# nhcha6/embodied-object-detection

Measured on AMD Instinct MI355X. Metric: frames/sec (640x640, implicit_memory); frames/sec/GPU = value / n_gpus, higher is better.
Workload: dtype f32

## Files before the change

embodied_object_detection_amd/_lib.py:

```python
from __future__ import annotations

import ctypes as C
import os

HERE = os.path.dirname(os.path.abspath(__file__))
LIB_PATH = os.environ.get("EOD_LIB_PATH") or os.path.join(HERE, "libeod_hip.so")

c_f32p = C.c_void_p
c_i32p = C.c_void_p
c_void_p = C.c_void_p


class EodError(RuntimeError):
    pass


_ERR = {-1: "EOD_ERR_BAD_DIMS", -2: "EOD_ERR_ALIGN", -3: "EOD_ERR_LAUNCH", -4: "EOD_ERR_NULL", -5: "EOD_ERR_CAPACITY"}


MAX_BATCH = 8
MAX_LEVELS = 40
SEMMAP_SCORES = 0x10000
SEMMAP_LOCATE = 0x40000
SEMMAP_PEAKS = 0x80000
SEMMAP_K_SHIFT, SEMMAP_RADIUS_SHIFT, SEMMAP_Q_SHIFT = 12, 20, 24


class EodConvDesc(C.Structure):
    _fields_ = [
        ("x", C.c_void_p), ("w", C.c_void_p), ("bias", C.c_void_p), ("res", C.c_void_p), ("y", C.c_void_p),
        ("workspace", C.c_void_p), ("workspace_bytes", C.c_size_t), ("m_count", C.c_void_p), ("m_unit", C.c_int32),
        ("m_segments", C.c_int32),
        ("N", C.c_int32), ("H", C.c_int32), ("W", C.c_int32), ("Cin", C.c_int32), ("OH", C.c_int32), ("OW", C.c_int32),
        ("Cout", C.c_int32), ("KH", C.c_int32), ("KW", C.c_int32), ("stride", C.c_int32), ("pad", C.c_int32),
        ("Kpad", C.c_int32), ("relu", C.c_int32), ("res_mode", C.c_int32), ("in_relu", C.c_int32),
        ("out_mode", C.c_int32), ("tap4", C.c_int32), ("force_tile", C.c_int32), ("force_splitk", C.c_int32),
        ("out_scale", C.c_float), ("levels", C.c_int32), ("level_off", C.c_int32 * (MAX_LEVELS + 1)), ("level_h", C.c_int32 * MAX_LEVELS),
        ("level_w", C.c_int32 * MAX_LEVELS), ("fuse_w", C.c_void_p), ("out_units", C.c_void_p), ("fuse_b", C.c_float), ("w_split", C.c_void_p),
        ("plan_rows", C.c_int32), ("lds_reserve", C.c_int32), ("gn_partial", C.c_void_p), ("gn_groups", C.c_int32),
        ("y2", C.c_void_p), ("split_n", C.c_int32), ("prefetch2", C.c_int32), ("gate", C.c_void_p),
        ("w_half", C.c_void_p), ("math", C.c_int32),
    ]


class EodConvPlan(C.Structure):
    _fields_ = [(n, C.c_int32) for n in ("tile", "bm", "bn", "bk", "splitk", "cps", "nchunks", "wavek", "glds", "tiles_m", "tiles_n",
                                         "gn_fused")]


class EodBoxRefine(C.Structure):
    _fields_ = [("deltas", C.c_void_p), ("ld", C.c_int32), ("wx", C.c_float), ("wy", C.c_float), ("ww", C.c_float), ("wh", C.c_float),
                ("clip", C.c_int32), ("img_w", C.c_float), ("img_h", C.c_float), ("boxes_out", C.c_void_p)]


class EodCenterNetLossDesc(C.Structure):
    _fields_ = [
        ("head_out", C.c_void_p), ("head_stride", C.c_int32), ("P", C.c_int32), ("levels", C.c_int32), ("level_off", C.c_int32 * 9),
        ("level_scale", C.c_float * 8), ("agn_heatmap", C.c_void_p), ("reg_targets", C.c_void_p), ("pos_inds", C.c_void_p),
        ("n_pos", C.c_int32), ("hm_focal_alpha", C.c_float), ("hm_focal_beta", C.c_float), ("loss_gamma", C.c_float),
        ("sigmoid_clamp", C.c_float), ("ignore_high_fp", C.c_float), ("pos_weight", C.c_float), ("neg_weight", C.c_float),
        ("reg_weight", C.c_float), ("num_pos_avg", C.c_float), ("reg_norm", C.c_float), ("counts_local", C.c_void_p),
        ("counts_total", C.c_void_p), ("world_size", C.c_float), ("d_head_out", C.c_void_p),
        ("losses", C.c_void_p), ("workspace", C.c_void_p), ("workspace_bytes", C.c_size_t),
    ]


class EodCenterNetTargetDesc(C.Structure):
    _fields_ = [
        ("gt_boxes", C.c_void_p), ("n_boxes", C.c_int32), ("levels", C.c_int32), ("level_off", C.c_int32 * 9), ("level_w", C.c_int32 * 8),
        ("level_stride", C.c_int32 * 8), ("soi_lo", C.c_float * 8), ("soi_hi", C.c_float * 8), ("hm_min_overlap", C.c_double),
        ("min_radius", C.c_double), ("agn_heatmap", C.c_void_p), ("reg_targets", C.c_void_p), ("pos_inds", C.c_void_p),
        ("counts", C.c_void_p),
    ]


class EodProposalDesc(C.Structure):
    _fields_ = [
        ("head_out", C.c_void_p), ("head_stride", C.c_int32), ("levels", C.c_int32), ("level_off", C.c_int32 * 6),
        ("level_w", C.c_int32 * 5), ("level_stride", C.c_int32 * 5), ("level_scale", C.c_float * 5),
        ("score_thresh", C.c_float), ("pre_nms_topk", C.c_int32), ("post_nms_topk", C.c_int32), ("nms_thresh", C.c_float),
        ("cap", C.c_int32), ("out_boxes", C.c_void_p), ("out_scores", C.c_void_p), ("out_count", C.c_void_p),
        ("workspace", C.c_void_p), ("workspace_bytes", C.c_size_t), ("batch", C.c_int32),
    ]


class EodDetDesc(C.Structure):
    _fields_ = [
        ("boxes", C.c_void_p), ("scores", C.c_void_p), ("count", C.c_void_p), ("R_cap", C.c_int32), ("C1", C.c_int32),
        ("img_w", C.c_float), ("img_h", C.c_float), ("score_thresh", C.c_float), ("nms_thresh", C.c_float),
        ("topk", C.c_int32), ("out_boxes", C.c_void_p), ("out_scores", C.c_void_p), ("out_classes", C.c_void_p),
        ("out_rows", C.c_void_p), ("out_count", C.c_void_p), ("workspace", C.c_void_p), ("workspace_bytes", C.c_size_t),
        ("out_unique_rows", C.c_void_p), ("out_unique_count", C.c_void_p), ("unique_cap", C.c_int32),
        ("out_rep_of", C.c_void_p), ("out_rep_list", C.c_void_p), ("out_rep_count", C.c_void_p), ("batch", C.c_int32),
    ]


class EodStageTailDesc(C.Structure):
    _fields_ = [("feat", C.c_void_p), ("zs", C.c_void_p), ("prob_acc", C.c_void_p), ("accumulate", C.c_int32), ("feat_norm_out", C.c_void_p),
                ("count", C.c_void_p), ("R_cap", C.c_int32), ("D", C.c_int32), ("C1", C.c_int32), ("temp", C.c_float), ("zs_mem", C.c_void_p),
                ("prop_scores", C.c_void_p), ("mem_scores_out", C.c_void_p), ("final_inv_stages", C.c_float), ("batch", C.c_int32),
                ("hb", C.c_void_p), ("w2", C.c_void_p), ("b2", C.c_void_p), ("hb_dim", C.c_int32), ("w2_ld", C.c_int32),
                ("boxes_in", C.c_void_p), ("boxes_out", C.c_void_p), ("deltas_out", C.c_void_p), ("wx", C.c_float), ("wy", C.c_float),
                ("ww", C.c_float), ("wh", C.c_float), ("clip", C.c_int32), ("img_w", C.c_float), ("img_h", C.c_float)]


class EodAdamWTensor(C.Structure):
    _fields_ = [("param", C.c_void_p), ("grad", C.c_void_p), ("exp_avg", C.c_void_p), ("exp_avg_sq", C.c_void_p), ("n", C.c_size_t),
                ("lr", C.c_double), ("weight_decay", C.c_double), ("step", C.c_int32), ("folded_out", C.c_void_p), ("row_scale", C.c_void_p),
                ("cols", C.c_int32), ("ld_out", C.c_int32), ("grad_of_folded", C.c_int32), ("inv_scale", C.c_float), ("found_inf", C.c_void_p)]


class EodRotateTensor(C.Structure):
    _fields_ = [("w", C.c_void_p), ("out", C.c_void_p), ("Cout", C.c_int32), ("KH", C.c_int32), ("KW", C.c_int32), ("Cin", C.c_int32),
                ("ld_in", C.c_int32), ("ld_out", C.c_int32)]


class EodMemWriteDesc(C.Structure):
    _fields_ = [
        ("featn", C.c_void_p), ("prop_boxes", C.c_void_p), ("prop_masks", C.c_void_p), ("det_rows", C.c_void_p),
        ("det_count", C.c_void_p), ("K_cap", C.c_int32), ("R_cap", C.c_int32), ("proj", C.c_void_p),
        ("H", C.c_int32), ("W", C.c_int32), ("D", C.c_int32), ("n_cells", C.c_int32), ("mask_thresh", C.c_float),
        ("mem", C.c_void_p), ("obs", C.c_void_p), ("k_out", C.c_void_p), ("workspace", C.c_void_p),
        ("workspace_bytes", C.c_size_t), ("dirty", C.c_void_p), ("err_flags", C.c_void_p), ("snapshot_f16", C.c_void_p),
        ("batch", C.c_int32),
    ]


SIGNATURES = {
    "eod_abi_version": (C.c_int, []),
    "eod_conv2d": (C.c_int, [C.POINTER(EodConvDesc), C.c_void_p]),
    "eod_conv2d_workspace_bytes": (C.c_size_t, [C.POINTER(EodConvDesc)]),
    "eod_conv2d_gn_fused": (C.c_int, [C.POINTER(EodConvDesc)]),
    "eod_conv2d_plan": (C.c_int, [C.POINTER(EodConvDesc), C.POINTER(EodConvPlan)]),
    "eod_groupnorm_partial_offset": (C.c_size_t, [C.c_int, C.c_int]),
    "eod_set_conv_math": (C.c_int, [C.c_int]),
    "eod_get_conv_math": (C.c_int, []),
    "eod_conv_split_weights_bytes": (C.c_size_t, [C.c_int, C.c_int]),
    "eod_conv_split_weights_bf16x3": (C.c_int, [C.c_void_p, C.c_int, C.c_int, C.c_void_p, C.c_void_p]),
    "eod_conv_half_weights_bytes": (C.c_size_t, [C.c_int, C.c_int]),
    "eod_conv_half_weights": (C.c_int, [C.c_void_p, C.c_int, C.c_int, C.c_void_p, C.c_void_p]),
    "eod_preprocess_image": (C.c_int, [C.c_void_p, C.c_void_p, C.c_int, C.c_int, C.c_int, C.c_int,
                                       C.POINTER(C.c_float), C.POINTER(C.c_float), C.c_void_p]),
    "eod_maxpool3x3s2": (C.c_int, [C.c_void_p, C.c_void_p] + [C.c_int] * 6 + [C.c_void_p]),
    "eod_groupnorm_workspace_bytes": (C.c_size_t, [C.POINTER(C.c_int32), C.c_int, C.c_int]),
    "eod_groupnorm_relu": (C.c_int, [C.c_void_p, C.c_void_p, C.c_void_p, C.c_void_p, C.POINTER(C.c_int32), C.c_int, C.c_int,
                                     C.c_int, C.c_float, C.c_void_p, C.c_int, C.c_void_p]),
    "eod_groupnorm_backward_workspace_bytes": (C.c_size_t, [C.POINTER(C.c_int32), C.c_int, C.c_int]),
    "eod_groupnorm_relu_backward": (C.c_int, [C.c_void_p, C.c_void_p, C.c_void_p, C.c_void_p, C.POINTER(C.c_int32), C.c_int, C.c_int, C.c_int,
                                              C.c_float, C.c_void_p, C.c_void_p, C.c_void_p, C.c_void_p, C.c_void_p, C.c_void_p]),
    "eod_mask_predictor_sigmoid": (C.c_int, [C.c_void_p, C.c_void_p, C.c_float, C.c_void_p, C.c_int, C.c_int, C.c_void_p,
                                             C.c_int, C.c_void_p, C.c_void_p]),
    "eod_roi_align": (C.c_int, [C.c_void_p, C.c_void_p, C.c_void_p, C.c_int, C.c_int, C.c_int, C.c_void_p, C.c_void_p, C.c_void_p,
                                C.c_int, C.c_int, C.c_void_p, C.c_int, C.c_int, C.c_void_p, C.c_void_p]),
    "eod_roi_align_backward": (C.c_int, [C.c_void_p, C.c_void_p, C.c_void_p, C.c_int, C.c_int, C.c_int, C.c_void_p, C.c_void_p, C.c_int,
                                         C.c_int, C.c_void_p, C.c_void_p]),
    "eod_centernet_loss_workspace_bytes": (C.c_size_t, []),
    "eod_centernet_loss": (C.c_int, [C.POINTER(EodCenterNetLossDesc), C.c_void_p]),
    "eod_fast_rcnn_loss_workspace_bytes": (C.c_size_t, [C.c_int]),
    "eod_fast_rcnn_loss": (C.c_int, [C.c_void_p, C.c_int, C.c_void_p, C.c_void_p, C.c_void_p, C.c_void_p, C.c_void_p, C.c_int, C.c_int,
                                     C.c_float, C.c_float, C.c_float, C.c_float, C.c_float, C.c_void_p, C.c_void_p, C.c_void_p,
                                     C.c_void_p, C.c_size_t, C.c_void_p]),
    "eod_match_label": (C.c_int, [C.c_void_p, C.c_int, C.c_void_p, C.c_void_p, C.c_int, C.c_float, C.c_int, C.c_void_p, C.c_void_p,
                                  C.c_void_p, C.c_void_p, C.c_void_p]),
    "eod_match_label_proposals": (C.c_int, [C.c_void_p, C.c_void_p, C.c_int, C.c_void_p, C.c_void_p, C.c_int, C.c_int, C.c_float, C.c_int,
                                            C.c_void_p, C.c_void_p, C.c_void_p, C.c_void_p, C.c_void_p, C.c_void_p]),
    "eod_sample_proposals": (C.c_int, [C.c_void_p, C.c_void_p, C.c_int, C.c_int, C.c_int, C.c_float, C.c_void_p, C.c_void_p, C.c_void_p]),
    "eod_zs_logits": (C.c_int, [C.c_void_p, C.c_void_p, C.c_int, C.c_int, C.c_int, C.c_float, C.c_void_p, C.c_int, C.c_void_p, C.c_void_p]),
    "eod_zs_logits_backward": (C.c_int, [C.c_void_p, C.c_void_p, C.c_void_p, C.c_int, C.c_int, C.c_int, C.c_int, C.c_float, C.c_void_p,
                                         C.c_void_p]),
    "eod_centernet_targets": (C.c_int, [C.POINTER(EodCenterNetTargetDesc), C.c_void_p]),
    "eod_unique_rows": (C.c_int, [C.c_void_p, C.c_void_p, C.c_int, C.c_int, C.c_void_p, C.c_void_p, C.c_void_p]),
    "eod_proposals_workspace_bytes": (C.c_size_t, [C.c_int, C.c_int, C.c_int, C.c_int]),
    "eod_centernet_proposals": (C.c_int, [C.POINTER(EodProposalDesc), C.c_void_p]),
    "eod_zs_classify": (C.c_int, [C.c_void_p, C.c_void_p, C.c_void_p, C.c_int, C.c_void_p, C.c_void_p, C.c_int, C.c_int,
                                  C.c_int, C.c_float, C.c_void_p, C.c_void_p, C.c_void_p, C.c_float, C.c_int, C.c_void_p]),
    "eod_cascade_stage_tail": (C.c_int, [C.POINTER(EodStageTailDesc), C.c_void_p]),
    "eod_apply_deltas": (C.c_int, [C.c_void_p, C.c_int, C.c_void_p, C.c_void_p, C.c_void_p, C.c_int, C.c_float, C.c_float,
                                   C.c_float, C.c_float, C.c_int, C.c_float, C.c_float, C.c_int, C.c_void_p]),
    "eod_cascade_scores": (C.c_int, [C.c_void_p, C.c_void_p, C.c_void_p, C.c_int, C.c_int, C.c_float, C.c_void_p]),
    "eod_detections_workspace_bytes": (C.c_size_t, [C.c_int, C.c_int]),
    "eod_fast_rcnn_inference": (C.c_int, [C.POINTER(EodDetDesc), C.c_void_p]),
    "eod_detector_postprocess": (C.c_int, [C.c_void_p, C.c_void_p, C.c_void_p, C.c_void_p, C.c_int, C.c_float, C.c_float,
                                           C.c_float, C.c_float, C.c_void_p, C.c_void_p, C.c_void_p, C.c_void_p, C.c_void_p,
                                           C.c_void_p, C.c_int, C.c_void_p]),
    "eod_concat_lists": (C.c_int, [C.c_void_p, C.c_void_p, C.c_int, C.c_int, C.c_int, C.c_void_p, C.c_void_p, C.c_void_p]),
    "eod_paste_masks": (C.c_int, [C.c_void_p, C.c_void_p, C.c_void_p, C.c_void_p, C.c_int, C.c_int, C.c_int, C.c_float,
                                  C.c_void_p, C.c_int, C.c_int, C.c_void_p]),
    "eod_unproject_grid_index": (C.c_int, [C.c_void_p, C.c_int, C.c_int, C.POINTER(C.c_float), C.c_float, C.c_float, C.c_float,
                                           C.c_float, C.POINTER(C.c_float), C.POINTER(C.c_float), C.c_float, C.c_int, C.c_int,
                                           C.c_int, C.c_void_p, C.c_void_p, C.c_void_p]),
    "eod_memory_normalize_f16": (C.c_int, [C.c_void_p, C.c_void_p, C.c_void_p, C.c_int, C.c_int, C.c_void_p]),
    "eod_memory_normalize_dirty_f16": (C.c_int, [C.c_void_p, C.c_void_p, C.c_void_p, C.c_void_p, C.c_int, C.c_int, C.c_void_p]),
    "eod_memory_gather_pool": (C.c_int, [C.c_void_p, C.c_void_p, C.c_int, C.c_int, C.c_int, C.c_int, C.c_void_p, C.c_void_p,
                                         C.c_int, C.c_int, C.c_void_p]),
    "eod_memory_pooled_halves": (C.c_size_t, [C.c_int, C.c_int]),
    "eod_memory_project_weights_bytes": (C.c_size_t, []),
    "eod_memory_project_prepare": (C.c_int, [C.c_void_p] * 8),
    "eod_memory_project_fuse": (C.c_int, [C.c_void_p, C.c_void_p, C.c_void_p, C.c_int, C.c_int, C.c_float, C.c_int, C.c_int, C.c_void_p]),
    "eod_memory_project_backward_weights": (C.c_int, [C.c_void_p] * 4 + [C.c_int, C.c_int, C.c_float] + [C.c_void_p] * 7),
    "eod_memory_project_backward_weights_workspace_bytes": (C.c_size_t, []),
    "eod_memory_project_backward_weights_ws": (C.c_int, [C.c_void_p] * 4 + [C.c_int, C.c_int, C.c_float] + [C.c_void_p] * 7 +
                                               [C.c_size_t, C.c_void_p]),
    "eod_memory_pool_backward": (C.c_int, [C.c_void_p] * 3 + [C.c_int, C.c_int] + [C.c_void_p] * 5),
    "eod_conv2d_backward_weights": (C.c_int, [C.c_void_p, C.c_void_p] + [C.c_int] * 9 + [C.c_void_p, C.c_void_p, C.c_void_p]),
    "eod_conv2d_backward_weights_levels_workspace_bytes": (C.c_size_t, [C.c_int] * 5),
    "eod_conv2d_backward_weights_levels": (C.c_int, [C.c_void_p, C.c_void_p, C.c_int, C.c_void_p, C.c_void_p, C.c_void_p] + [C.c_int] * 5 +
                                           [C.c_void_p, C.c_void_p, C.c_void_p, C.c_size_t, C.c_void_p]),
    "eod_conv2d_backward_weights_workspace_bytes": (C.c_size_t, [C.c_int] * 9),
    "eod_conv2d_backward_weights_ws": (C.c_int, [C.c_void_p, C.c_void_p] + [C.c_int] * 9 + [C.c_void_p, C.c_void_p, C.c_void_p, C.c_size_t,
                                                                                          C.c_void_p]),
    "eod_conv2d_backward_input": (C.c_int, [C.c_void_p, C.c_void_p] + [C.c_int] * 10 + [C.c_void_p, C.c_void_p]),
    "eod_upsample2_sum_backward": (C.c_int, [C.c_void_p, C.c_void_p, C.c_int, C.c_int, C.c_int, C.c_int, C.c_int, C.c_void_p]),
    "eod_maxpool3x3s2_backward": (C.c_int, [C.c_void_p] * 4 + [C.c_int] * 6 + [C.c_void_p]),
    "eod_relu_backward": (C.c_int, [C.c_void_p, C.c_void_p, C.c_void_p, C.c_size_t, C.c_void_p]),
    "eod_adamw_step": (C.c_int, [C.c_void_p, C.c_void_p, C.c_void_p, C.c_void_p, C.c_size_t, C.c_double, C.c_double, C.c_double, C.c_double,
                                 C.c_double, C.c_int, C.c_double, C.c_void_p]),
    "eod_conv_rotate_weights": (C.c_int, [C.c_void_p, C.c_int, C.c_int, C.c_int, C.c_int, C.c_int, C.c_void_p, C.c_int, C.c_void_p]),
    "eod_conv_rotate_weights_multi": (C.c_int, [C.POINTER(EodRotateTensor), C.c_int, C.c_void_p]),
    "eod_adamw_step_multi": (C.c_int, [C.POINTER(EodAdamWTensor), C.c_int, C.c_double, C.c_double, C.c_double, C.c_double, C.c_void_p]),
    "eod_memory_scores": (C.c_int, [C.c_void_p, C.c_void_p, C.c_void_p, C.c_void_p, C.c_void_p, C.c_int, C.c_int, C.c_int,
                                    C.c_void_p]),
    "eod_memory_write_workspace_bytes": (C.c_size_t, [C.c_int] * 6),
    "eod_memory_write_init": (C.c_int, [C.c_void_p, C.c_size_t, C.c_int, C.c_int, C.c_int, C.c_int, C.c_int, C.c_int, C.c_void_p]),
    "eod_memory_write": (C.c_int, [C.POINTER(EodMemWriteDesc), C.c_void_p]),
    "eod_semmap_labels": (C.c_int, [C.c_void_p, C.c_void_p, C.c_void_p, C.c_int, C.c_int, C.c_int, C.c_float, C.c_void_p,
                                    C.c_void_p, C.c_void_p]),
    "eod_fill_f32": (C.c_int, [C.c_void_p, C.c_float, C.c_size_t, C.c_void_p]),
    "eod_fill_i32": (C.c_int, [C.c_void_p, C.c_int32, C.c_size_t, C.c_void_p]),
}

_lib = None


def load():
    global _lib
    if _lib is not None:
        return _lib
    if not os.path.exists(LIB_PATH):
        raise EodError(
            f"{LIB_PATH} is missing: the HIP extension is not built. Run `python -m embodied_object_detection_amd.build` "
            "(hipcc --offload-arch=gfx950). There is no CPU fallback for the product path.")
    lib = C.CDLL(LIB_PATH)
    for name, (res, args) in SIGNATURES.items():
        fn = getattr(lib, name)
        fn.restype = res
        fn.argtypes = args
    _lib = lib
    return lib


def check(status: int, what: str):
    if status != 0:
        raise EodError(f"{what} failed: {_ERR.get(status, status)}")
```

embodied_object_detection_amd/csrc/conv_common.h:

```cpp
#pragma once
#include "eod_common.h"
#include "conv_border_order.h"
#include "../../include/eod_hip.h"

namespace eodconv {


struct ConvArgs {
  const float* x;
  const float* w;
  const float* bias;
  const float* res;
  const float* gate;
  float* y;
  float* partial;
  const int* m_count;
  int m_unit;
  int m_segs, seg_rows;
  const float* fuse_w;
  const int* out_units;
  float fuse_b;
  int N, H, W, Cin, OH, OW, Cout, KH, KW, stride, pad, Kpad;
  int M, nchunks, splitk, cps;
  int relu, res_mode, in_relu, out_mode;
  int tiles_m, tiles_n;
  float out_scale;
  int nlv;
  int lv_off[EOD_MAX_LEVELS + 1], lv_h[EOD_MAX_LEVELS], lv_w[EOD_MAX_LEVELS];
  unsigned x_bytes, w_bytes;
  const void* w3;
  unsigned w3_bytes;
  const void* wh;
  unsigned wh_bytes;
  double* gn_partial;
  int gn_groups;
  float* y2;
  int split_n;
  FastDiv div_ow, div_oh, div_cd, div_row;
  int border;
  FastDiv div_bh, div_bw, div_bi;
};

__device__ __forceinline__ int conv_row_limit(const ConvArgs& p, int M) {
  if (p.m_count && p.m_segs <= 1) {
    const int lim = *p.m_count * p.m_unit;
    M = lim < M ? lim : M;
  }
  return M;
}

__device__ __forceinline__ bool conv_row_active(const ConvArgs& p, int m) {
  if (!p.m_count || p.m_segs <= 1) return true;
  const int s = m / p.seg_rows;
  return m - s * p.seg_rows < p.m_count[s] * p.m_unit;
}

__device__ __forceinline__ bool conv_tile_active(const ConvArgs& p, int m0, int bm) {
  if (!p.m_count || p.m_segs <= 1) return true;
  const int last = (m0 + bm - 1 < p.M ? m0 + bm - 1 : p.M - 1);
  const int s0 = m0 / p.seg_rows, s1 = last / p.seg_rows;
  if (m0 - s0 * p.seg_rows < p.m_count[s0] * p.m_unit) return true;
  for (int s = s0 + 1; s <= s1; ++s)
    if (p.m_count[s] > 0) return true;
  return false;
}

__device__ __forceinline__ int border_rois(const ConvArgs& p) {
  const int c = *p.m_count;
  return c < p.N ? c : p.N;
}
__device__ __forceinline__ int border_storage_row(const ConvArgs& p, int m, int rois) {
  const BorderRow b = border_row(m, rois, p.OH, p.OW, p.div_ow, p.div_bh, p.div_bw, p.div_bi);
  return (b.img * p.OH + b.oy) * p.OW + b.ox;
}

template <bool GATE = false>
__device__ __forceinline__ float epilogue_store(const ConvArgs& p, float v, int m, int n) {
  int co = n;
  size_t oidx;
  if (p.out_mode == 1) {
    const int Cd = p.Cout >> 2;
    const int quad = (int)fdiv((unsigned)n, p.div_cd);
    co = n - quad * Cd;
    const int dy = quad >> 1, dx = quad & 1;
    const int t = (int)fdiv((unsigned)m, p.div_ow);
    const int ox = m - t * p.OW;
    const int img = (int)fdiv((unsigned)t, p.div_oh);
    const int oy = t - img * p.OH;
    oidx = ((size_t)(img * 2 * p.OH + 2 * oy + dy) * (2 * p.OW) + (2 * ox + dx)) * Cd + co;
  } else {
    oidx = (size_t)m * p.Cout + n;
  }
  if (p.bias) v += p.bias[co];
  v *= p.out_scale;
  if (p.res_mode == 1) {
    v += p.res[(size_t)m * p.Cout + n];
  } else if (p.res_mode == 2) {
    const int t = (int)fdiv((unsigned)m, p.div_ow);
    const int ox = m - t * p.OW;
    const int img = (int)fdiv((unsigned)t, p.div_oh);
    const int oy = t - img * p.OH;
    const int rh = p.OH >> 1, rw = p.OW >> 1;
    v += p.res[((size_t)(img * rh + (oy >> 1)) * rw + (ox >> 1)) * p.Cout + n];
  }
  if (p.split_n > 0) {
    if (n >= p.split_n) {
      if (p.relu) v = fmaxf(v, 0.0f);
      p.y2[(size_t)m * (p.Cout - p.split_n) + (n - p.split_n)] = v;
    } else {
      p.y[(size_t)m * p.split_n + n] = v;
    }
    return v;
  }
  if (p.relu) v = fmaxf(v, 0.0f);
  if (GATE && p.gate && !(p.gate[oidx] > 0.0f)) v = 0.0f;
  p.y[oidx] = v;
  return v;
}

__device__ __forceinline__ unsigned long long tap_mask(int iy0, int ix0, int hh, int ww, int KH, int KW) {
  unsigned long long mask = 0;
  int tp = 0;
  for (int ky = 0; ky < KH; ++ky) {
    const bool rok = (unsigned)(iy0 + ky) < (unsigned)hh;
    for (int kx = 0; kx < KW; ++kx, ++tp) {
      const bool ok = rok && ((unsigned)(ix0 + kx) < (unsigned)ww);
      mask |= (unsigned long long)ok << tp;
    }
  }
  return mask;
}

template <int TM, int TN, bool GATE = false, bool BORDER = false>
__device__ __forceinline__ void store_wave_tiles(const ConvArgs& p, const f32x16 (&acc)[TM][TN], int m_base, int n_base, int M, int z,
                                                 int lane) {
  const int half = lane >> 5;
  const int rois = BORDER ? border_rois(p) : 0;
#pragma unroll
  for (int i = 0; i < TM; ++i) {
#pragma unroll
    for (int j = 0; j < TN; ++j) {
      const int n = n_base + j * 32 + (lane & 31);
#pragma unroll
      for (int r = 0; r < 16; ++r) {
        const int row = (r & 3) + 8 * (r >> 2) + 4 * half;
        const int m = m_base + i * 32 + row;
        if (m < M && n < p.Cout && conv_row_active(p, m)) {
          const float v = acc[i][j][r];
          if (BORDER) {
            epilogue_store<GATE>(p, v, border_storage_row(p, m, rois), n);
          } else if (p.splitk > 1) {
            p.partial[((size_t)z * p.M + m) * p.Cout + n] = v;
          } else {
            epilogue_store<GATE>(p, v, m, n);
          }
        }
      }
    }
  }
}

void launch_conv_fp32(const ConvArgs& a, int tile, int bk, bool tap4, dim3 grid, hipStream_t s, int lds_reserve = 0, int prefetch2 = 0);
void launch_conv_bf16x3(const ConvArgs& a, int tile, dim3 grid, hipStream_t s);
void launch_conv_wavek(const ConvArgs& a, int nw, dim3 grid, hipStream_t s);
void launch_conv_pointwise(const ConvArgs& a, int np, dim3 grid, hipStream_t s);
void launch_split_weights(const float* w, void* out, int Cout, int Kpad, hipStream_t s);
void launch_conv_f16(const ConvArgs& a, int tile, int bk, dim3 grid, hipStream_t s);
void launch_half_weights(const float* w, void* out, int Cout, int Kpad, hipStream_t s);

}
```

embodied_object_detection_amd/csrc/conv_fp32.hip:

```cpp
#include "conv_operands.h"

namespace eodconv {
namespace {

template <int BM, int BN, int BK, bool TAP4, bool MULTI, int PIPE = 0>
__global__ __launch_bounds__(256) void conv_igemm_kernel(ConvArgs p) {
  constexpr bool BORDER = PIPE == 3;
  static_assert(!BORDER || (BM == 64 && BN == 64 && BK == 32 && !TAP4 && !MULTI), "border-major order: the plain 64x64 kernel");
  constexpr bool PF2 = PIPE == 1;
  constexpr bool DB = PIPE == 2;
  constexpr int LS = BK + 4;
  constexpr int TM = BM / 64, TN = BN / 64;
  constexpr int QPR = BK / 4;
  constexpr int RPP = 256 / QPR;
  constexpr int AR = BM / RPP, BR = BN / RPP;
  static_assert(!TAP4 || BK == 32, "the stem path stages one 7x7 tap per float4: BK must be 32");
  constexpr int BUF = (BM + BN) * LS;
  __shared__ __attribute__((aligned(16))) float lds[(DB ? 2 : 1) * BUF];
  float* As = lds;
  float* Bs = lds + BM * LS;

  const int tid = threadIdx.x;
  const int lane = tid & 63;
  const int wave = tid >> 6;
  const int wm = wave >> 1, wn = wave & 1;

  int M, tile_m, tile_n;
  if constexpr (BORDER) {
    if (!conv_claim_tile_border<BM>(p, M, tile_m, tile_n)) return;
  } else {
    const int t = conv_first_tile<BM>(p, M);
    if (t < 0) return;
    tile_m = t / p.tiles_n;
    tile_n = t - tile_m * p.tiles_n;
  }
  const int m0 = tile_m * BM, n0 = tile_n * BN;
  if (!conv_tile_active(p, m0, BM)) return;
  const int z = blockIdx.y;
  int c_end;
  const int c_begin = conv_chunk_range(p, p.cps, z, c_end);

  const int lr = tid / QPR, lq = tid % QPR;
  int a_off[AR], a_iy[AR], a_ix[AR];
  unsigned a_voff[AR];
  unsigned long long a_mask[AR];
  unsigned a_pitch[MULTI ? AR : 1];
  const int rois = BORDER ? border_rois(p) : 0;
#pragma unroll
  for (int i = 0; i < AR; ++i) {
    const int m = m0 + lr + RPP * i;
    const bool rowok = m < M;
    RowOrigin o;
    if constexpr (BORDER) o = conv_row_origin_border(p, m, rowok, rois);
    else o = conv_row_origin<MULTI>(p, m, rowok);
    a_iy[i] = rowok ? o.iy0 : -(1 << 28);
    a_ix[i] = o.ix0;
    a_off[i] = o.off;
    if (!TAP4) conv_row_address<MULTI>(p, o, rowok, lq, a_voff[i], a_mask[i], a_pitch[MULTI ? i : 0]);
  }
  unsigned w_voff[BR];
#pragma unroll
  for (int j = 0; j < BR; ++j) w_voff[j] = conv_w_row_offset(p, n0 + lr + RPP * j, lq);
  const __amdgpu_buffer_rsrc_t rsrc_x = conv_buffer(p.x, p.x_bytes);
  const __amdgpu_buffer_rsrc_t rsrc_w = conv_buffer(p.w, p.w_bytes);

  unsigned live = 0;
  if constexpr (BORDER) {
    unsigned mine = 0;
#pragma unroll
    for (int i = 0; i < AR; ++i) mine |= (unsigned)a_mask[i];
    unsigned wv = 0;
#pragma unroll
    for (int tp = 0; tp < 9; ++tp) wv |= (__ballot((mine >> tp) & 1u) != 0ull ? 1u : 0u) << tp;
    if (lane == 0) lds[wave] = __uint_as_float(wv);
    __syncthreads();
    live = __float_as_uint(lds[0]) | __float_as_uint(lds[1]) | __float_as_uint(lds[2]) | __float_as_uint(lds[3]);
    live = __builtin_amdgcn_readfirstlane(live);
    __syncthreads();
    c_end = c_begin + __popc(live) * (p.Cin / BK);
  }

  f32x4 ar0[AR], br0[BR];
  f32x4 ar1[PF2 ? AR : 1], br1[PF2 ? BR : 1];
  ChunkWalker<BK, MULTI> walk(p, c_begin);
  auto load_chunk = [&](int chunk, auto& ar, auto& br) {
    int k0 = chunk * BK;
    if (!TAP4) {
      if constexpr (BORDER) {
        const unsigned rest = live >> walk.tap;
        if (walk.c0 == 0 && !(rest & 1u)) walk.seek(p, walk.tap + __builtin_ctz(rest));
      }
      const TapInfo ti = walk.next(p);
      if constexpr (BORDER) k0 = (int)(ti.k0b >> 2);
#pragma unroll
      for (int i = 0; i < AR; ++i) ar[i] = conv_load_a<MULTI>(rsrc_x, ti, a_voff[i], a_mask[i], a_pitch[MULTI ? i : 0]);
    } else {
      const int tap = chunk * 8 + lq;
      const int ky = tap / p.KW;
      const int kx = tap - ky * p.KW;
      const bool tv = tap < p.KH * p.KW;
#pragma unroll
      for (int i = 0; i < AR; ++i) {
        const int iy = a_iy[i] + ky, ix = a_ix[i] + kx;
        const bool ok = tv && ((unsigned)iy < (unsigned)p.H) && ((unsigned)ix < (unsigned)p.W);
        f32x4 v = {0.f, 0.f, 0.f, 0.f};
        if (ok) v = *reinterpret_cast<const f32x4*>(p.x + (size_t)(a_off[i] + iy * p.W + ix) * 4);
        ar[i] = v;
      }
    }
    if (p.in_relu) {
#pragma unroll
      for (int i = 0; i < AR; ++i) ar[i] = conv_relu4(ar[i]);
    }
#pragma unroll
    for (int j = 0; j < BR; ++j)
      br[j] = __builtin_bit_cast(f32x4, __builtin_amdgcn_raw_buffer_load_b128(rsrc_w, w_voff[j], k0 * 4, 0));
  };

  f32x16 acc[TM][TN];
#pragma unroll
  for (int i = 0; i < TM; ++i)
#pragma unroll
    for (int j = 0; j < TN; ++j)
#pragma unroll
      for (int r = 0; r < 16; ++r) acc[i][j][r] = 0.f;
  f32x16 acc_b;
#pragma unroll
  for (int r = 0; r < 16; ++r) acc_b[r] = 0.f;

  const int frag_row = lane & 31;
  const int frag_k = 4 * (lane >> 5);
  const float* a_base = As + (wm * TM * 32 + frag_row) * LS + frag_k;
  const float* b_base = Bs + (wn * TN * 32 + frag_row) * LS + frag_k;

  auto multiply = [&](const float* ab, const float* bb) {
#pragma unroll
    for (int kk = 0; kk < BK / 8; ++kk) {
      f32x4 af[TM], bf[TN];
#pragma unroll
      for (int i = 0; i < TM; ++i) af[i] = *reinterpret_cast<const f32x4*>(ab + i * 32 * LS + kk * 8);
#pragma unroll
      for (int j = 0; j < TN; ++j) bf[j] = *reinterpret_cast<const f32x4*>(bb + j * 32 * LS + kk * 8);
      __builtin_amdgcn_s_setprio(1);
#pragma unroll
      for (int tt = 0; tt < 4; ++tt)
#pragma unroll
        for (int i = 0; i < TM; ++i)
#pragma unroll
          for (int j = 0; j < TN; ++j)
            if (TM * TN == 1 && (tt & 1))
              acc_b = __builtin_amdgcn_mfma_f32_32x32x2f32(af[i][tt], bf[j][tt], acc_b, 0, 0, 0);
            else
              acc[i][j] = __builtin_amdgcn_mfma_f32_32x32x2f32(af[i][tt], bf[j][tt], acc[i][j], 0, 0, 0);
      __builtin_amdgcn_s_setprio(0);
    }
  };
  auto stage_and_multiply = [&](auto& ar, auto& br, int next_chunk) {
#pragma unroll
    for (int i = 0; i < AR; ++i) *reinterpret_cast<f32x4*>(As + (lr + RPP * i) * LS + 4 * lq) = ar[i];
#pragma unroll
    for (int j = 0; j < BR; ++j) *reinterpret_cast<f32x4*>(Bs + (lr + RPP * j) * LS + 4 * lq) = br[j];
    __syncthreads();
    if (next_chunk < c_end) load_chunk(next_chunk, ar, br);
    if constexpr (TM * TN == 1) {
      f32x4 af[2], bf[2];
      af[0] = *reinterpret_cast<const f32x4*>(a_base);
      bf[0] = *reinterpret_cast<const f32x4*>(b_base);
#pragma unroll
      for (int kk = 0; kk < BK / 8; ++kk) {
        const int cur = kk & 1, nxt = cur ^ 1;
        if (kk + 1 < BK / 8) {
          af[nxt] = *reinterpret_cast<const f32x4*>(a_base + (kk + 1) * 8);
          bf[nxt] = *reinterpret_cast<const f32x4*>(b_base + (kk + 1) * 8);
        }
        __builtin_amdgcn_s_setprio(1);
#pragma unroll
        for (int tt = 0; tt < 4; ++tt)
          if (tt & 1)
            acc_b = __builtin_amdgcn_mfma_f32_32x32x2f32(af[cur][tt], bf[cur][tt], acc_b, 0, 0, 0);
          else
            acc[0][0] = __builtin_amdgcn_mfma_f32_32x32x2f32(af[cur][tt], bf[cur][tt], acc[0][0], 0, 0, 0);
        __builtin_amdgcn_s_setprio(0);
      }
    } else {
      multiply(a_base, b_base);
    }
    __syncthreads();
  };
  load_chunk(c_begin, ar0, br0);
  if constexpr (DB) {
    auto store_tiles = [&](int buf) {
#pragma unroll
      for (int i = 0; i < AR; ++i) *reinterpret_cast<f32x4*>(As + buf * BUF + (lr + RPP * i) * LS + 4 * lq) = ar0[i];
#pragma unroll
      for (int j = 0; j < BR; ++j) *reinterpret_cast<f32x4*>(Bs + buf * BUF + (lr + RPP * j) * LS + 4 * lq) = br0[j];
    };
    store_tiles(0);
    __syncthreads();
    int cur = 0;
    for (int chunk = c_begin; chunk < c_end; ++chunk) {
      const bool more = chunk + 1 < c_end;
      if (more) load_chunk(chunk + 1, ar0, br0);
      multiply(a_base + cur * BUF, b_base + cur * BUF);
      if (more) store_tiles(cur ^ 1);
      __syncthreads();
      cur ^= 1;
    }
  } else if constexpr (PF2) {
    if (c_begin + 1 < c_end) load_chunk(c_begin + 1, ar1, br1);
    for (int chunk = c_begin; chunk < c_end; chunk += 2) {
      stage_and_multiply(ar0, br0, chunk + 2);
      if (chunk + 1 < c_end) stage_and_multiply(ar1, br1, chunk + 3);
    }
  } else {
    for (int chunk = c_begin; chunk < c_end; ++chunk) stage_and_multiply(ar0, br0, chunk + 1);
  }

  if (TM * TN == 1) {
#pragma unroll
    for (int r = 0; r < 16; ++r) acc[0][0][r] += acc_b[r];
  }
  if constexpr (BM == 64 && BN == 256) {
    if (p.out_mode == 2) {
      float sred[16];
#pragma unroll
      for (int r = 0; r < 16; ++r) sred[r] = 0.f;
#pragma unroll
      for (int j = 0; j < TN; ++j) {
        const int co = (wn * TN + j) * 32 + (lane & 31);
        const float bw = p.bias ? p.bias[co] : 0.f;
        const float pw = p.fuse_w[co];
#pragma unroll
        for (int r = 0; r < 16; ++r) {
          float v = (acc[0][j][r] + bw) * p.out_scale;
          if (p.relu) v = fmaxf(v, 0.f);
          sred[r] += v * pw;
        }
      }
#pragma unroll
      for (int off = 16; off > 0; off >>= 1)
#pragma unroll
        for (int r = 0; r < 16; ++r) sred[r] += __shfl_xor(sred[r], off, 64);
      float* red = lds;
      if ((lane & 31) == 0) {
        const int half = lane >> 5;
#pragma unroll
        for (int r = 0; r < 16; ++r) red[(wm * 2 + wn) * 32 + (r & 3) + 8 * (r >> 2) + 4 * half] = sred[r];
      }
      __syncthreads();
      if (tid < BM) {
        const int wr = tid >> 5, rr = tid & 31;
        const float v = red[(wr * 2 + 0) * 32 + rr] + red[(wr * 2 + 1) * 32 + rr] + p.fuse_b;
        const int m = m0 + tid;
        if (m < M) {
          const int tq = (int)fdiv((unsigned)m, p.div_ow);
          const int ox = m - tq * p.OW;
          const int img = (int)fdiv((unsigned)tq, p.div_oh);
          const int oy = tq - img * p.OH;
          const int unit = p.out_units ? p.out_units[img] : img;
          const int dy = tile_n >> 1, dx = tile_n & 1;
          p.y[((size_t)unit * 2 * p.OH + 2 * oy + dy) * (2 * p.OW) + 2 * ox + dx] = eod_sigmoid_precise(v);
        }
      }
      return;
    }
  }
  store_wave_tiles<TM, TN, BM == 64 && BN == 64, BORDER>(p, acc, m0 + wm * TM * 32, n0 + wn * TN * 32, M, z, lane);
}


template <int NW, bool MULTI>
__global__ __launch_bounds__(NW * 64) void conv_wavek_kernel(ConvArgs p) {
  constexpr int BK = 32;
  constexpr int LS = BK + 4;
  constexpr int AR = 4;
  __shared__ __attribute__((aligned(16))) float lds[NW * 2 * 32 * LS];
  const int tid = threadIdx.x;
  const int lane = tid & 63;
  const int wave = tid >> 6;
  float* As = lds + wave * (2 * 32 * LS);
  float* Bs = As + 32 * LS;

  int M;
  const int t = conv_first_tile<32>(p, M);
  if (t < 0) return;
  const int tile_m = t / p.tiles_n;
  const int tile_n = t - tile_m * p.tiles_n;
  const int m0 = tile_m * 32, n0 = tile_n * 32;
  if (!conv_tile_active(p, m0, 32)) return;

  int c_end;
  const int c_begin = conv_chunk_range(p, (p.nchunks + NW - 1) / NW, wave, c_end);

  const int lr = lane >> 3, lq = lane & 7;
  unsigned a_voff[AR];
  unsigned long long a_mask[AR];
  unsigned a_pitch[MULTI ? AR : 1];
  unsigned w_voff[AR];
#pragma unroll
  for (int i = 0; i < AR; ++i) {
    conv_row_address<MULTI>(p, m0 + lr + 8 * i, M, lq, a_voff[i], a_mask[i], a_pitch[MULTI ? i : 0]);
    w_voff[i] = conv_w_row_offset(p, n0 + lr + 8 * i, lq);
  }
  const __amdgpu_buffer_rsrc_t rsrc_x = conv_buffer(p.x, p.x_bytes);
  const __amdgpu_buffer_rsrc_t rsrc_w = conv_buffer(p.w, p.w_bytes);

  f32x4 ar0[AR], br0[AR], ar1[AR], br1[AR];
  ChunkWalker<BK, MULTI> walk(p, c_begin);
  auto load_chunk = [&](int chunk, f32x4 (&ar)[AR], f32x4 (&br)[AR]) {
    const int k0 = chunk * BK;
    const TapInfo ti = walk.next(p);
#pragma unroll
    for (int i = 0; i < AR; ++i) ar[i] = conv_load_a<MULTI>(rsrc_x, ti, a_voff[i], a_mask[i], a_pitch[MULTI ? i : 0]);
    if (p.in_relu) {
#pragma unroll
      for (int i = 0; i < AR; ++i) ar[i] = conv_relu4(ar[i]);
    }
#pragma unroll
    for (int j = 0; j < AR; ++j)
      br[j] = __builtin_bit_cast(f32x4, __builtin_amdgcn_raw_buffer_load_b128(rsrc_w, w_voff[j], k0 * 4, 0));
  };

  f32x16 acc, acc_b;
#pragma unroll
  for (int r = 0; r < 16; ++r) {
    acc[r] = 0.f;
    acc_b[r] = 0.f;
  }
  const int frag_row = lane & 31;
  const int frag_k = 4 * (lane >> 5);
  const float* a_base = As + frag_row * LS + frag_k;
  const float* b_base = Bs + frag_row * LS + frag_k;

  auto stage_and_multiply = [&](f32x4 (&ar)[AR], f32x4 (&br)[AR], int next_chunk) {
#pragma unroll
    for (int i = 0; i < AR; ++i) *reinterpret_cast<f32x4*>(As + (lr + 8 * i) * LS + 4 * lq) = ar[i];
#pragma unroll
    for (int j = 0; j < AR; ++j) *reinterpret_cast<f32x4*>(Bs + (lr + 8 * j) * LS + 4 * lq) = br[j];
    __builtin_amdgcn_fence(__ATOMIC_RELEASE, "wavefront");
    __builtin_amdgcn_wave_barrier();
    __builtin_amdgcn_fence(__ATOMIC_ACQUIRE, "wavefront");
    if (next_chunk < c_end) load_chunk(next_chunk, ar, br);
#pragma unroll
    for (int kk = 0; kk < BK / 8; ++kk) {
      const f32x4 af = *reinterpret_cast<const f32x4*>(a_base + kk * 8);
      const f32x4 bf = *reinterpret_cast<const f32x4*>(b_base + kk * 8);
      acc = __builtin_amdgcn_mfma_f32_32x32x2f32(af[0], bf[0], acc, 0, 0, 0);
      acc_b = __builtin_amdgcn_mfma_f32_32x32x2f32(af[1], bf[1], acc_b, 0, 0, 0);
      acc = __builtin_amdgcn_mfma_f32_32x32x2f32(af[2], bf[2], acc, 0, 0, 0);
      acc_b = __builtin_amdgcn_mfma_f32_32x32x2f32(af[3], bf[3], acc_b, 0, 0, 0);
    }
    __builtin_amdgcn_fence(__ATOMIC_RELEASE, "wavefront");
    __builtin_amdgcn_wave_barrier();
    __builtin_amdgcn_fence(__ATOMIC_ACQUIRE, "wavefront");
  };
  if (c_begin < c_end) load_chunk(c_begin, ar0, br0);
  if (c_begin + 1 < c_end) load_chunk(c_begin + 1, ar1, br1);
  for (int chunk = c_begin; chunk < c_end; chunk += 2) {
    stage_and_multiply(ar0, br0, chunk + 2);
    if (chunk + 1 < c_end) stage_and_multiply(ar1, br1, chunk + 3);
  }
#pragma unroll
  for (int r = 0; r < 16; ++r) acc[r] += acc_b[r];

  __syncthreads();
  float* red = lds;
  if (wave > 0) {
#pragma unroll
    for (int r = 0; r < 16; ++r) red[((wave - 1) * 16 + r) * 64 + lane] = acc[r];
  }
  __syncthreads();
  if (wave != 0) return;
#pragma unroll
  for (int w = 1; w < NW; ++w)
#pragma unroll
    for (int r = 0; r < 16; ++r) acc[r] += red[((w - 1) * 16 + r) * 64 + lane];
  f32x16 out[1][1];
  out[0][0] = acc;
  store_wave_tiles<1, 1, true>(p, out, m0, n0, M, 0, lane);
}

}

template <int BM, int BN>
static void launch_fp32_tile(const ConvArgs& a, bool tap4, int bk, dim3 grid, hipStream_t s, int dyn) {
  if (tap4)
    hipLaunchKernelGGL((conv_igemm_kernel<BM, BN, 32, true, false>), grid, dim3(256), dyn, s, a);
  else if (a.nlv > 0 && bk == 64)
    hipLaunchKernelGGL((conv_igemm_kernel<BM, BN, 64, false, true>), grid, dim3(256), dyn, s, a);
  else if (a.nlv > 0)
    hipLaunchKernelGGL((conv_igemm_kernel<BM, BN, 32, false, true>), grid, dim3(256), dyn, s, a);
  else if (bk == 64)
    hipLaunchKernelGGL((conv_igemm_kernel<BM, BN, 64, false, false>), grid, dim3(256), dyn, s, a);
  else
    hipLaunchKernelGGL((conv_igemm_kernel<BM, BN, 32, false, false>), grid, dim3(256), dyn, s, a);
}

void launch_conv_fp32(const ConvArgs& a, int tile, int bk, bool tap4, dim3 grid, hipStream_t s, int lds_reserve, int prefetch2) {
  const int dyn = lds_reserve > 0 ? lds_reserve : 0;
  if (a.border) {
    hipLaunchKernelGGL((conv_igemm_kernel<64, 64, 32, false, false, 3>), grid, dim3(256), dyn, s, a);
    return;
  }
  if (prefetch2 == 1 && !tap4 && a.nlv == 0 && bk == 32 && tile == 3) {
    hipLaunchKernelGGL((conv_igemm_kernel<64, 64, 32, false, false, 1>), grid, dim3(256), dyn, s, a);
    return;
  }
  if (prefetch2 == 2 && !tap4 && bk == 32 && tile == 3) {
    if (a.nlv > 0) hipLaunchKernelGGL((conv_igemm_kernel<64, 64, 32, false, true, 2>), grid, dim3(256), dyn, s, a);
    else hipLaunchKernelGGL((conv_igemm_kernel<64, 64, 32, false, false, 2>), grid, dim3(256), dyn, s, a);
    return;
  }
  switch (tile) {
    case 5: hipLaunchKernelGGL((conv_igemm_kernel<64, 256, 32, false, false>), grid, dim3(256), dyn, s, a); break;
    case 1: launch_fp32_tile<128, 128>(a, tap4, bk, grid, s, dyn); break;
    case 2: launch_fp32_tile<128, 64>(a, tap4, bk, grid, s, dyn); break;
    default: launch_fp32_tile<64, 64>(a, tap4, bk, grid, s, dyn); break;
  }
}

void launch_conv_wavek(const ConvArgs& a, int nw, dim3 grid, hipStream_t s) {
  if (a.nlv > 0) {
    if (nw == 8) hipLaunchKernelGGL((conv_wavek_kernel<8, true>), grid, dim3(512), 0, s, a);
    else hipLaunchKernelGGL((conv_wavek_kernel<4, true>), grid, dim3(256), 0, s, a);
  } else {
    if (nw == 8) hipLaunchKernelGGL((conv_wavek_kernel<8, false>), grid, dim3(512), 0, s, a);
    else hipLaunchKernelGGL((conv_wavek_kernel<4, false>), grid, dim3(256), 0, s, a);
  }
}

}
```

embodied_object_detection_amd/csrc/conv_igemm.hip:

```cpp
#include "conv_common.h"
#include "../../include/eod_hip.h"
#include <atomic>
#include <cstdlib>
#include <cstring>

namespace {

using namespace eodconv;

template <int VEC>
__global__ __launch_bounds__(256) void conv_splitk_reduce_kernel(ConvArgs p) {
  EOD_CHAIN_PRIO();
  const int M = conv_row_limit(p, p.M);
  const unsigned per_row = (unsigned)p.Cout / VEC;
  const unsigned total = (unsigned)M * per_row;
  const size_t slab = (size_t)p.M * p.Cout;
  for (unsigned idx = blockIdx.x * blockDim.x + threadIdx.x; idx < total; idx += gridDim.x * blockDim.x) {
    const unsigned m = fdiv(idx, p.div_row);
    if (!conv_row_active(p, (int)m)) continue;
    const unsigned n = (idx - m * per_row) * VEC;
    const float* src = p.partial + (size_t)m * p.Cout + n;
    if (VEC == 4) {
      f32x4 v = {0.f, 0.f, 0.f, 0.f};
      for (int zb = 0; zb < p.splitk; zb += 4) {
        f32x4 t[4];
#pragma unroll
        for (int j = 0; j < 4; ++j)
          if (zb + j < p.splitk) t[j] = *reinterpret_cast<const f32x4*>(src + (size_t)(zb + j) * slab);
#pragma unroll
        for (int j = 0; j < 4; ++j)
          if (zb + j < p.splitk) v += t[j];
      }
      epilogue_store<true>(p, v.x, (int)m, (int)n);
      epilogue_store<true>(p, v.y, (int)m, (int)n + 1);
      epilogue_store<true>(p, v.z, (int)m, (int)n + 2);
      epilogue_store<true>(p, v.w, (int)m, (int)n + 3);
    } else {
      float v = 0.f;
      for (int z = 0; z < p.splitk; ++z) v += src[z * slab];
      epilogue_store<true>(p, v, (int)m, (int)n);
    }
  }
}

#define EOD_GN_ROWS 32
__global__ __launch_bounds__(256) void conv_splitk_reduce_gn_kernel(ConvArgs p) {
  EOD_CHAIN_PRIO();
  __shared__ double red[4][64][2];
  int level = 0, first_chunk = 0;
  for (;;) {
    const int rows = p.lv_off[level + 1] - p.lv_off[level];
    const int nch = (rows + EOD_GN_ROWS - 1) / EOD_GN_ROWS;
    if ((int)blockIdx.x < first_chunk + nch || level + 1 >= p.nlv) break;
    first_chunk += nch;
    ++level;
  }
  const int r0 = p.lv_off[level] + ((int)blockIdx.x - first_chunk) * EOD_GN_ROWS;
  const int r1 = min(r0 + EOD_GN_ROWS, p.lv_off[level + 1]);
  const int C = p.Cout;
  const int c4 = C >> 2;
  const int nsub = 256 / c4;
  const int col = threadIdx.x % c4, sub = threadIdx.x / c4;
  const int cpg4 = (C / p.gn_groups) >> 2;
  const size_t slab = (size_t)p.M * C;
  double s = 0.0, q = 0.0;
  for (int r = r0 + sub; r < r1; r += nsub) {
    const float* src = p.partial + (size_t)r * C + col * 4;
    f32x4 v = {0.f, 0.f, 0.f, 0.f};
    for (int zb = 0; zb < p.splitk; zb += 4) {
      f32x4 t[4];
#pragma unroll
      for (int j = 0; j < 4; ++j)
        if (zb + j < p.splitk) t[j] = *reinterpret_cast<const f32x4*>(src + (size_t)(zb + j) * slab);
#pragma unroll
      for (int j = 0; j < 4; ++j)
        if (zb + j < p.splitk) v += t[j];
    }
    const double o0 = (double)epilogue_store<true>(p, v.x, r, col * 4 + 0);
    const double o1 = (double)epilogue_store<true>(p, v.y, r, col * 4 + 1);
    const double o2 = (double)epilogue_store<true>(p, v.z, r, col * 4 + 2);
    const double o3 = (double)epilogue_store<true>(p, v.w, r, col * 4 + 3);
    s += o0; q += o0 * o0;
    s += o1; q += o1 * o1;
    s += o2; q += o2 * o2;
    s += o3; q += o3 * o3;
  }
  for (int off = 1; off < cpg4; off <<= 1) {
    s += __shfl_xor(s, off, 64);
    q += __shfl_xor(q, off, 64);
  }
  if ((col % cpg4) == 0) {
    red[sub][col / cpg4][0] = s;
    red[sub][col / cpg4][1] = q;
  }
  __syncthreads();
  if ((int)threadIdx.x < p.gn_groups) {
    double ts = 0.0, tq = 0.0;
    for (int u = 0; u < nsub; ++u) {
      ts += red[u][threadIdx.x][0];
      tq += red[u][threadIdx.x][1];
    }
    p.gn_partial[((size_t)blockIdx.x * p.gn_groups + threadIdx.x) * 2 + 0] = ts;
    p.gn_partial[((size_t)blockIdx.x * p.gn_groups + threadIdx.x) * 2 + 1] = tq;
  }
}

std::atomic<int>& math_mode() {
  static std::atomic<int> v([] {
    const char* e = getenv("EOD_CONV_MATH");
    if (e && strcmp(e, "bf16x3") == 0) return EOD_MATH_BF16X3;
    if (e && strcmp(e, "f16") == 0) return EOD_MATH_F16;
    return EOD_MATH_FP32;
  }());
  return v;
}

struct Plan {
  int tile;
  int bk;
  int glds;
  int bm, bn, tiles_m, tiles_n, splitk, cps, nchunks;
  int wavek;
  int pw_np;
  int border;
};

constexpr int kForcePointwise = 30;

int effective_math(const EodConvDesc* d) { return d->math > 0 ? d->math - 1 : math_mode().load(std::memory_order_relaxed); }

bool pointwise_eligible(const EodConvDesc* d) {
  return effective_math(d) == EOD_MATH_FP32 && d->KH == 1 && d->KW == 1 && d->stride == 1 && d->pad == 0 && d->levels <= 0 && !d->tap4 &&
         d->Cin == d->Kpad && (d->Cin == 64 || d->Cin == 128 || d->Cin == 256) && d->Cout % 64 == 0 && d->out_mode == 0 &&
         (d->res_mode == 0 || d->res_mode == 1) && !d->in_relu && !d->gate && !d->m_count && d->split_n == 0 && !d->gn_partial &&
         d->lds_reserve == 0;
}

constexpr int kForceBorder = 43;
constexpr bool kBorderAuto = true;

bool border_eligible(const EodConvDesc* d) {
  return effective_math(d) == EOD_MATH_FP32 && d->KH == 3 && d->KW == 3 && d->stride == 1 && d->pad == 1 && d->levels <= 0 && !d->tap4 &&
         d->m_count && d->m_segments <= 1 && d->m_unit == d->OH * d->OW && d->OH >= 3 && d->OW >= 3 && d->Cin % 32 == 0 &&
         d->out_mode == 0 && d->res_mode == 0 && !d->in_relu && !d->gate && d->split_n == 0 && !d->gn_partial && d->prefetch2 == 0;
}

Plan make_plan(const EodConvDesc* d, int M) {
  static const int cfg[5][2] = {{128, 128}, {128, 64}, {64, 64}, {256, 128}, {64, 256}};
  Plan pl{};
  int pick = 2;
  const int ft = d->force_tile % 10, fbk = d->force_tile / 10;
  const bool half_ok = !d->tap4 && !d->in_relu;
  const bool f16_forced = (fbk == 8 || fbk == 9) && half_ok;
  if (f16_forced) pick = ft == 4 ? 3 : 2;
  else if (ft >= 1 && ft <= 3) pick = ft - 1;
  else if (ft == 4 && fbk == 5 && half_ok) pick = 3;
  const bool bk64_ok = !d->tap4 && d->Cin % 64 == 0 && d->Kpad % 64 == 0;
  pl.glds = f16_forced ? 3 : ((fbk == 5 && half_ok) ? 2 : 0);
  const int Mp = (d->plan_rows > 0 && d->plan_rows < M) ? d->plan_rows : M;
  const int math = effective_math(d);
  if (d->force_tile == 0 && math == EOD_MATH_F16 && half_ok) {
    pl.glds = 3;
    pick = (long)((Mp + 255) / 256) * ((d->Cout + 127) / 128) >= 256 ? 3 : 2;
  }
  if (d->force_tile == 0 && math == EOD_MATH_BF16X3 && half_ok) {
    pl.glds = 2;
    const long t128 = (long)((Mp + 127) / 128) * ((d->Cout + 127) / 128);
    const long t256 = (long)((Mp + 255) / 256) * ((d->Cout + 127) / 128);
    pick = t256 >= 256 ? 3 : (t128 >= 512 ? 0 : 2);
  }
  if (d->out_mode == 2) {
    pick = 4;
    pl.glds = 0;
  }
  if (d->gate) {
    const bool f16_gated = d->math == EOD_MATH_F16 + 1 && half_ok && d->levels <= 0 && (d->force_tile == 0 || f16_forced);
    pick = 2;
    pl.glds = f16_gated ? 3 : 0;
  }
  if (pl.glds == 3) pl.bk = (fbk == 8 && d->Cin % 64 == 0) ? 64 : 32;
  else pl.bk = (pl.glds == 0 && d->out_mode != 2 && fbk == 2 && bk64_ok) ? 64 : 32;
  const int nchunks = d->Kpad / pl.bk;
  pl.nchunks = nchunks;
  pl.tile = pick + 1;
  pl.bm = cfg[pick][0];
  pl.bn = cfg[pick][1];
  pl.tiles_m = (M + pl.bm - 1) / pl.bm;
  pl.tiles_n = (d->Cout + pl.bn - 1) / pl.bn;
  const long tiles = (long)((Mp + pl.bm - 1) / pl.bm) * pl.tiles_n;
  int splitk = 1;
  if (d->out_mode == 2) {
    splitk = 1;
  } else if (d->force_splitk > 0) {
    splitk = d->force_splitk;
  } else if (pl.glds == 0 && !d->tap4 && nchunks >= 8 &&
             ((d->force_tile == 6 || d->force_tile == 7) ||
              (tiles < 256 && nchunks <= 192 && pl.bk == 32 && d->force_tile == 0 &&
               ((Mp <= 512 && nchunks / (nchunks >= 64 ? 8 : 4) >= 8) || nchunks >= 128)))) {
    pl.wavek = d->force_tile == 6 ? 4 : (d->force_tile == 7 ? 8 : (nchunks >= 64 ? 8 : 4));
    pl.bk = 32;
    pl.nchunks = d->Kpad / 32;
    pl.bm = pl.bn = 32;
    pl.tiles_m = (M + 31) / 32;
    pl.tiles_n = (d->Cout + 31) / 32;
  } else if (tiles < 256 && nchunks >= 8) {
    const int target = (nchunks >= 128 && Mp <= 512) ? 1792 : 512;
    int want = (int)((target + tiles - 1) / tiles);
    int maxs = nchunks / 4;
    splitk = want < maxs ? want : maxs;
    if (splitk < 1) splitk = 1;
  } else if (tiles >= 256 && tiles <= 1024 && d->m_count == nullptr && nchunks >= 18) {
    double best = 1e30;
    for (int sct = 1; sct <= 4; ++sct) {
      if (nchunks / sct < 9) break;
      const double est = (double)((tiles * sct + 255) / 256) / sct + (sct > 1 ? 0.12 : 0.0);
      if (est < best - 1e-9) {
        best = est;
        splitk = sct;
      }
    }
  }
  if (splitk > nchunks) splitk = nchunks;
  pl.cps = (nchunks + splitk - 1) / splitk;
  pl.splitk = (nchunks + pl.cps - 1) / pl.cps;
  const bool pw_forced = d->force_tile == kForcePointwise && d->force_splitk <= 1;
  const bool pw_auto = d->force_tile == 0 && d->force_splitk == 0 && pointwise_eligible(d) && pl.splitk == 1 && !pl.wavek && tiles >= 256 &&
                       !(d->Kpad == 256 && d->Cout < 1024);
  if (pw_forced || pw_auto) {
    const int panels = d->Cout / 64;
    const long row_tiles = (Mp + 63) / 64;
    const long want = tiles >= 256 ? 512 : 1;
    int np = 1;
    for (int cand = 4; cand > 1; cand >>= 1)
      if (panels >= cand && row_tiles * ((panels + cand - 1) / cand) >= want) {
        np = cand;
        break;
      }
    pl.pw_np = np;
    pl.tile = 6;
    pl.glds = 0;
    pl.bk = 32;
    pl.nchunks = d->Kpad / 32;
    pl.bm = 64;
    pl.bn = 64 * np;
    pl.tiles_m = (M + 63) / 64;
    pl.tiles_n = (panels + np - 1) / np;
    pl.splitk = 1;
    pl.cps = pl.nchunks;
    pl.wavek = 0;
  }
  const bool border_forced = d->force_tile == kForceBorder && d->force_splitk <= 1;
  const bool border_auto = kBorderAuto && d->force_tile == 0 && border_eligible(d) && pl.glds == 0 && pl.tile == 3 && pl.bk == 32 &&
                           pl.splitk == 1 && !pl.wavek;
  if (border_forced) {
    pl.splitk = 1;
    pl.cps = pl.nchunks;
  }
  pl.border = (border_forced || border_auto) ? 1 : 0;
  return pl;
}

int total_rows(const EodConvDesc* d) { return d->levels > 0 ? d->level_off[d->levels] : d->N * d->OH * d->OW; }

int check_desc(const EodConvDesc* d) {
  if (!d || !d->x || !d->w || !d->y) return EOD_ERR_NULL;
  if (d->N <= 0 || d->Cin <= 0 || d->Cout <= 0) return EOD_ERR_BAD_DIMS;
  if (d->levels <= 0 && (d->H <= 0 || d->W <= 0 || d->OH <= 0 || d->OW <= 0)) return EOD_ERR_BAD_DIMS;
  if (d->KH <= 0 || d->KW <= 0 || d->stride <= 0 || d->pad < 0) return EOD_ERR_BAD_DIMS;
  if (d->Kpad % 32 != 0 || d->Kpad < d->KH * d->KW * d->Cin) return EOD_ERR_BAD_DIMS;
  if (d->tap4) {
    if (d->Cin != 4) return EOD_ERR_BAD_DIMS;
  } else {
    if (d->Cin % 32 != 0 || d->Kpad != d->KH * d->KW * d->Cin) return EOD_ERR_BAD_DIMS;
  }
  if (d->levels > 0) {
    if (d->levels > EOD_MAX_LEVELS || d->N != 1 || d->stride != 1 || d->KH != d->KW || d->pad != d->KH / 2 || d->tap4 || d->out_mode != 0 ||
        d->res_mode == 2 || d->level_off[0] != 0)
      return EOD_ERR_BAD_DIMS;
    for (int l = 0; l < d->levels; ++l)
      if (d->level_h[l] <= 0 || d->level_w[l] <= 0 || d->level_off[l + 1] - d->level_off[l] != d->level_h[l] * d->level_w[l])
        return EOD_ERR_BAD_DIMS;
  } else {
    if (d->OH != (d->H + 2 * d->pad - d->KH) / d->stride + 1) return EOD_ERR_BAD_DIMS;
    if (d->OW != (d->W + 2 * d->pad - d->KW) / d->stride + 1) return EOD_ERR_BAD_DIMS;
  }
  if (d->levels <= 0 && (long)d->N * d->H * d->W * d->Cin >= (1L << 29)) return EOD_ERR_BAD_DIMS;
  if ((long)d->Cout * d->Kpad >= (1L << 29)) return EOD_ERR_BAD_DIMS;
  if (d->KH * d->KW > 64) return EOD_ERR_BAD_DIMS;
  if ((long)total_rows(d) * (d->Cout > d->Cin ? d->Cout : d->Cin) >= (1L << 31)) return EOD_ERR_BAD_DIMS;
  if (d->out_mode == 1 && (d->Cout % 4 != 0)) return EOD_ERR_BAD_DIMS;
  if (d->out_mode == 2) {
    if (d->Cout != 1024 || d->KH != 1 || d->KW != 1 || d->stride != 1 || d->tap4 || d->levels > 0 || d->res_mode != 0 || d->in_relu ||
        d->force_splitk > 1)
      return EOD_ERR_BAD_DIMS;
    if (!d->fuse_w) return EOD_ERR_NULL;
  }
  if (d->out_mode < 0 || d->out_mode > 2) return EOD_ERR_BAD_DIMS;
  if (d->res_mode != 0 && !d->res) return EOD_ERR_NULL;
  if (d->res_mode == 2 && ((d->OH & 1) || (d->OW & 1))) return EOD_ERR_BAD_DIMS;
  if (d->m_count && d->m_unit <= 0) return EOD_ERR_BAD_DIMS;
  if (d->m_segments > 1) {
    if (!d->m_count || d->levels > 0 || d->out_mode == 2 || d->m_segments > EOD_MAX_BATCH || d->N % d->m_segments != 0)
      return EOD_ERR_BAD_DIMS;
    if (((long)(d->N / d->m_segments) * d->OH * d->OW) % d->m_unit != 0) return EOD_ERR_BAD_DIMS;
  }
  if (d->gate && (d->out_mode != 0 || d->split_n != 0 || d->gn_partial)) return EOD_ERR_BAD_DIMS;
  if (d->gate && d->force_tile != 0 && d->force_tile % 10 != 3 && d->force_tile != 6 && d->force_tile != 7) return EOD_ERR_BAD_DIMS;
  if (d->gate && d->force_tile / 10 == 5) return EOD_ERR_BAD_DIMS;
  if (d->gate && (d->force_tile / 10 == 8 || d->force_tile / 10 == 9) &&
      (d->math != EOD_MATH_F16 + 1 || d->force_tile % 10 != 3 || d->levels > 0 || d->tap4 || d->in_relu))
    return EOD_ERR_BAD_DIMS;
  if (d->math < 0 || d->math > EOD_MATH_F16 + 1) return EOD_ERR_BAD_DIMS;
  if ((d->force_tile / 10 == 8 || d->force_tile / 10 == 9) && d->force_tile % 10 != 3 && d->force_tile % 10 != 4) return EOD_ERR_BAD_DIMS;
  if (d->lds_reserve < 0 || d->lds_reserve > 48 * 1024) return EOD_ERR_BAD_DIMS;
  if (d->force_tile == kForcePointwise && (!pointwise_eligible(d) || d->force_splitk > 1)) return EOD_ERR_BAD_DIMS;
  if (d->force_tile == kForceBorder && (!border_eligible(d) || d->force_splitk > 1)) return EOD_ERR_BAD_DIMS;
  if (d->split_n != 0) {
    if (!d->y2) return EOD_ERR_NULL;
    if (d->split_n < 0 || d->split_n >= d->Cout || d->out_mode != 0 || d->res_mode != 0 || d->levels > 0 || d->gn_partial)
      return EOD_ERR_BAD_DIMS;
  }
  if (d->gn_partial) {
    const int cpg = d->gn_groups > 0 ? d->Cout / d->gn_groups : 0;
    if (d->levels <= 0 || d->m_count || d->out_mode != 0 || d->gn_groups <= 0 || d->gn_groups > 64 || d->Cout % d->gn_groups != 0 ||
        cpg > 64 || (cpg & (cpg - 1)) != 0 || cpg < 4 || d->Cout % 4 != 0 || d->Cout > 1024 || 256 % (d->Cout / 4) != 0 ||
        64 % (cpg / 4) != 0)
      return EOD_ERR_BAD_DIMS;
  }
  if (!eod_aligned16(d->x) || !eod_aligned16(d->w) || !eod_aligned16(d->w_split) || !eod_aligned16(d->w_half)) return EOD_ERR_ALIGN;
  return EOD_OK;
}

}

extern "C" int eod_set_conv_math(int mode) {
  if (mode != EOD_MATH_FP32 && mode != EOD_MATH_BF16X3 && mode != EOD_MATH_F16) return EOD_ERR_BAD_DIMS;
  return math_mode().exchange(mode);
}

extern "C" int eod_get_conv_math(void) { return math_mode().load(); }

extern "C" size_t eod_conv_split_weights_bytes(int Cout, int Kpad) {
  return (Cout > 0 && Kpad > 0 && Kpad % 32 == 0) ? (size_t)Cout * Kpad * 6 : 0;
}

extern "C" int eod_conv_split_weights_bf16x3(const float* w, int Cout, int Kpad, void* out, eod_stream_t stream) {
  if (!w || !out) return EOD_ERR_NULL;
  if (Cout <= 0 || Kpad <= 0 || Kpad % 32 != 0 || (long)Cout * Kpad * 6 >= (1L << 32)) return EOD_ERR_BAD_DIMS;
  if (!eod_aligned16(w) || !eod_aligned16(out)) return EOD_ERR_ALIGN;
  launch_split_weights(w, out, Cout, Kpad, static_cast<hipStream_t>(stream));
  return eod_launch_status();
}

extern "C" size_t eod_conv_half_weights_bytes(int Cout, int Kpad) {
  return (Cout > 0 && Kpad > 0 && Kpad % 32 == 0) ? (size_t)Cout * Kpad * 2 : 0;
}

extern "C" int eod_conv_half_weights(const float* w, int Cout, int Kpad, void* out, eod_stream_t stream) {
  if (!w || !out) return EOD_ERR_NULL;
  if (Cout <= 0 || Kpad <= 0 || Kpad % 32 != 0 || (long)Cout * Kpad >= (1L << 29)) return EOD_ERR_BAD_DIMS;
  if (!eod_aligned16(w) || !eod_aligned16(out)) return EOD_ERR_ALIGN;
  launch_half_weights(w, out, Cout, Kpad, static_cast<hipStream_t>(stream));
  return eod_launch_status();
}

extern "C" int eod_conv2d_gn_fused(const EodConvDesc* d) {
  EodConvDesc t = *d;
  t.gn_partial = nullptr;
  if (check_desc(&t) != EOD_OK) return 0;
  return make_plan(&t, total_rows(&t)).splitk > 1 ? 1 : 0;
}

extern "C" int eod_conv2d_plan(const EodConvDesc* d, EodConvPlan* out) {
  if (!out) return EOD_ERR_NULL;
  const int st = check_desc(d);
  if (st != EOD_OK) return st;
  const Plan pl = make_plan(d, total_rows(d));
  out->tile = pl.tile; out->bm = pl.bm; out->bn = pl.bn; out->bk = pl.bk;
  out->splitk = pl.splitk; out->cps = pl.cps; out->nchunks = pl.nchunks;
  out->wavek = pl.wavek; out->glds = pl.glds;
  out->tiles_m = pl.tiles_m; out->tiles_n = pl.tiles_n;
  out->gn_fused = (d->gn_partial && pl.splitk > 1) ? 1 : 0;
  return EOD_OK;
}

extern "C" size_t eod_conv2d_workspace_bytes(const EodConvDesc* d) {
  if (check_desc(d) != EOD_OK) return 0;
  const int M = total_rows(d);
  const Plan pl = make_plan(d, M);
  if (pl.splitk <= 1) return 0;
  return (size_t)pl.splitk * M * d->Cout * sizeof(float);
}

extern "C" int eod_conv2d(const EodConvDesc* d, eod_stream_t stream) {
  const int st = check_desc(d);
  if (st != EOD_OK) return st;
  hipStream_t s = static_cast<hipStream_t>(stream);
  ConvArgs a{};
  a.x = d->x; a.w = d->w; a.bias = d->bias; a.res = d->res; a.y = d->y;
  a.partial = d->workspace;
  a.m_count = d->m_count; a.m_unit = d->m_unit;
  a.m_segs = d->m_segments > 1 ? d->m_segments : 1;
  a.seg_rows = a.m_segs > 1 ? (d->N / d->m_segments) * d->OH * d->OW : 0;
  a.fuse_w = d->fuse_w; a.out_units = d->out_units; a.fuse_b = d->fuse_b;
  a.N = d->N; a.H = d->H; a.W = d->W; a.Cin = d->Cin; a.OH = d->OH; a.OW = d->OW; a.Cout = d->Cout;
  a.KH = d->KH; a.KW = d->KW; a.stride = d->stride; a.pad = d->pad; a.Kpad = d->Kpad;
  a.M = total_rows(d);
  a.div_ow = eod_make_fastdiv((unsigned)(d->OW > 0 ? d->OW : 1));
  a.div_oh = eod_make_fastdiv((unsigned)(d->OH > 0 ? d->OH : 1));
  a.div_row = eod_make_fastdiv((unsigned)(d->Cout % 4 == 0 ? d->Cout / 4 : d->Cout));
  a.div_cd = eod_make_fastdiv((unsigned)((d->Cout >> 2) > 0 ? (d->Cout >> 2) : 1));
  a.div_bh = eod_make_fastdiv((unsigned)(d->OH > 2 ? d->OH - 2 : 1));
  a.div_bw = eod_make_fastdiv((unsigned)(d->OW > 2 ? d->OW - 2 : 1));
  a.div_bi = eod_make_fastdiv((unsigned)(d->OH > 2 && d->OW > 2 ? (d->OH - 2) * (d->OW - 2) : 1));
  {
    const size_t xe = d->levels > 0 ? (size_t)d->level_off[d->levels] * d->Cin : (size_t)d->N * d->H * d->W * d->Cin;
    a.x_bytes = (unsigned)(xe * sizeof(float));
    a.w_bytes = (unsigned)((size_t)d->Cout * d->Kpad * sizeof(float));
    a.w3 = d->w_split;
    a.w3_bytes = (unsigned)((size_t)d->Cout * d->Kpad * 6);
    a.wh = d->w_half;
    a.wh_bytes = (unsigned)((size_t)d->Cout * d->Kpad * 2);
  }
  a.nlv = d->levels > 0 ? d->levels : 0;
  for (int l = 0; l < a.nlv; ++l) {
    a.lv_off[l] = d->level_off[l];
    a.lv_h[l] = d->level_h[l];
    a.lv_w[l] = d->level_w[l];
  }
  if (a.nlv) a.lv_off[a.nlv] = d->level_off[a.nlv];
  a.relu = d->relu; a.res_mode = d->res_mode; a.in_relu = d->in_relu; a.out_mode = d->out_mode;
  a.gate = d->gate;
  a.out_scale = d->out_scale;
  a.gn_partial = d->gn_partial;
  a.gn_groups = d->gn_groups;
  a.y2 = d->y2;
  a.split_n = d->split_n;
  const Plan pl = make_plan(d, a.M);
  if (d->gn_partial && pl.splitk <= 1) return EOD_ERR_BAD_DIMS;
  a.nchunks = pl.nchunks;
  a.splitk = pl.splitk; a.cps = pl.cps; a.tiles_m = pl.tiles_m; a.tiles_n = pl.tiles_n;
  a.border = pl.border;
  if (pl.splitk > 1) {
    const size_t need = (size_t)pl.splitk * a.M * a.Cout * sizeof(float);
    if (!d->workspace || d->workspace_bytes < need) return EOD_ERR_CAPACITY;
  }
  dim3 grid(pl.tiles_m * pl.tiles_n, pl.splitk);
  if (pl.border) grid.x = (pl.tiles_m + 7) / 8 * 8 * pl.tiles_n;
  if (pl.pw_np) launch_conv_pointwise(a, pl.pw_np, grid, s);
  else if (pl.wavek) launch_conv_wavek(a, pl.wavek, grid, s);
  else if (pl.glds == 3) launch_conv_f16(a, pl.tile, pl.bk, grid, s);
  else if (pl.glds == 2) launch_conv_bf16x3(a, pl.tile, grid, s);
  else launch_conv_fp32(a, pl.tile, pl.bk, d->tap4 != 0, grid, s, d->lds_reserve, d->prefetch2);
  if (pl.splitk > 1) {
    const size_t total = (size_t)a.M * a.Cout;
    const bool vec = a.Cout % 4 == 0;
    int blocks = (int)((total / (vec ? 4 : 1) + 255) / 256);
    if (blocks > 2048) blocks = 2048;
    if (blocks < 1) blocks = 1;
    if (a.gn_partial) {
      int chunks = 0;
      for (int l = 0; l < a.nlv; ++l) chunks += (a.lv_off[l + 1] - a.lv_off[l] + EOD_GN_ROWS - 1) / EOD_GN_ROWS;
      hipLaunchKernelGGL(conv_splitk_reduce_gn_kernel, dim3(chunks), dim3(256), 0, s, a);
    } else if (vec) hipLaunchKernelGGL(conv_splitk_reduce_kernel<4>, dim3(blocks), dim3(256), 0, s, a);
    else hipLaunchKernelGGL(conv_splitk_reduce_kernel<1>, dim3(blocks), dim3(256), 0, s, a);
  }
  return eod_launch_status();
}
```

embodied_object_detection_amd/csrc/conv_operands.h:

```cpp
#pragma once
#include "conv_common.h"

namespace eodconv {

template <int BM>
__device__ __forceinline__ int conv_first_tile(const ConvArgs& p, int& M) {
  M = conv_row_limit(p, p.M);
  const int ntiles = ((M + BM - 1) / BM) * p.tiles_n;
  if ((int)blockIdx.x >= ntiles) return -1;
  return xcd_remap(blockIdx.x, ntiles);
}

template <int BM>
__device__ __forceinline__ bool conv_claim_tile_border(const ConvArgs& p, int& M, int& tile_m, int& tile_n) {
  M = conv_row_limit(p, p.M);
  const int live = (M + BM - 1) / BM;
  const int xcd = blockIdx.x & 7, k = blockIdx.x >> 3;
  const int g = k / p.tiles_n;
  const int r = g * 8 + xcd;
  tile_n = k - g * p.tiles_n;
  tile_m = live - 1 - r;
  return r < live;
}

__device__ __forceinline__ int conv_chunk_range(const ConvArgs& p, int per, int idx, int& c_end) {
  const int c_begin = idx * per;
  c_end = c_begin + per;
  if (c_end > p.nchunks) c_end = p.nchunks;
  return c_begin;
}

struct RowOrigin {
  int iy0, ix0, off, hh, ww;
};
template <bool MULTI>
__device__ __forceinline__ RowOrigin conv_row_origin(const ConvArgs& p, int m, bool rowok) {
  RowOrigin o = {0, 0, 0, 1, 1};
  if (rowok) {
    if (MULTI) {
      int l = 0;
      while (l + 1 < p.nlv && m >= p.lv_off[l + 1]) ++l;
      const int local = m - p.lv_off[l];
      o.ww = p.lv_w[l];
      o.hh = p.lv_h[l];
      const int oy = local / o.ww;
      o.iy0 = oy - p.pad;
      o.ix0 = (local - oy * o.ww) - p.pad;
      o.off = p.lv_off[l];
    } else {
      const int t = (int)fdiv((unsigned)m, p.div_ow);
      const int ox = m - t * p.OW;
      const int img = (int)fdiv((unsigned)t, p.div_oh);
      const int oy = t - img * p.OH;
      o.iy0 = oy * p.stride - p.pad;
      o.ix0 = ox * p.stride - p.pad;
      o.off = img * p.H * p.W;
      o.hh = p.H;
      o.ww = p.W;
    }
  }
  return o;
}

__device__ __forceinline__ RowOrigin conv_row_origin_border(const ConvArgs& p, int m, bool rowok, int rois) {
  RowOrigin o = {0, 0, 0, 1, 1};
  if (rowok) {
    const BorderRow b = border_row(m, rois, p.OH, p.OW, p.div_ow, p.div_bh, p.div_bw, p.div_bi);
    o.iy0 = b.oy * p.stride - p.pad;
    o.ix0 = b.ox * p.stride - p.pad;
    o.off = b.img * p.H * p.W;
    o.hh = p.H;
    o.ww = p.W;
  }
  return o;
}

template <bool MULTI>
__device__ __forceinline__ void conv_row_address(const ConvArgs& p, const RowOrigin& o, bool rowok, int lq, unsigned& voff,
                                                 unsigned long long& mask, unsigned& pitch) {
  mask = rowok ? tap_mask(o.iy0, o.ix0, o.hh, o.ww, p.KH, p.KW) : 0ull;
  voff = (unsigned)(((o.off + o.iy0 * o.ww + o.ix0) * p.Cin + 4 * lq) * 4);
  if (MULTI) pitch = (unsigned)(o.ww * p.Cin * 4);
}
template <bool MULTI>
__device__ __forceinline__ void conv_row_address(const ConvArgs& p, int m, int M, int lq, unsigned& voff, unsigned long long& mask,
                                                 unsigned& pitch) {
  const bool rowok = m < M;
  conv_row_address<MULTI>(p, conv_row_origin<MULTI>(p, m, rowok), rowok, lq, voff, mask, pitch);
}

__device__ __forceinline__ unsigned conv_w_row_offset(const ConvArgs& p, int n, int lq) {
  return n < p.Cout ? (unsigned)((n * p.Kpad + 4 * lq) * 4) : 0xFFFFFFFFu;
}

__device__ __forceinline__ __amdgpu_buffer_rsrc_t conv_buffer(const void* ptr, unsigned bytes) {
  return __builtin_amdgcn_make_buffer_rsrc(const_cast<void*>(ptr), 0, bytes, 0x00020000);
}

struct TapInfo {
  int tap, ky;
  unsigned tap_off, k0b;
};

template <int BK, bool MULTI>
struct ChunkWalker {
  int tap, c0, ky, kx, k0;
  __device__ __forceinline__ ChunkWalker(const ConvArgs& p, int c_begin) {
    k0 = c_begin * BK;
    tap = k0 / p.Cin;
    c0 = k0 - tap * p.Cin;
    ky = tap / p.KW;
    kx = tap - ky * p.KW;
  }
  __device__ __forceinline__ void seek(const ConvArgs& p, int t) {
    tap = t;
    c0 = 0;
    k0 = t * p.Cin;
    ky = t / p.KW;
    kx = t - ky * p.KW;
  }
  __device__ __forceinline__ TapInfo next(const ConvArgs& p) {
    TapInfo ti;
    ti.tap = tap < 63 ? tap : 63;
    ti.ky = ky;
    ti.tap_off = MULTI ? (unsigned)((kx * p.Cin + c0) * 4) : (unsigned)(((ky * p.W + kx) * p.Cin + c0) * 4);
    ti.k0b = (unsigned)(k0 * 4);
    k0 += BK;
    c0 += BK;
    if (c0 >= p.Cin) {
      c0 = 0;
      ++tap;
      if (++kx == p.KW) {
        kx = 0;
        ++ky;
      }
    }
    return ti;
  }
};

template <bool MULTI>
__device__ __forceinline__ f32x4 conv_load_a(__amdgpu_buffer_rsrc_t rsrc_x, const TapInfo& ti, unsigned voff, unsigned long long mask,
                                             unsigned pitch) {
  const bool ok = (mask >> ti.tap) & 1ull;
  unsigned vo = voff + ti.tap_off;
  if (MULTI) vo += (unsigned)ti.ky * pitch;
  vo = ok ? vo : 0xFFFFFFFFu;
  return __builtin_bit_cast(f32x4, __builtin_amdgcn_raw_buffer_load_b128(rsrc_x, vo, 0, 0));
}

__device__ __forceinline__ f32x4 conv_relu4(f32x4 v) {
  v.x = fmaxf(v.x, 0.f);
  v.y = fmaxf(v.y, 0.f);
  v.z = fmaxf(v.z, 0.f);
  v.w = fmaxf(v.w, 0.f);
  return v;
}

}
```

embodied_object_detection_amd/modeling/backbone.py:

```python
from __future__ import annotations

from typing import Dict, List, Optional, Tuple

import torch

from .. import ops
from ..registry import BACKBONE_REGISTRY

RESNET50_LAYERS = (3, 4, 6, 3)


class ResNet50Trunk:
    def __init__(self, sd: Dict[str, torch.Tensor], device):
        base = "backbone.bottom_up.base"

        def bn(p):
            return sd[f"{p}.weight"], sd[f"{p}.bias"], sd[f"{p}.running_mean"], sd[f"{p}.running_var"]

        w, b = ops.fold_bn(sd[f"{base}.conv1.weight"], *bn(f"{base}.bn1"))
        self.stem = ops.Conv(w, b, stride=2, pad=3, device=device, cin_pad=4, name="stem")
        self.blocks: List[Tuple] = []
        for li, nblk in enumerate(RESNET50_LAYERS, start=1):
            for bi in range(nblk):
                p = f"{base}.layer{li}.{bi}"
                stride = 2 if (bi == 0 and li > 1) else 1
                w1, b1 = ops.fold_bn(sd[f"{p}.conv1.weight"], *bn(f"{p}.bn1"))
                w2, b2 = ops.fold_bn(sd[f"{p}.conv2.weight"], *bn(f"{p}.bn2"))
                w3, b3 = ops.fold_bn(sd[f"{p}.conv3.weight"], *bn(f"{p}.bn3"))
                c1 = ops.Conv(w1, b1, device=device, name=f"{p}.conv1")
                c2 = ops.Conv(w2, b2, stride=stride, pad=1, device=device, name=f"{p}.conv2")
                c3 = ops.Conv(w3, b3, device=device, name=f"{p}.conv3")
                ds = None
                if f"{p}.downsample.0.weight" in sd:
                    wd, bd = ops.fold_bn(sd[f"{p}.downsample.0.weight"], *bn(f"{p}.downsample.1"))
                    ds = ops.Conv(wd, bd, stride=stride, device=device, name=f"{p}.downsample")
                self.blocks.append((li, c1, c2, c3, ds))

    def forward(self, x4: torch.Tensor, H: int, W: int, N: int = 1, plan_like_single: bool = True, keep: Optional[dict] = None,
                math: Optional[str] = None):
        mk = {} if math is None else {"math": math}

        def pr(conv, hh, ww):
            oh, ow = conv.out_hw(hh, ww)
            return oh * ow if (N > 1 and plan_like_single) else 0

        x = self.stem(x4, N, H, W, relu=True, plan_rows=pr(self.stem, H, W), **mk)
        h, w = self.stem.out_hw(H, W)
        stem_out, hs, ws = x, h, w
        x, h, w = ops.maxpool3x3s2(x, N, h, w, 64)
        if keep is not None:
            keep["stem"] = (stem_out, hs, ws, x, h, w)
            keep["blocks"] = []
        feats = {}
        cur_layer = 1
        for (li, c1, c2, c3, ds) in self.blocks:
            if li != cur_layer:
                feats[f"layer{cur_layer + 1}"] = (x, h, w)
                cur_layer = li
            sc = x
            if ds is not None:
                sc = ds(x, N, h, w, plan_rows=pr(ds, h, w), **mk)
            o = c1(x, N, h, w, relu=True, plan_rows=pr(c1, h, w), **mk)
            o1 = o
            o = c2(o, N, h, w, relu=True, plan_rows=pr(c2, h, w), **mk)
            h2, w2 = c2.out_hw(h, w)
            x_in = x
            x = c3(o, N, h2, w2, res=sc, res_mode=1, relu=True, plan_rows=pr(c3, h2, w2), **mk)
            if keep is not None:
                keep["blocks"].append((x_in, o1, o, x, h, w, h2, w2))
            h, w = h2, w2
        feats[f"layer{cur_layer + 1}"] = (x, h, w)
        return feats


class CustomRecurrentFPN:
    size_divisibility = 32

    def __init__(self, cfg, sd: Dict[str, torch.Tensor], device):
        self.device = device
        self.memory_type = cfg.MODEL.MEMORY_TYPE
        self.feat_fusion = cfg.MODEL.MAP_FEAT_FUSION
        self.map_feature_weight = float(cfg.MODEL.MAP_FEATURE_WEIGHT)
        if self.memory_type == "implicit_memory" and self.feat_fusion not in ("sum", "mem_only", "image_only"):
            raise ValueError(f"MODEL.MAP_FEAT_FUSION={self.feat_fusion!r} not supported (timm.py:181-186)")
        self.bottom_up = ResNet50Trunk(sd, device)
        self.lateral, self.output = {}, {}
        for l in (3, 4, 5):
            self.lateral[l] = ops.Conv(sd[f"backbone.fpn_lateral{l}.weight"], sd[f"backbone.fpn_lateral{l}.bias"], device=device,
                                       name=f"fpn_lateral{l}")
            self.output[l] = ops.Conv(sd[f"backbone.fpn_output{l}.weight"], sd[f"backbone.fpn_output{l}.bias"], pad=1, device=device,
                                      name=f"fpn_output{l}")
        self.p6 = ops.Conv(sd["backbone.top_block.p6.weight"], sd["backbone.top_block.p6.bias"], stride=2, pad=1, device=device, name="p6")
        self.p7 = ops.Conv(sd["backbone.top_block.p7.weight"], sd["backbone.top_block.p7.bias"], stride=2, pad=1, device=device, name="p7")
        self.merge = ops.MemoryProjector([sd[f"backbone.map_merge_projection{i}.weight"] for i in (1, 2, 3)],
                                         [sd[f"backbone.map_merge_projection{i}.bias"] for i in (1, 2, 3)], device)
        self._plans = {}
        self.pool_in_torch_order = True

    def level_shapes(self, H: int, W: int) -> List[Tuple[int, int]]:
        hw = [(H // 8, W // 8), (H // 16, W // 16), (H // 32, W // 32)]
        h6, w6 = self.p6.out_hw(*hw[2])
        h7, w7 = self.p7.out_hw(h6, w6)
        return hw + [(h6, w6), (h7, w7)]

    def _plan(self, H: int, W: int, which: int = 0):
        key = (H, W, which)
        if key not in self._plans:
            shapes = self.level_shapes(H, W)
            off = [0]
            for (h, w) in shapes:
                off.append(off[-1] + h * w)
            feats = torch.empty((off[-1], 256), dtype=torch.float32, device=self.device)
            views = [feats[off[i]:off[i + 1]].view(1, shapes[i][0], shapes[i][1], 256) for i in range(5)]
            pooled = torch.empty((ops.pooled_rows(H, W), 512), dtype=torch.float16, device=self.device)
            self._plans[key] = (shapes, off, feats, views, pooled)
        return self._plans[key]

    def top_down(self, c: dict, H: int, W: int, which: int = 0):
        shapes, off, feats, views, pooled = self._plan(H, W, which)
        (c5, h5, w5), (c4, h4, w4), (c3, h3, w3) = c["layer5"], c["layer4"], c["layer3"]
        assert (h3, w3) == shapes[0] and (h5, w5) == shapes[2]
        lat5 = self.lateral[5](c5, 1, h5, w5)
        self.output[5](lat5, 1, h5, w5, out=views[2])
        lat4 = self.lateral[4](c4, 1, h4, w4, res=lat5, res_mode=2)
        self.output[4](lat4, 1, h4, w4, out=views[1])
        lat3 = self.lateral[3](c3, 1, h3, w3, res=lat4, res_mode=2)
        self.output[3](lat3, 1, h3, w3, out=views[0])

    def top_down_batched(self, c: dict, H: int, W: int, N: int):
        (c5, h5, w5), (c4, h4, w4), (c3, h3, w3) = c["layer5"], c["layer4"], c["layer3"]
        lat5 = self.lateral[5](c5, N, h5, w5, plan_rows=h5 * w5)
        p5 = self.output[5](lat5, N, h5, w5, plan_rows=h5 * w5)
        lat4 = self.lateral[4](c4, N, h4, w4, res=lat5, res_mode=2, plan_rows=h4 * w4)
        p4 = self.output[4](lat4, N, h4, w4, plan_rows=h4 * w4)
        lat3 = self.lateral[3](c3, N, h3, w3, res=lat4, res_mode=2, plan_rows=h3 * w3)
        p3 = self.output[3](lat3, N, h3, w3, plan_rows=h3 * w3)
        return [p3, p4, p5]

    def fuse_memory_and_top(self, H: int, W: int, memory_f16: Optional[torch.Tensor], proj: Optional[torch.Tensor], which: int = 0,
                            err: Optional[torch.Tensor] = None):
        shapes, off, feats, views, pooled = self._plan(H, W, which)
        h5, w5 = shapes[2]
        if self.memory_type == "implicit_memory" and self.feat_fusion != "image_only":
            if memory_f16 is None or proj is None:
                raise ValueError("implicit_memory needs the fp16 memory table and proj_indices")
            ops.memory_gather_pool(memory_f16, proj, H, W, out=pooled, err=err, torch_order=self.pool_in_torch_order)
            self.merge(pooled, feats, H, W, self.map_feature_weight, self.feat_fusion)
        self.p6(views[2], 1, h5, w5, out=views[3])
        self.p7(views[3], 1, shapes[3][0], shapes[3][1], in_relu=True, out=views[4])
        return feats, views, shapes, off

    def forward(self, x4: torch.Tensor, H: int, W: int, memory_f16: Optional[torch.Tensor], proj: Optional[torch.Tensor],
                which: int = 0, err: Optional[torch.Tensor] = None):
        self.top_down(self.bottom_up.forward(x4, H, W), H, W, which)
        return self.fuse_memory_and_top(H, W, memory_f16, proj, which, err)


@BACKBONE_REGISTRY.register()
def build_p67_timm_fpn_backbone_recurrent(cfg, sd, device):
    if cfg.MODEL.TIMM.BASE_NAME != "resnet50_in21k_map":
        raise ValueError("MODEL.TIMM.BASE_NAME must be 'resnet50_in21k_map' for the recurrent path")
    return CustomRecurrentFPN(cfg, sd, device)
```

embodied_object_detection_amd/modeling/batched.py:

```python
from __future__ import annotations

from typing import Dict, List, Optional

import torch

from .. import ops
from .meta_arch import PYRAMID_SETS, CustomRCNNRecurrent


def _share_weights(dst: CustomRCNNRecurrent, src: CustomRCNNRecurrent):
    def convs(m: CustomRCNNRecurrent):
        out = [m.backbone.bottom_up.stem]
        for (_li, c1, c2, c3, ds) in m.backbone.bottom_up.blocks:
            out += [c1, c2, c3] + ([ds] if ds is not None else [])
        for l in (3, 4, 5):
            out += [m.backbone.lateral[l], m.backbone.output[l]]
        out += [m.backbone.p6, m.backbone.p7]
        out += [t[0] for t in m.proposal_generator.tower] + [m.proposal_generator.out_conv]
        for st in m.roi_heads.stages:
            out += [st["fc1"], st["fc2"], st["cls"], st["bb0"], st["bb2"]]
        out += list(m.roi_heads.mask_convs) + [m.roi_heads.deconv]
        return out

    for a, b in zip(convs(dst), convs(src)):
        a.w, a.bias, a.w_split, a.w_half = b.w, b.bias, b.w_split, b.w_half
    dst.backbone.merge.prepared = src.backbone.merge.prepared
    for a, b in zip(dst.proposal_generator.tower, src.proposal_generator.tower):
        pass
    for sa, sb in zip(dst.roi_heads.stages, src.roi_heads.stages):
        sa["zs"] = sb["zs"]
    dst.roi_heads.pred_w = src.roi_heads.pred_w
    dst.zs_weight = src.zs_weight


class BatchedSequences:

    def __init__(self, cfg, batch: int, state_dict: Optional[Dict[str, torch.Tensor]] = None, concurrent_scenes: int = 0):
        if batch < 1:
            raise ValueError("batch must be >= 1")
        self.concurrent_scenes = int(concurrent_scenes)
        self.scenes: List[CustomRCNNRecurrent] = [CustomRCNNRecurrent(cfg, state_dict) for _ in range(batch)]
        for m in self.scenes[1:]:
            _share_weights(m, self.scenes[0])
        torch.cuda.empty_cache()
        self.device = self.scenes[0].device
        self._stream_pool = [torch.cuda.Stream(device=self.device, priority=-1) for _ in range(batch)]
        self.streams = list(self._stream_pool)
        self.trunk_stream = torch.cuda.Stream(device=self.device, priority=-1)
        self._ev_in = torch.cuda.Event()
        self._ev_trunk = torch.cuda.Event()
        self._ev_done = [[torch.cuda.Event(), torch.cuda.Event()] for _ in range(batch)]
        for m in self.scenes:
            m.prefetch_trunk = False
        self.intra_scene_overlap = False
        self.trunk_lookahead = True
        self.stagger = True
        for m in self.scenes:
            m.front_event = torch.cuda.Event()

    def __call__(self, episodes: List[List[dict]]):
        return self.forward(episodes)

    def _batched_trunk(self, scenes: List[CustomRCNNRecurrent], frames: List[dict]):
        m0 = self.scenes[0]
        B = len(frames)
        H, W = int(frames[0]["image"].shape[-2]), int(frames[0]["image"].shape[-1])
        if any((int(f["image"].shape[-2]), int(f["image"].shape[-1])) != (H, W) for f in frames):
            raise ValueError("the frames of one lock-step must have one size")
        xs = []
        for m, f in zip(scenes, frames):
            x4, Hp, Wp = ops.preprocess_image(m._device_image(f), m.pixel_mean, m.pixel_std)
            xs.append(x4)
        x = torch.cat(xs, dim=0)
        c = m0.backbone.bottom_up.forward(x, Hp, Wp, N=B)
        p345 = m0.backbone.top_down_batched(c, Hp, Wp, B)
        for b, (m, f) in enumerate(zip(scenes, frames)):
            nxt = (m._pyramid + 1) % PYRAMID_SETS
            shapes, off, feats, views, pooled = m.backbone._plan(Hp, Wp, nxt)
            for l in range(3):
                views[l].copy_(p345[l][b:b + 1])
            m._prefetched = (f["image"], Hp, Wp)
        return Hp, Wp

    def forward(self, episodes: List[Optional[List[dict]]]):
        B = len(self.scenes)
        if len(episodes) != B:
            raise ValueError(f"need {B} episodes (None for a sequence that sits this call out)")
        episodes = [e if e else [] for e in episodes]
        T = max(len(e) for e in episodes)
        first = next((e[0] for e in episodes if e), None)
        if first is not None:
            n_conc = self.concurrent_scenes if self.concurrent_scenes > 0 else 2
            self.streams = [self._stream_pool[b % max(1, min(n_conc, B))] for b in range(B)]
        outs: List[List[dict]] = [[] for _ in range(B)]
        pending: List[List] = [[] for _ in range(B)]
        cur = torch.cuda.current_stream(self.device)
        ts = self.trunk_stream if self.trunk_lookahead else cur
        active = lambda t: [b for b in range(B) if t < len(episodes[b])]

        def enqueue_trunk(t: int):
            act = active(t)
            for b in act:
                m = self.scenes[b]
                if t >= (2 if self.trunk_lookahead else 1):
                    ts.wait_event(self._ev_done[b][t % 2 if self.trunk_lookahead else (t - 1) % 2])
                rd = m._pyr_reader.get((m._pyramid + 1) % PYRAMID_SETS)
                if rd is not None:
                    ts.wait_event(rd)
            with torch.cuda.stream(ts):
                self._batched_trunk([self.scenes[b] for b in act], [episodes[b][t] for b in act])
                self._ev_trunk.record(ts)

        self._ev_in.record(cur)
        if self.trunk_lookahead:
            ts.wait_event(self._ev_in)
        if T:
            enqueue_trunk(0)
        for t in range(T):
            for b in active(t):
                m, f, s = self.scenes[b], episodes[b][t], self.streams[b]
                s.wait_event(self._ev_trunk)
                if t == 0:
                    s.wait_event(self._ev_in)
                    prev = [a for a in active(0) if a < b]
                    if self.stagger and prev:
                        s.wait_event(self.scenes[prev[-1]].front_event)
                with torch.cuda.stream(s):
                    if f["memory_reset"]:
                        m.reset_memory(int(episodes[b][0]["memory"].shape[0]))
                    if m.implicit_memory is None:
                        raise RuntimeError("first frame of a scene must carry memory_reset=True")
                    refresh = m.test_type in ("default", "episodic") or (m.test_type == "longterm" and t == 0)
                    m._ev_trunk = self._ev_trunk
                    m.overlap_branches = self.intra_scene_overlap
                    m.inference_frame(f, refresh_memory_snapshot=refresh, materialize=False)
                    pending[b].append(m._post_ticket())
                    self._ev_done[b][t % 2].record(s)
            if t + 1 < T:
                enqueue_trunk(t + 1)
            for b, m in enumerate(self.scenes):
                if len(pending[b]) == 3:
                    with torch.cuda.stream(self.streams[b]):
                        outs[b].append({"instances": m._materialize(pending[b].pop(0))})
        for b, m in enumerate(self.scenes):
            with torch.cuda.stream(self.streams[b]):
                for ticket in pending[b]:
                    outs[b].append({"instances": m._materialize(ticket)})
            if episodes[b]:
                cur.wait_event(self._ev_done[b][(len(episodes[b]) - 1) % 2])
        torch.cuda.current_stream(self.device).synchronize()
        return outs
```

embodied_object_detection_amd/modeling/meta_arch.py:

```python
from __future__ import annotations

from typing import Dict, List, Optional, Tuple

import time as _time

import numpy as np
import torch

from .. import _lib, ops
from ..checkpoint import fill_missing, load_checkpoint, load_zs_weight, reset_cls_test, synthetic_state_dict
from ..registry import BACKBONE_REGISTRY, META_ARCH_REGISTRY, PROPOSAL_GENERATOR_REGISTRY, ROI_HEADS_REGISTRY
from ..structures import Boxes, Instances
from .utils import query_classifier


_SCHED_STREAMS: Dict[int, Tuple[torch.cuda.Stream, ...]] = {}
RESULT_SETS = 3
PYRAMID_SETS = 6


def _sched_streams(device: torch.device) -> Tuple[torch.cuda.Stream, ...]:
    idx = device.index if device.index is not None else torch.cuda.current_device()
    if idx not in _SCHED_STREAMS:
        _SCHED_STREAMS[idx] = tuple(torch.cuda.Stream(device=device, priority=-1) for _ in range(4))
    return _SCHED_STREAMS[idx]


_DET_STREAMS: Dict[int, torch.cuda.Stream] = {}


def _det_stream(device: torch.device) -> torch.cuda.Stream:
    idx = device.index if device.index is not None else torch.cuda.current_device()
    if idx not in _DET_STREAMS:
        _DET_STREAMS[idx] = torch.cuda.Stream(device=device, priority=0)
    return _DET_STREAMS[idx]


def _query_matrix(model, mem, classifier, num_classes):
    if mem is None:
        raise _lib.EodError("semantic_map: no memory yet (no frame has run)")
    if classifier is None:
        return model.zs_weight
    return query_classifier(classifier, num_classes, bool(getattr(model.roi_heads, "norm_weight", True)), model.device)


def _semmap_query(model, mem, obs, classifier, num_classes, thresh):
    zs = _query_matrix(model, mem, classifier, num_classes)
    return ops.semmap_query(mem, obs, zs, model.obs_score_thresh if thresh is None else float(thresh))


def _semmap_locate(model, mem, obs, classes, classifier, num_classes, thresh, map_shape, radius, topk):
    zs = _query_matrix(model, mem, classifier, num_classes)
    cols = None
    if map_shape is not None:
        rows, cols = int(map_shape[0]), int(map_shape[1])
        if rows * cols != mem.shape[0]:
            raise _lib.EodError(f"locate: map_shape {tuple(map_shape)} does not hold the memory's {mem.shape[0]} cells")
    return ops.semmap_locate(mem, obs, zs, classes, model.obs_score_thresh if thresh is None else float(thresh), cols=cols,
                             radius=radius, topk=topk)


@META_ARCH_REGISTRY.register()
class CustomRCNNRecurrent:
    def __init__(self, cfg, state_dict: Optional[Dict[str, torch.Tensor]] = None):
        dev = str(cfg.MODEL.DEVICE)
        if not dev.startswith("cuda"):
            raise _lib.EodError(
                f"MODEL.DEVICE={dev!r}: the product path is HIP-only (no CPU fallback). The CPU restatement lives in "
                "oracle/ and is test infrastructure.")
        if not torch.cuda.is_available():
            raise _lib.EodError("no GPU visible: the HIP product path cannot run")
        _lib.load()
        self.cfg = cfg
        self.device = torch.device(dev if ":" in dev else "cuda:0")
        torch.cuda.set_device(self.device)
        self.map_conditioned = cfg.MODEL.TIMM.BASE_NAME == "resnet50_in21k_map"
        self.memory_type = cfg.MODEL.MEMORY_TYPE
        self.save_semmap = bool(cfg.MODEL.TEST_SAVE_SEMMAP)
        self.output_dir = cfg.OUTPUT_DIR
        self.cls_score_thresh = float(cfg.MODEL.MEMORY_CLS_SCORE_THRESH)
        self.obs_score_thresh = float(cfg.MODEL.MEMORY_OBS_SCORE_THRESH)
        self.test_type = cfg.MODEL.TEST_TYPE
        if self.test_type not in ("default", "episodic", "longterm"):
            raise ValueError(f"MODEL.TEST_TYPE={self.test_type!r}")
        self.pixel_mean = [float(v) for v in cfg.MODEL.PIXEL_MEAN]
        self.pixel_std = [float(v) for v in cfg.MODEL.PIXEL_STD]
        self.mask_threshold = 0.5
        self.training = False
        self.lazy_proposal_masks = True
        self.dedup_detection_masks = True
        self.overlap_branches = True
        self._side_stream = None
        self._ev_props = self._ev_pm = self._ev_box = self._ev_mem = self._ev_sel = None
        self.prefetch_trunk = True
        self._ev_start = None
        self._trunk_stream = None
        self._ev_trunk = None
        self._prefetched = None
        self._pyramid = 0
        self.lookahead_frames = 2
        self.lookahead_depth: Optional[int] = 3
        self._ahead: List[dict] = []
        self.front_event: Optional[torch.cuda.Event] = None
        self.detection_pass_after = "cascade"
        self._det_stream = None
        self._ev_call = None
        self._ev_det = [None] * RESULT_SETS
        self._pyr_reader = {}
        self._frame_no = 0

        num_classes = int(cfg.MODEL.ROI_HEADS.NUM_CLASSES)
        if state_dict is None:
            if cfg.MODEL.WEIGHTS and str(cfg.MODEL.WEIGHTS).endswith((".pth", ".pkl")) and __import__("os").path.exists(cfg.MODEL.WEIGHTS):
                sd, _ = load_checkpoint(cfg.MODEL.WEIGHTS, num_classes)
                state_dict = fill_missing(sd, 0, num_classes, cfg.MODEL.ROI_BOX_HEAD.ZEROSHOT_WEIGHT_PATH)
            else:
                state_dict = synthetic_state_dict(0, num_classes, cfg.MODEL.ROI_BOX_HEAD.ZEROSHOT_WEIGHT_PATH)
        if cfg.MODEL.RESET_CLS_TESTS and cfg.MODEL.TEST_CLASSIFIERS:
            import os
            p = cfg.MODEL.TEST_CLASSIFIERS[0]
            if not os.path.exists(p):
                p = cfg.MODEL.ROI_BOX_HEAD.ZEROSHOT_WEIGHT_PATH
            state_dict = dict(state_dict)
            reset_cls_test(state_dict, p, int(cfg.MODEL.TEST_NUM_CLASSES[0]))
        self.state_dict_ref = state_dict
        self.zs_weight = load_zs_weight(cfg.MODEL.ROI_BOX_HEAD.ZEROSHOT_WEIGHT_PATH).contiguous().to(self.device)
        self.C1 = self.zs_weight.shape[1]

        self.backbone = BACKBONE_REGISTRY.get(cfg.MODEL.BACKBONE.NAME)(cfg, state_dict, self.device)
        self.proposal_generator = PROPOSAL_GENERATOR_REGISTRY.get(cfg.MODEL.PROPOSAL_GENERATOR.NAME)(cfg, state_dict, self.device)
        self.roi_heads = ROI_HEADS_REGISTRY.get(cfg.MODEL.ROI_HEADS.NAME)(cfg, state_dict, self.device, self.proposal_generator.cap)
        R = self.proposal_generator.cap
        self.mem_scores = torch.zeros((R, self.C1), dtype=torch.float32, device=self.device)
        self.mem_selector = ops.DetectionSelector(R, self.C1, 100, self.device, unique=True)
        self._uniq_rows, self._uniq_count = self.mem_selector.uniq_rows, self.mem_selector.uniq_count
        self._mem_scores_frame = -1
        self.implicit_memory: Optional[torch.Tensor] = None
        self.observations: Optional[torch.Tensor] = None
        self.semmap = None
        self._mem_f16: Optional[torch.Tensor] = None
        self._dirty: Optional[torch.Tensor] = None
        self._f16_valid = False
        self._dirty_pending = False
        self.snapshot_follows_write: Optional[bool] = None
        self._err = torch.zeros((1,), dtype=torch.int32, device=self.device)
        self._writer = None
        self._writer_key = None
        self._post = None
        self._posts = None
        self._post_slot = 0
        self.last_stats: Dict[str, torch.Tensor] = {}
        self.stats_log = None
        self.trace = None
        self.host_profile = {"frames": 0, "enqueue_s": 0.0, "materialize_s": 0.0, "wait_s": 0.0}

    def eval(self):
        self.training = False
        return self

    def train(self, mode: bool = True):
        self.training = bool(mode)
        return self

    def to(self, *_a, **_k):
        return self

    def __call__(self, batched_inputs):
        return self.forward(batched_inputs)

    def reset_memory(self, n_cells: int):
        if self.implicit_memory is None or self.implicit_memory.shape[0] != n_cells:
            self.implicit_memory = torch.empty((n_cells, 512), dtype=torch.float32, device=self.device)
            self.observations = torch.empty((n_cells,), dtype=torch.float32, device=self.device)
            self._mem_f16 = torch.empty((n_cells, 512), dtype=torch.float16, device=self.device)
            self._dirty = torch.empty((n_cells,), dtype=torch.int32, device=self.device)
        lib = _lib.load()
        s = torch.cuda.current_stream().cuda_stream
        _lib.check(lib.eod_fill_f32(self.implicit_memory.data_ptr(), 0.0, self.implicit_memory.numel(), s), "fill")
        _lib.check(lib.eod_fill_f32(self.observations.data_ptr(), 0.0, self.observations.numel(), s), "fill")
        _lib.check(lib.eod_fill_i32(self._mem_f16.data_ptr(), 0, self._mem_f16.numel() // 2, s), "fill")
        _lib.check(lib.eod_fill_i32(self._dirty.data_ptr(), 0, n_cells, s), "fill")
        self._f16_valid = True
        self._dirty_pending = False
        self.semmap = None

    def invalidate_memory_snapshot(self):
        self._f16_valid = False

    def _refresh_memory_snapshot(self):
        if self._f16_valid:
            if self._dirty_pending:
                ops.memory_normalize_dirty_f16(self.implicit_memory, self.observations, self._dirty, self._mem_f16)
        else:
            ops.memory_normalize_f16(self.implicit_memory, self.observations, out=self._mem_f16)
            _lib.check(_lib.load().eod_fill_i32(self._dirty.data_ptr(), 0, self._dirty.numel(), torch.cuda.current_stream().cuda_stream), "fill")
            self._f16_valid = True
        self._dirty_pending = False

    def _ensure_frame_buffers(self, H: int, W: int, n_cells: int):
        key = (H, W, n_cells)
        if self._writer_key != key:
            self._writer = ops.MemoryWriter(H, W, n_cells, 100, self.proposal_generator.cap, self.device, mask_thresh=0.5)
            self._writer_key = key
        if self._posts is None or self._posts[0]["hw"] != (H, W):
            D = self.roi_heads.topk
            dev = self.device
            self._posts = [dict(
                hw=(H, W), boxes=None, scores=None, classes=None, masks=None,
                src=torch.zeros((D,), dtype=torch.int32, device=dev), count=torch.zeros((1,), dtype=torch.int32, device=dev),
                count_host=torch.zeros((1,), dtype=torch.int32).pin_memory(), err_host=torch.zeros((1,), dtype=torch.int32).pin_memory(),
                ready=torch.cuda.Event(), err_ready=torch.cuda.Event()) for _ in range(RESULT_SETS)]
            self._post_slot = 0
        self._post = self._posts[self._post_slot]

    def forward(self, batched_inputs: List[List[dict]]):
        if self.training:
            if getattr(self, "trainer", None) is None:
                raise RuntimeError("training mode needs a trainer: `modeling.training.Trainer(model, state_dict)` attaches itself to the "
                                   "model; then `model.train(); losses = model(data); trainer.optimizer_step()`")
            return self.trainer.forward_backward_frames(batched_inputs)
        if self.overlap_branches:
            caller = torch.cuda.current_stream(self.device)
            ms = _sched_streams(self.device)[2]
            if self._ev_call is None:
                self._ev_call = (torch.cuda.Event(), torch.cuda.Event())
            self._ev_call[0].record(caller)
            ms.wait_event(self._ev_call[0])
            with torch.cuda.stream(ms):
                out = self._forward_frames(batched_inputs)
                self._ev_call[1].record(ms)
            caller.wait_event(self._ev_call[1])
            return out
        return self._forward_frames(batched_inputs)

    def _forward_frames(self, batched_inputs: List[List[dict]]):
        batch_output = []
        pending = []
        for input_seq in batched_inputs:
            for i, frame in enumerate(input_seq):
                n_cells = int(input_seq[0]["memory"].shape[0])
                if frame["memory_reset"]:
                    self.reset_memory(n_cells)
                if self.implicit_memory is None:
                    raise RuntimeError("first frame of a scene must carry memory_reset=True (custom_rcnn.py:485 reads unset state)")
                refresh = self.test_type in ("default", "episodic") or (self.test_type == "longterm" and i == 0)
                nxt = input_seq[i + 1:i + 1 + PYRAMID_SETS] or None
                last = nxt is None and input_seq is batched_inputs[-1]
                t0 = _time.perf_counter()
                self.inference_frame(frame, refresh_memory_snapshot=refresh, materialize=False, next_frame=nxt,
                                     trailing_detection_pass=not last)
                pending.append(self._post_ticket())
                t1 = _time.perf_counter()
                if len(pending) == RESULT_SETS:
                    batch_output.append({"instances": self._materialize(pending.pop(0))})
                hp = self.host_profile
                hp["frames"] += 1
                hp["enqueue_s"] += t1 - t0
                hp["materialize_s"] += _time.perf_counter() - t1
                if self.save_semmap and i == 0:
                    self.save_memory_snapshot(frame["sequence_name"])
        for ticket in pending:
            batch_output.append({"instances": self._materialize(ticket)})
        return batch_output

    def _post_ticket(self):
        P = self._post
        cur = torch.cuda.current_stream(self.device)
        P["err_host"].copy_(self._err, non_blocking=True)
        k = self._post_slot
        if self.overlap_branches:
            ds = self._det_stream
            ds.wait_event(self._ev_det[k])
            P["err_ready"].record(cur)
            ds.wait_event(P["err_ready"])
            with torch.cuda.stream(ds):
                P["count_host"].copy_(P["count"], non_blocking=True)
                P["ready"].record(ds)
        else:
            P["count_host"].copy_(P["count"], non_blocking=True)
            P["ready"].record(cur)
        self._post_slot = (self._post_slot + 1) % RESULT_SETS
        return P

    def _device_image(self, frame) -> torch.Tensor:
        img = frame["image"]
        if not torch.is_tensor(img):
            img = torch.as_tensor(np.asarray(img))
        if img.dtype != torch.uint8:
            img = img.to(torch.uint8)
        return img.to(self.device, non_blocking=True).contiguous()

    def _device_proj(self, frame) -> torch.Tensor:
        p = frame["proj_indices"]
        if not torch.is_tensor(p):
            p = torch.from_numpy(np.ascontiguousarray(p))
        if p.dim() == 3:
            p = p.squeeze(2)
        if p.dtype != torch.int32:
            p = p.to(torch.int32)
        return p.to(self.device, non_blocking=True).contiguous()

    def _enqueue_trunk(self, frames: List[dict], after: torch.cuda.Event, first: int = 0):
        if self._trunk_stream is None:
            self._trunk_stream = _sched_streams(self.device)[1]
            self._ev_trunk = torch.cuda.Event()
        ts = self._trunk_stream
        ts.wait_event(after)
        done = torch.cuda.Event()
        sets = [(self._pyramid + 1 + first + b) % PYRAMID_SETS for b in range(len(frames))]
        for st in sets:
            if st in self._pyr_reader:
                ts.wait_event(self._pyr_reader[st])
        with torch.cuda.stream(ts):
            self._mark("trunk_lookahead_begin", ts)
            xs = []
            for f in frames:
                x4, Hp, Wp = ops.preprocess_image(self._device_image(f), self.pixel_mean, self.pixel_std)
                xs.append(x4)
            if len(frames) == 1:
                self.backbone.top_down(self.backbone.bottom_up.forward(xs[0], Hp, Wp), Hp, Wp, sets[0])
            else:
                n = len(frames)
                c = self.backbone.bottom_up.forward(torch.cat(xs, dim=0), Hp, Wp, N=n)
                p345 = self.backbone.top_down_batched(c, Hp, Wp, n)
                for b, st in enumerate(sets):
                    views = self.backbone._plan(Hp, Wp, st)[3]
                    for l in range(3):
                        views[l].copy_(p345[l][b:b + 1])
            done.record(ts)
            self._mark("trunk_lookahead", ts)
        self._ahead = self._ahead + [dict(image=f["image"], Hp=Hp, Wp=Wp, event=done) for f in frames]

    def inference_frame(self, frame: dict, refresh_memory_snapshot: bool = True, materialize: bool = True,
                        next_frame=None, trailing_detection_pass: bool = False):
        H, W = int(frame["image"].shape[-2]), int(frame["image"].shape[-1])
        if H % 32 or W % 32:
            raise ValueError("H and W must be multiples of 32 (proj_indices is not padded: SURVEY §8 notation)")
        proj = self._device_proj(frame)
        if tuple(proj.shape) != (H, W):
            raise ValueError(f"proj_indices shape {tuple(proj.shape)} != image {(H, W)}")
        n_cells = self.implicit_memory.shape[0]
        self._ensure_frame_buffers(H, W, n_cells)
        self._frame_no += 1
        self._mark("start")

        mem_f16 = None
        if self.memory_type == "implicit_memory":
            if refresh_memory_snapshot:
                self._refresh_memory_snapshot()
            mem_f16 = self._mem_f16

        coming = [] if next_frame is None else (list(next_frame) if isinstance(next_frame, (list, tuple)) else [next_frame])
        pre, start_batch, first_ahead = self._claim_lookahead(frame, coming)
        if start_batch:
            if self._ev_start is None:
                self._ev_start = torch.cuda.Event()
            self._ev_start.record(torch.cuda.current_stream(self.device))
        views, shapes, props = self._front(frame, pre, proj, mem_f16)
        if start_batch:
            self._enqueue_trunk(start_batch, self._ev_start, first_ahead)
        if self.roi_heads.fuses_mem_rescore(self.zs_weight):
            self._mem_scores_frame = self._frame_no
        if self.overlap_branches:
            self._frame_pipelined(frame, (H, W), views, shapes, props, proj, trailing_detection_pass)
        else:
            self._frame_in_order(frame, (H, W), views, shapes, props, proj)

        P = self._post
        self.last_stats = {"prop_count": props[2], "det_count": P["count"], "mem_k": self._writer.k_out,
                           "det_mask_rois": self.roi_heads.last_selector.rep_count if self.dedup_detection_masks else P["count"]}
        if self.stats_log is not None:
            if self.overlap_branches and trailing_detection_pass:
                with torch.cuda.stream(self._det_stream):
                    cnt = P["count"].clone()
            else:
                cnt = P["count"].clone()
            self.stats_log.append((props[2].clone(), cnt, self._writer.k_out.clone(), self._uniq_count.clone(),
                                   self.last_stats["det_mask_rois"].clone()))
        if not materialize:
            return None
        return {"instances": self._materialize(self._post_ticket())}

    def _claim_lookahead(self, frame: dict, coming: List[dict]):
        cur = torch.cuda.current_stream(self.device)
        ext, self._prefetched = self._prefetched, None
        if isinstance(ext, tuple):
            self._ahead = [dict(image=ext[0], Hp=ext[1], Wp=ext[2], event=self._ev_trunk)]
        ahead = self._ahead
        hit = bool(ahead) and ahead[0]["image"] is frame["image"]
        if ahead and not hit:
            for e in ahead:
                cur.wait_event(e["event"])
            ahead = []
        pre = None
        if hit:
            pre = ahead.pop(0)
            cur.wait_event(pre["event"])
        self._pyramid = (self._pyramid + 1) % PYRAMID_SETS
        if not hit and self._pyramid in self._pyr_reader:
            cur.wait_event(self._pyr_reader[self._pyramid])
        keep = 0
        while keep < len(ahead) and keep < len(coming) and ahead[keep]["image"] is coming[keep]["image"]:
            keep += 1
        for e in ahead[keep:]:
            cur.wait_event(e["event"])
        self._ahead = ahead = ahead[:keep]
        depth = max(1, int(self.lookahead_frames)) if self.lookahead_depth is None else max(1, int(self.lookahead_depth))
        batch = []
        if self.prefetch_trunk and self.overlap_branches and len(ahead) < min(depth, PYRAMID_SETS - 2):
            room = PYRAMID_SETS - 2 - len(ahead)
            batch = coming[len(ahead):len(ahead) + min(max(1, int(self.lookahead_frames)), room)]
            n_same = 0
            for f in batch:
                if tuple(f["image"].shape) != tuple(batch[0]["image"].shape):
                    break
                n_same += 1
            batch = batch[:n_same]
        return pre, batch, len(ahead)

    def _front(self, frame: dict, pre: Optional[dict], proj, mem_f16):
        if pre is not None:
            feats, views, shapes, off = self.backbone.fuse_memory_and_top(pre["Hp"], pre["Wp"], mem_f16, proj, self._pyramid, self._err)
        else:
            x4, Hp, Wp = ops.preprocess_image(self._device_image(frame), self.pixel_mean, self.pixel_std)
            feats, views, shapes, off = self.backbone.forward(x4, Hp, Wp, mem_f16, proj, self._pyramid, self._err)
        return views, shapes, self.proposal_generator.forward(feats, shapes, off)

    def _frame_in_order(self, frame: dict, image_hw, views, shapes, props, proj):
        H, W = image_hw
        prop_boxes, prop_scores, prop_count = props
        det = self.roi_heads.forward_box(views, shapes, prop_boxes, prop_scores, prop_count, (H, W),
                                         mem_rescore=(self.zs_weight, self.mem_scores))
        det_boxes, det_scores, det_classes, det_rows, det_count = det
        if self.front_event is not None:
            self.front_event.record(torch.cuda.current_stream(self.device))
        self._detection_masks(views, shapes, det_boxes, det_count)
        mem_sel = None
        if self.lazy_proposal_masks:
            mem_sel = self.select_memory_instances(prop_boxes, prop_scores, prop_count, (H, W))
            prop_masks = self.roi_heads.forward_mask_memory(views, shapes, prop_boxes, prop_count, rows=self._uniq_rows,
                                                            rows_count=self._uniq_count, tag=("prop", self._frame_no))
        else:
            prop_masks = self.roi_heads.forward_mask_memory(views, shapes, prop_boxes, prop_count, tag=("prop_all", self._frame_no))
        self._postprocess_and_paste(det_boxes, det_scores, det_classes, det_count, (H, W), frame, self._post)
        self.update_implicit_memory(prop_boxes, prop_scores, prop_count, prop_masks, proj, (H, W), mem_sel)

    def _frame_pipelined(self, frame: dict, image_hw, views, shapes, props, proj, trailing_detection_pass: bool):
        H, W = image_hw
        prop_boxes, prop_scores, prop_count = props
        main = torch.cuda.current_stream(self.device)
        if self._side_stream is None:
            self._side_stream = _sched_streams(self.device)[0]
            self._ev_props, self._ev_pm, self._ev_box, self._ev_mem, self._ev_sel = (torch.cuda.Event() for _ in range(5))
        side = self._side_stream
        self._ev_props.record(main)
        self._mark("proposals", main)
        lazy = self.lazy_proposal_masks
        if not lazy:
            prop_masks = self.roi_heads.forward_mask_memory(views, shapes, prop_boxes, prop_count,
                                                            bufs=self.roi_heads.proposal_pass_buffers(), tag=("prop_all", self._frame_no))
            self._ev_pm.record(main)
        mem_sel = None

        def select_memory():
            nonlocal mem_sel
            mem_sel = self.select_memory_instances(prop_boxes, prop_scores, prop_count, (H, W))
            self._ev_sel.record(side)
            self._mark("mem_select", side)

        side.wait_event(self._ev_props)
        with torch.cuda.stream(side):
            k = self._post_slot
            if self._ev_det[k] is not None:
                side.wait_event(self._ev_det[k])
            det = self.roi_heads.forward_box(views, shapes, prop_boxes, prop_scores, prop_count, (H, W), sel=k,
                                             mem_rescore=(self.zs_weight, self.mem_scores),
                                             after_cascade=select_memory if lazy else None)
            self._ev_box.record(side)
            self._mark("cascade+det_select", side)
        det_after = self.detection_pass_after if lazy else "cascade"
        if det_after == "cascade":
            self._enqueue_detection_pass(views, shapes, det, (H, W), frame)
        if lazy:
            main.wait_event(self._ev_sel)
            prop_masks = self.roi_heads.forward_mask_memory(views, shapes, prop_boxes, prop_count, rows=self._uniq_rows,
                                                            rows_count=self._uniq_count,
                                                            bufs=self.roi_heads.proposal_pass_buffers(), tag=("prop", self._frame_no))
            self._ev_pm.record(main)
            self._mark("prop_masks", main)
        if det_after == "proposal_masks":
            self._enqueue_detection_pass(views, shapes, det, (H, W), frame, after=self._ev_pm)
        with torch.cuda.stream(side):
            if not lazy:
                mem_sel = self.select_memory_instances(prop_boxes, prop_scores, prop_count, (H, W))
            side.wait_event(self._ev_pm)
            self.update_implicit_memory(prop_boxes, prop_scores, prop_count, prop_masks, proj, (H, W), mem_sel)
            self._ev_mem.record(side)
            self._mark("mem_write", side)
        if det_after == "memory_write":
            self._enqueue_detection_pass(views, shapes, det, (H, W), frame, after=self._ev_mem)
        main.wait_event(self._ev_mem)
        if not trailing_detection_pass:
            main.wait_event(self._ev_det[self._post_slot])

    def _mark(self, name: str, stream=None):
        if self.trace is None:
            return
        ev = torch.cuda.Event(enable_timing=True)
        ev.record(stream if stream is not None else torch.cuda.current_stream(self.device))
        self.trace.append((self._frame_no, name, ev))

    def _detection_masks(self, views, shapes, det_boxes, det_count):
        rh = self.roi_heads
        sel = rh.last_selector
        if self.dedup_detection_masks:
            return rh.forward_mask(views, shapes, det_boxes, sel.rep_count, rh.topk, rh.det_masks, rows=sel.rep_list,
                                   lds_reserve=rh.det_pass_lds_reserve, tag=("det", self._frame_no))
        return rh.forward_mask(views, shapes, det_boxes, det_count, rh.topk, rh.det_masks, lds_reserve=rh.det_pass_lds_reserve,
                               tag=("det", self._frame_no))

    def _postprocess_and_paste(self, det_boxes, det_scores, det_classes, det_count, image_hw, frame, P):
        H, W = image_hw
        out_h, out_w = int(frame.get("height", H)), int(frame.get("width", W))
        if (out_h, out_w) != (H, W):
            raise NotImplementedError("output size != input size is not used on this path (train_mp3d.py:487-490)")
        D, dev = self.roi_heads.topk, self.device
        P["boxes"] = torch.empty((D, 4), dtype=torch.float32, device=dev)
        P["scores"] = torch.empty((D,), dtype=torch.float32, device=dev)
        P["classes"] = torch.empty((D,), dtype=torch.int32, device=dev)
        P["masks"] = torch.empty((D, H, W), dtype=torch.uint8, device=dev)
        ops.detector_postprocess(det_boxes, det_scores, det_classes, det_count, self.roi_heads.topk, out_w / W, out_h / H,
                                 float(out_w), float(out_h), P["boxes"], P["scores"], P["classes"], P["src"], P["count"],
                                 remap=self.roi_heads.last_selector.rep_of if self.dedup_detection_masks else None)
        ops.paste_masks(self.roi_heads.det_masks, P["boxes"], P["src"], P["count"], self.roi_heads.topk, out_h, out_w,
                        self.mask_threshold, P["masks"])

    def _enqueue_detection_pass(self, views, shapes, det, image_hw, frame, after=None):
        if self._det_stream is None:
            self._det_stream = _det_stream(self.device)
            self._ev_det = [torch.cuda.Event() for _ in range(RESULT_SETS)]
        ds = self._det_stream
        det_boxes, det_scores, det_classes, det_rows, det_count = det
        k = self._post_slot
        ds.wait_event(self._ev_box)
        if after is not None:
            ds.wait_event(after)
        with torch.cuda.stream(ds):
            self._mark("det_pass_begin", ds)
            self._detection_masks(views, shapes, det_boxes, det_count)
            self._postprocess_and_paste(det_boxes, det_scores, det_classes, det_count, image_hw, frame, self._post)
            self._ev_det[k].record(ds)
            self._mark("det_pass", ds)
        self._pyr_reader[self._pyramid] = self._ev_det[k]

    def select_memory_instances(self, prop_boxes, prop_scores, prop_count, image_hw):
        H, W = image_hw
        R = self.proposal_generator.cap
        if self._mem_scores_frame != self._frame_no:
            ops.memory_scores(self.roi_heads.featn0, self.zs_weight, prop_scores, self.mem_scores, prop_count, R, self.C1)
        _, _, _, rows, cnt = self.mem_selector(prop_boxes, self.mem_scores, prop_count, float(W), float(H), self.cls_score_thresh, 0.5)
        return rows, cnt

    def update_implicit_memory(self, prop_boxes, prop_scores, prop_count, prop_masks, proj, image_hw, mem_sel=None):
        rows, cnt = mem_sel if mem_sel is not None else self.select_memory_instances(prop_boxes, prop_scores, prop_count, image_hw)
        self._last_write = (prop_boxes, prop_masks, rows, cnt, proj)
        follow = self.snapshot_follows_write if self.snapshot_follows_write is not None else self.test_type in ("default", "episodic")
        if follow and self._f16_valid and not self._dirty_pending:
            self._writer(self.roi_heads.featn0, prop_boxes, prop_masks, rows, cnt, proj, self.implicit_memory, self.observations,
                         err=self._err, snapshot=self._mem_f16)
        else:
            self._writer(self.roi_heads.featn0, prop_boxes, prop_masks, rows, cnt, proj, self.implicit_memory, self.observations,
                         dirty=self._dirty, err=self._err)
            self._dirty_pending = True

    def save_memory_snapshot(self, sequence_name: str) -> str:
        from ..data.snapshot import write_snapshot
        semmap = self.semantic_map()
        return write_snapshot(self.output_dir, sequence_name, semmap.cpu().numpy(), self.implicit_memory.cpu().numpy(),
                              self.observations.cpu().numpy())

    def _materialize(self, P) -> Instances:
        t0 = _time.perf_counter()
        P["ready"].synchronize()
        self.host_profile["wait_s"] += _time.perf_counter() - t0
        flags = int(P["err_host"][0])
        if flags:
            self._err.zero_()
            raise _lib.EodError(
                f"device error flags {flags:#x}: proj_indices holds cell indices outside [0, {self.implicit_memory.shape[0]}) "
                "(an index image written for another map size?); they were clamped, the frame's results are not trustworthy")
        n = int(P["count_host"][0])
        inst = Instances(P["hw"])
        cur = torch.cuda.current_stream(self.device)
        for k in ("boxes", "scores", "classes", "masks"):
            P[k].record_stream(cur)
        inst.pred_boxes = Boxes(P["boxes"][:n])
        inst.scores = P["scores"][:n]
        inst.pred_classes = P["classes"][:n].to(torch.int64)
        inst.pred_masks = P["masks"][:n].view(torch.bool)
        P["boxes"] = P["scores"] = P["classes"] = P["masks"] = None
        return inst

    def semantic_map(self, classifier=None, num_classes: Optional[int] = None, thresh: Optional[float] = None, scores: bool = False):
        if classifier is None and not scores:
            self.semmap = ops.semmap_labels(self.implicit_memory, self.observations, self.zs_weight,
                                            self.obs_score_thresh if thresh is None else float(thresh))
            return self.semmap
        return _semmap_query(self, self.implicit_memory, self.observations, classifier, num_classes, thresh)

    def locate(self, classes, classifier=None, num_classes: Optional[int] = None, thresh: Optional[float] = None, map_shape=None,
               radius: int = 1, topk: int = 8):
        return _semmap_locate(self, self.implicit_memory, self.observations, classes, classifier, num_classes, thresh, map_shape,
                              radius, topk)

    def proposals_snapshot(self):
        dec = self.proposal_generator._plans[next(iter(self.proposal_generator._plans))][3]
        n = int(dec.count.item())
        return dict(proposal_boxes=dec.boxes[:n].cpu(), scores=dec.scores[:n].cpu(),
                    feat=self.roi_heads.feat0.view(-1, 512)[:n].cpu(), featn=self.roi_heads.featn0[:n].cpu(),
                    pred_masks=self.roi_heads.prop_masks[:n].cpu())
```

embodied_object_detection_amd/ops.py:

```python
from __future__ import annotations

import ctypes as C
from typing import Dict, Optional, Sequence, Tuple

import numpy as np
import torch

from . import _lib
from ._lib import EodConvDesc, EodDetDesc, EodMemWriteDesc, EodProposalDesc, check


_raw_stream = getattr(torch._C, "_cuda_getCurrentRawStream", None)


def _stream() -> int:
    if _raw_stream is not None:
        return _raw_stream(torch.cuda.current_device())
    return torch.cuda.current_stream().cuda_stream


def _ptr(t: Optional[torch.Tensor]) -> Optional[int]:
    return None if t is None else t.data_ptr()


def _need_cuda(*ts):
    for t in ts:
        if t is not None and not t.is_cuda:
            raise _lib.EodError("HIP product path needs device tensors (no CPU fallback)")


class Workspace:

    def __init__(self):
        self.bufs = {}

    def get(self, nbytes: int, device) -> torch.Tensor:
        key = (device.index if isinstance(device, torch.device) else str(device), _stream())
        buf = self.bufs.get(key)
        if buf is None or buf.numel() < nbytes:
            buf = torch.empty(max(int(nbytes), 1 << 20), dtype=torch.uint8, device=device)
            self.bufs[key] = buf
        return buf


_conv_ws = Workspace()


_CONV_MATH = {"fp32": 0, "bf16x3": 1, "f16": 2}
WGRAD_F16 = 512


def set_conv_math(mode: str) -> str:
    if mode not in _CONV_MATH:
        hint = ""
        if str(mode).lower() == "fp16":
            hint = (' ("fp16" / FP16 is the config key of autocast training: modeling.training.build_trainer / AmpTrainer, which choose '
                    'the arithmetic per launch; the process-wide inference arithmetic is "f16")')
        raise ValueError(f"conv math must be one of {sorted(_CONV_MATH)}, got {mode!r}{hint}")
    prev = _lib.load().eod_set_conv_math(_CONV_MATH[mode])
    check(min(prev, 0), "eod_set_conv_math")
    return {v: k for k, v in _CONV_MATH.items()}[prev]


def get_conv_math() -> str:
    return {v: k for k, v in _CONV_MATH.items()}[_lib.load().eod_get_conv_math()]


def fold_bn(w: torch.Tensor, bn_w, bn_b, bn_mean, bn_var, eps: float = 1e-5):
    scale = bn_w / torch.sqrt(bn_var + eps)
    return w * scale.view(-1, 1, 1, 1), bn_b - bn_mean * scale


def pack_conv_weight(w_oihw: torch.Tensor, cin_pad: Optional[int] = None) -> Tuple[torch.Tensor, int]:
    O, I, KH, KW = w_oihw.shape
    w = w_oihw.permute(0, 2, 3, 1).contiguous()
    if cin_pad is not None and cin_pad != I:
        wp = torch.zeros((O, KH, KW, cin_pad), dtype=w.dtype)
        wp[..., :I] = w
        w = wp
    K = w.shape[1] * w.shape[2] * w.shape[3]
    Kpad = (K + 31) // 32 * 32
    out = torch.zeros((O, Kpad), dtype=torch.float32)
    out[:, :K] = w.reshape(O, K)
    return out.contiguous(), Kpad


class Conv:

    def __init__(self, w_oihw: torch.Tensor, bias: Optional[torch.Tensor], stride: int = 1, pad: int = 0,
                 device="cuda", cin_pad: Optional[int] = None, deconv: bool = False, name: str = ""):
        self.name = name
        if deconv:
            Cin, Cout, kh, kw = w_oihw.shape
            assert kh == 2 and kw == 2
            w = w_oihw.permute(2, 3, 1, 0).reshape(4 * Cout, Cin, 1, 1).contiguous()
            self.out_mode = 1
            self.KH = self.KW = 1
            self.stride, self.pad = 1, 0
            self.Cin, self.Cout = Cin, 4 * Cout
        else:
            w = w_oihw
            self.out_mode = 0
            self.Cout, cin, self.KH, self.KW = w.shape
            self.Cin = cin_pad or cin
            self.stride, self.pad = stride, pad
        packed, self.Kpad = pack_conv_weight(w, cin_pad)
        self.tap4 = 1 if self.Cin == 4 else 0
        if not self.tap4 and self.Cin % 32 != 0:
            raise ValueError(f"{name}: Cin={self.Cin} must be a multiple of 32 (or 4 for the stem)")
        self.w = packed.to(device)
        self.bias = None if bias is None else bias.detach().to(torch.float32).contiguous().to(device)
        self.desc = EodConvDesc()
        self._lib = _lib.load()
        self.w_split = None
        self.w_half = None
        self.event_log = None
        self.event_tag = None
        self.lds_reserve = 0
        self.prefetch2 = 0

    def out_hw(self, H: int, W: int) -> Tuple[int, int]:
        return ((H + 2 * self.pad - self.KH) // self.stride + 1, (W + 2 * self.pad - self.KW) // self.stride + 1)

    def __call__(self, x: torch.Tensor, N: int, H: int, W: int, *, res: Optional[torch.Tensor] = None, res_mode: int = 0,
                 relu: bool = False, in_relu: bool = False, out_scale: float = 1.0, m_count: Optional[torch.Tensor] = None,
                 m_unit: int = 0, out: Optional[torch.Tensor] = None, force_tile: int = 0, force_splitk: int = 0,
                 levels: Optional[Tuple[Sequence[int], Sequence[Tuple[int, int]]]] = None,
                 fuse: Optional[Tuple[torch.Tensor, float, Optional[torch.Tensor]]] = None, presplit: bool = True,
                 plan_rows: int = 0, gn_stats: Optional[torch.Tensor] = None, gn_groups: int = 32,
                 split: Optional[Tuple[int, torch.Tensor]] = None, m_segments: int = 0,
                 gate: Optional[torch.Tensor] = None, math: Optional[str] = None) -> torch.Tensor:
        _need_cuda(x, res, out, gate)
        if fuse is not None:
            if self.out_mode != 1 or out is None:
                raise ValueError("fuse= needs a deconv layer and an explicit probability buffer `out`")
            _need_cuda(fuse[0], fuse[2])
        OH, OW = self.out_hw(H, W) if levels is None else (0, 0)
        if levels is not None and out is None:
            out = torch.empty((levels[0][-1], self.Cout), dtype=torch.float32, device=x.device)
        if out is None:
            if self.out_mode == 1:
                out = torch.empty((N, 2 * OH, 2 * OW, self.Cout // 4), dtype=torch.float32, device=x.device)
            else:
                out = torch.empty((N, OH, OW, self.Cout), dtype=torch.float32, device=x.device)
        d = self.desc
        d.x, d.w, d.bias, d.res, d.y = x.data_ptr(), self.w.data_ptr(), _ptr(self.bias), _ptr(res), out.data_ptr()
        d.m_count, d.m_unit, d.m_segments = _ptr(m_count), m_unit, int(m_segments)
        d.gate = _ptr(gate)
        if math is not None and math not in _CONV_MATH:
            raise ValueError(f"math={math!r}: one of {sorted(_CONV_MATH)} or None")
        d.math = 0 if math is None else _CONV_MATH[math] + 1
        d.N, d.H, d.W, d.Cin, d.OH, d.OW, d.Cout = N, H, W, self.Cin, OH, OW, self.Cout
        d.KH, d.KW, d.stride, d.pad, d.Kpad = self.KH, self.KW, self.stride, self.pad, self.Kpad
        d.relu, d.res_mode, d.in_relu, d.out_mode, d.tap4 = int(relu), res_mode, int(in_relu), self.out_mode, self.tap4
        if fuse is not None:
            d.out_mode, d.fuse_w, d.fuse_b, d.out_units = 2, fuse[0].data_ptr(), float(fuse[1]), _ptr(fuse[2])
        else:
            d.fuse_w, d.fuse_b, d.out_units = None, 0.0, None
        d.force_tile, d.force_splitk, d.out_scale = force_tile, force_splitk, out_scale
        d.plan_rows = plan_rows
        d.lds_reserve = self.lds_reserve
        d.prefetch2 = self.prefetch2
        d.gn_partial, d.gn_groups = None, 0
        self.gn_fused = False
        if split is not None:
            _need_cuda(split[1])
            d.split_n, d.y2 = int(split[0]), split[1].data_ptr()
        else:
            d.split_n, d.y2 = 0, None
        if levels is not None:
            off, shapes = levels
            d.levels = len(shapes)
            for i, o in enumerate(off):
                d.level_off[i] = o
            for i, (h, w) in enumerate(shapes):
                d.level_h[i], d.level_w[i] = h, w
        else:
            d.levels = 0
        mode = math if math is not None else get_conv_math()
        use_split = force_tile // 10 == 5 if force_tile else (mode == "bf16x3")
        if use_split and self.w_split is None and not self.tap4:
            nb = self._lib.eod_conv_split_weights_bytes(self.Cout, self.Kpad)
            self.w_split = torch.empty((nb,), dtype=torch.uint8, device=self.w.device)
            check(self._lib.eod_conv_split_weights_bf16x3(self.w.data_ptr(), self.Cout, self.Kpad, self.w_split.data_ptr(), _stream()),
                  f"eod_conv_split_weights_bf16x3[{self.name}]")
        d.w_split = self.w_split.data_ptr() if (use_split and self.w_split is not None and presplit) else None
        use_half = force_tile // 10 in (8, 9) if force_tile else (mode == "f16")
        if use_half and self.w_half is None and not self.tap4:
            nb = self._lib.eod_conv_half_weights_bytes(self.Cout, self.Kpad)
            self.w_half = torch.empty((nb,), dtype=torch.uint8, device=self.w.device)
            check(self._lib.eod_conv_half_weights(self.w.data_ptr(), self.Cout, self.Kpad, self.w_half.data_ptr(), _stream()),
                  f"eod_conv_half_weights[{self.name}]")
            if not torch.cuda.is_current_stream_capturing():
                torch.cuda.current_stream(self.w.device).synchronize()
        d.w_half = self.w_half.data_ptr() if (use_half and self.w_half is not None and presplit) else None
        if gn_stats is not None and levels is not None and self._lib.eod_conv2d_gn_fused(C.byref(d)):
            d.gn_partial = gn_stats.data_ptr() + self._lib.eod_groupnorm_partial_offset(len(levels[1]), gn_groups)
            d.gn_groups = gn_groups
            self.gn_fused = True
        d.workspace, d.workspace_bytes = None, 0
        need = self._lib.eod_conv2d_workspace_bytes(C.byref(d))
        if need:
            ws = _conv_ws.get(need, x.device)
            d.workspace, d.workspace_bytes = ws.data_ptr(), ws.numel()
        if self.event_log is not None:
            e0, e1 = torch.cuda.Event(enable_timing=True), torch.cuda.Event(enable_timing=True)
            e0.record()
            check(self._lib.eod_conv2d(C.byref(d), _stream()), f"eod_conv2d[{self.name}]")
            e1.record()
            self.event_log.append((e0, e1, self.event_tag))
            return out
        check(self._lib.eod_conv2d(C.byref(d), _stream()), f"eod_conv2d[{self.name}]")
        return out

    def plan(self) -> Dict[str, int]:
        p = _lib.EodConvPlan()
        check(self._lib.eod_conv2d_plan(C.byref(self.desc), C.byref(p)), f"eod_conv2d_plan[{self.name}]")
        return {n: int(getattr(p, n)) for n, _t in p._fields_}


def preprocess_image(img_u8_chw: torch.Tensor, mean: Sequence[float], std: Sequence[float], div: int = 32,
                     out: Optional[torch.Tensor] = None) -> Tuple[torch.Tensor, int, int]:
    _need_cuda(img_u8_chw)
    assert img_u8_chw.dtype == torch.uint8 and img_u8_chw.dim() == 3 and img_u8_chw.is_contiguous()
    _, H, W = img_u8_chw.shape
    Hp, Wp = (H + div - 1) // div * div, (W + div - 1) // div * div
    if out is None:
        out = torch.empty((1, Hp, Wp, 4), dtype=torch.float32, device=img_u8_chw.device)
    assert out.numel() == Hp * Wp * 4 and out.is_contiguous()
    m = (C.c_float * 3)(*mean)
    s = (C.c_float * 3)(*std)
    check(_lib.load().eod_preprocess_image(img_u8_chw.data_ptr(), out.data_ptr(), H, W, Hp, Wp, m, s, _stream()),
          "eod_preprocess_image")
    return out, Hp, Wp


def maxpool3x3s2(x: torch.Tensor, N: int, H: int, W: int, Cc: int) -> Tuple[torch.Tensor, int, int]:
    OH, OW = (H + 2 - 3) // 2 + 1, (W + 2 - 3) // 2 + 1
    y = torch.empty((N, OH, OW, Cc), dtype=torch.float32, device=x.device)
    check(_lib.load().eod_maxpool3x3s2(x.data_ptr(), y.data_ptr(), N, H, W, Cc, OH, OW, _stream()), "eod_maxpool3x3s2")
    return y, OH, OW


def groupnorm_workspace(level_off: Sequence[int], device, groups: int = 32) -> torch.Tensor:
    lo = (C.c_int32 * len(level_off))(*level_off)
    n = _lib.load().eod_groupnorm_workspace_bytes(lo, len(level_off) - 1, groups)
    return torch.empty(((n + 7) // 8,), dtype=torch.float64, device=device)


def groupnorm_relu(x: torch.Tensor, gamma: torch.Tensor, beta: torch.Tensor, level_off: Sequence[int], Cc: int,
                   stats: torch.Tensor, groups: int = 32, eps: float = 1e-5, out: Optional[torch.Tensor] = None,
                   partial_ready: bool = False) -> torch.Tensor:
    if out is None:
        out = torch.empty_like(x)
    lo = (C.c_int32 * len(level_off))(*level_off)
    check(_lib.load().eod_groupnorm_relu(x.data_ptr(), out.data_ptr(), gamma.data_ptr(), beta.data_ptr(), lo, len(level_off) - 1,
                                         Cc, groups, eps, stats.data_ptr(), int(partial_ready), _stream()), "eod_groupnorm_relu")
    return out


def groupnorm_relu_backward(x: torch.Tensor, y: torch.Tensor, dy: torch.Tensor, gamma: torch.Tensor, level_off: Sequence[int], Cc: int,
                            fwd_stats: torch.Tensor, groups: int = 32, eps: float = 1e-5):
    _need_cuda(x, y, dy, gamma, fwd_stats)
    lo = (C.c_int32 * len(level_off))(*level_off)
    lib = _lib.load()
    ws = torch.empty((lib.eod_groupnorm_backward_workspace_bytes(lo, len(level_off) - 1, Cc) // 8,), dtype=torch.float64, device=x.device)
    dx = torch.empty_like(x)
    dgamma = torch.empty((Cc,), dtype=torch.float32, device=x.device)
    dbeta = torch.empty((Cc,), dtype=torch.float32, device=x.device)
    check(lib.eod_groupnorm_relu_backward(x.data_ptr(), y.data_ptr(), dy.data_ptr(), gamma.data_ptr(), lo, len(level_off) - 1, Cc, groups, eps,
                                          fwd_stats.data_ptr(), ws.data_ptr(), dx.data_ptr(), dgamma.data_ptr(), dbeta.data_ptr(), _stream()),
          "eod_groupnorm_relu_backward")
    return dx, dgamma, dbeta


def mask_predictor_sigmoid(x: torch.Tensor, w: torch.Tensor, bias: float, rows: int, Cc: int, count: Optional[torch.Tensor],
                           unit_rows: int, out: Optional[torch.Tensor] = None, out_units: Optional[torch.Tensor] = None) -> torch.Tensor:
    if out is None:
        out = torch.empty((rows,), dtype=torch.float32, device=x.device)
    check(_lib.load().eod_mask_predictor_sigmoid(x.data_ptr(), w.data_ptr(), bias, out.data_ptr(), rows, Cc, _ptr(count),
                                                 unit_rows, _ptr(out_units), _stream()), "eod_mask_predictor_sigmoid")
    return out


def roi_align(p3, p4, p5, h3: int, w3: int, Cc: int, boxes: torch.Tensor, count: Optional[torch.Tensor], R_cap: int, S: int,
              out: Optional[torch.Tensor] = None, box_rows: Optional[torch.Tensor] = None, batch: int = 1,
              boxes_per_image: int = 0, refine=None) -> torch.Tensor:
    if out is None:
        out = torch.empty((R_cap, S, S, Cc), dtype=torch.float32, device=p3.device)
    ref = None
    if refine is not None:
        deltas, ld, (wx, wy, ww, wh), clip, img_w, img_h, boxes_out = refine
        _need_cuda(deltas, boxes_out)
        ref = _lib.EodBoxRefine(deltas.data_ptr(), ld, wx, wy, ww, wh, int(clip), img_w, img_h, boxes_out.data_ptr())
    check(_lib.load().eod_roi_align(p3.data_ptr(), p4.data_ptr(), p5.data_ptr(), h3, w3, Cc, boxes.data_ptr(), _ptr(box_rows),
                                    _ptr(count), R_cap, S, out.data_ptr(), batch, boxes_per_image, None if ref is None else C.byref(ref),
                                    _stream()), "eod_roi_align")
    return out


def roi_align_backward(dp3, dp4, dp5, h3: int, w3: int, Cc: int, boxes: torch.Tensor, count: Optional[torch.Tensor], R_cap: int, S: int,
                       g: torch.Tensor):
    _need_cuda(dp3, dp4, dp5, boxes, g)
    assert g.is_contiguous() and tuple(g.shape) == (R_cap, S, S, Cc)
    check(_lib.load().eod_roi_align_backward(dp3.data_ptr(), dp4.data_ptr(), dp5.data_ptr(), h3, w3, Cc, boxes.data_ptr(), _ptr(count),
                                             R_cap, S, g.data_ptr(), _stream()), "eod_roi_align_backward")


def concat_lists(lists: torch.Tensor, counts: torch.Tensor, cap_in: int, id_stride: int, batch: int, out: torch.Tensor,
                 out_count: torch.Tensor):
    check(_lib.load().eod_concat_lists(lists.data_ptr(), counts.data_ptr(), cap_in, id_stride, batch, out.data_ptr(), out_count.data_ptr(),
                                       _stream()), "eod_concat_lists")
    return out, out_count


def unique_rows(rows: torch.Tensor, count: torch.Tensor, K_cap: int, R_cap: int, out_rows: torch.Tensor, out_count: torch.Tensor):
    check(_lib.load().eod_unique_rows(rows.data_ptr(), count.data_ptr(), K_cap, R_cap, out_rows.data_ptr(), out_count.data_ptr(),
                                      _stream()), "eod_unique_rows")


class ProposalDecoder:

    def __init__(self, level_hw: Sequence[Tuple[int, int]], strides: Sequence[int], scales: Sequence[float], score_thresh: float,
                 pre_nms_topk: int, post_nms_topk: int, nms_thresh: float, cap: int, device, head_stride: int = 5, batch: int = 1):
        self.lib = _lib.load()
        d = EodProposalDesc()
        off = [0]
        for (h, w) in level_hw:
            off.append(off[-1] + h * w)
        d.levels = len(level_hw)
        for i, o in enumerate(off):
            d.level_off[i] = o
        for i, (h, w) in enumerate(level_hw):
            d.level_w[i] = w
            d.level_stride[i] = strides[i]
            d.level_scale[i] = scales[i]
        d.head_stride = head_stride
        d.score_thresh, d.pre_nms_topk, d.post_nms_topk, d.nms_thresh, d.cap = score_thresh, pre_nms_topk, post_nms_topk, nms_thresh, cap
        nbytes = self.lib.eod_proposals_workspace_bytes(off[-1], d.levels, pre_nms_topk, batch)
        d.batch = batch
        self.ws = torch.empty((nbytes,), dtype=torch.uint8, device=device)
        self.boxes = torch.zeros((batch * cap, 4), dtype=torch.float32, device=device)
        self.scores = torch.zeros((batch * cap,), dtype=torch.float32, device=device)
        self.count = torch.zeros((batch,), dtype=torch.int32, device=device)
        d.out_boxes, d.out_scores, d.out_count = self.boxes.data_ptr(), self.scores.data_ptr(), self.count.data_ptr()
        d.workspace, d.workspace_bytes = self.ws.data_ptr(), nbytes
        self.desc = d
        self.total = off[-1]
        self.level_off = off

    def __call__(self, head_out: torch.Tensor):
        self.desc.head_out = head_out.data_ptr()
        check(self.lib.eod_centernet_proposals(C.byref(self.desc), _stream()), "eod_centernet_proposals")
        return self.boxes, self.scores, self.count


class DetectionSelector:

    def __init__(self, R_cap: int, C1: int, topk: int, device, unique: bool = False, groups: bool = False, batch: int = 1):
        self.lib = _lib.load()
        self.R_cap, self.C1, self.topk, self.batch = R_cap, C1, topk, batch
        nbytes = self.lib.eod_detections_workspace_bytes(R_cap, C1)
        if nbytes == 0:
            raise _lib.EodError(f"eod_fast_rcnn_inference: {R_cap} rows x {C1 - 1} classes are not supported (at most 512 rows, 2047 classes)")
        self.ws = torch.zeros((nbytes,), dtype=torch.uint8, device=device)
        B = batch
        self.boxes = torch.zeros((B * topk, 4), dtype=torch.float32, device=device)
        self.scores = torch.zeros((B * topk,), dtype=torch.float32, device=device)
        self.classes = torch.zeros((B * topk,), dtype=torch.int32, device=device)
        self.rows = torch.zeros((B * topk,), dtype=torch.int32, device=device)
        self.count = torch.zeros((B,), dtype=torch.int32, device=device)
        d = EodDetDesc()
        d.R_cap, d.C1, d.topk, d.batch = R_cap, C1, topk, batch
        d.out_boxes, d.out_scores, d.out_classes = self.boxes.data_ptr(), self.scores.data_ptr(), self.classes.data_ptr()
        d.out_rows, d.out_count = self.rows.data_ptr(), self.count.data_ptr()
        d.workspace, d.workspace_bytes = self.ws.data_ptr(), nbytes
        self.uniq_rows = self.uniq_count = None
        if unique:
            self.uniq_rows = torch.zeros((B * R_cap,), dtype=torch.int32, device=device)
            self.uniq_count = torch.zeros((B,), dtype=torch.int32, device=device)
            d.out_unique_rows, d.out_unique_count, d.unique_cap = self.uniq_rows.data_ptr(), self.uniq_count.data_ptr(), R_cap
        self.rep_of = self.rep_list = self.rep_count = None
        if groups:
            self.rep_of = torch.zeros((B * topk,), dtype=torch.int32, device=device)
            self.rep_list = torch.zeros((B * topk,), dtype=torch.int32, device=device)
            self.rep_count = torch.zeros((B,), dtype=torch.int32, device=device)
            d.out_rep_of, d.out_rep_list, d.out_rep_count = self.rep_of.data_ptr(), self.rep_list.data_ptr(), self.rep_count.data_ptr()
        self.desc = d

    def __call__(self, boxes: torch.Tensor, scores: torch.Tensor, count: Optional[torch.Tensor], img_w: float, img_h: float,
                 score_thresh: float, nms_thresh: float):
        d = self.desc
        d.boxes, d.scores, d.count = boxes.data_ptr(), scores.data_ptr(), _ptr(count)
        d.img_w, d.img_h, d.score_thresh, d.nms_thresh = img_w, img_h, score_thresh, nms_thresh
        check(self.lib.eod_fast_rcnn_inference(C.byref(d), _stream()), "eod_fast_rcnn_inference")
        return self.boxes, self.scores, self.classes, self.rows, self.count


ZS_WIDE = 2
ZS_MAX_C1 = 24
ZS_WIDE_MAX_C1 = 2048


def _zs_refusal(name: str, C1: int, wide: bool) -> str:
    if wide:
        return (f"{name}: {C1 - 1} classes + background exceed the wide classifier kernel's {ZS_WIDE_MAX_C1} columns "
                f"(at most {ZS_WIDE_MAX_C1 - 1} classes on the HIP path)")
    return (f"{name}: {C1 - 1} classes + background do not fit the narrow kernel's LDS-staged class matrix (at most {ZS_MAX_C1 - 1} "
            f"classes); pass wide=True for a RESET_CLS_TESTS / TEST_NUM_CLASSES vocabulary of up to {ZS_WIDE_MAX_C1 - 1} classes")


def zs_classify(feat, zs, prob_acc, accumulate: bool, featn_out, count, R_cap: int, C1: int, temp: float = 50.0, zs_mem=None,
                prop_scores=None, mem_scores_out=None, final_inv_stages: float = 0.0, batch: int = 1, wide: bool = False):
    st = _lib.load().eod_zs_classify(feat.data_ptr(), zs.data_ptr(), prob_acc.data_ptr(), int(bool(accumulate)) | (ZS_WIDE if wide else 0),
                                     _ptr(featn_out), _ptr(count), R_cap, 512, C1, temp, _ptr(zs_mem), _ptr(prop_scores),
                                     _ptr(mem_scores_out), float(final_inv_stages), batch, _stream())
    if st == -5:
        raise _lib.EodError(_zs_refusal("eod_zs_classify", C1, wide))
    check(st, "eod_zs_classify")


def cascade_stage_tail(feat, zs, prob_acc, accumulate: bool, featn_out, count, R_cap: int, C1: int, temp: float, hb, bb2: "Conv", boxes_in,
                       boxes_out, weights, clip: bool, img_w: float, img_h: float, zs_mem=None, prop_scores=None, mem_scores_out=None,
                       final_inv_stages: float = 0.0, deltas_out=None, batch: int = 1, wide: bool = False):
    d = _lib.EodStageTailDesc()
    d.feat, d.zs, d.prob_acc, d.feat_norm_out, d.count = feat.data_ptr(), zs.data_ptr(), prob_acc.data_ptr(), _ptr(featn_out), _ptr(count)
    d.accumulate = int(bool(accumulate)) | (ZS_WIDE if wide else 0)
    d.R_cap, d.D, d.C1, d.temp = R_cap, 512, C1, temp
    d.zs_mem, d.prop_scores, d.mem_scores_out, d.final_inv_stages, d.batch = _ptr(zs_mem), _ptr(prop_scores), _ptr(mem_scores_out), float(final_inv_stages), batch
    d.hb, d.w2, d.b2, d.hb_dim, d.w2_ld = hb.data_ptr(), bb2.w.data_ptr(), bb2.bias.data_ptr(), bb2.Cin, bb2.Kpad
    d.boxes_in, d.boxes_out, d.deltas_out = boxes_in.data_ptr(), boxes_out.data_ptr(), _ptr(deltas_out)
    d.wx, d.wy, d.ww, d.wh = weights
    d.clip, d.img_w, d.img_h = int(clip), img_w, img_h
    st = _lib.load().eod_cascade_stage_tail(C.byref(d), _stream())
    if st == -5:
        raise _lib.EodError(_zs_refusal("eod_cascade_stage_tail", C1, wide))
    check(st, "eod_cascade_stage_tail")


def apply_deltas(deltas, ld: int, boxes, out, count, R_cap: int, weights, clip: bool, img_w: float, img_h: float, batch: int = 1):
    wx, wy, ww, wh = weights
    check(_lib.load().eod_apply_deltas(deltas.data_ptr(), ld, boxes.data_ptr(), out.data_ptr(), _ptr(count), R_cap, wx, wy, ww, wh,
                                       int(clip), img_w, img_h, batch, _stream()), "eod_apply_deltas")


def cascade_scores(prob_acc, prop_scores, count, R_cap: int, C1: int, inv_stages: float):
    check(_lib.load().eod_cascade_scores(prob_acc.data_ptr(), prop_scores.data_ptr(), _ptr(count), R_cap, C1, inv_stages, _stream()),
          "eod_cascade_scores")


def memory_scores(featn, zs, prop_scores, scores_out, count, R_cap: int, C1: int):
    check(_lib.load().eod_memory_scores(featn.data_ptr(), zs.data_ptr(), prop_scores.data_ptr(), scores_out.data_ptr(), _ptr(count),
                                        R_cap, 512, C1, _stream()), "eod_memory_scores")


def detector_postprocess(boxes, scores, classes, count, cap: int, sx: float, sy: float, out_w: float, out_h: float, ob, os_, oc, osrc,
                         ocount, remap=None, batch: int = 1):
    check(_lib.load().eod_detector_postprocess(boxes.data_ptr(), scores.data_ptr(), classes.data_ptr(), _ptr(count), cap, sx, sy,
                                               out_w, out_h, ob.data_ptr(), os_.data_ptr(), oc.data_ptr(), osrc.data_ptr(),
                                               ocount.data_ptr(), _ptr(remap), batch, _stream()), "eod_detector_postprocess")


def paste_masks(prob, boxes, rows, count, K_cap: int, H: int, W: int, thr: float, out: torch.Tensor, batch: int = 1,
                prob_units: int = 0):
    check(_lib.load().eod_paste_masks(prob.data_ptr(), boxes.data_ptr(), _ptr(rows), _ptr(count), K_cap, H, W, thr, out.data_ptr(),
                                      batch, prob_units, _stream()), "eod_paste_masks")
    return out


def unproject_grid_index(depth: torch.Tensor, T: np.ndarray, intr, proj_shift, map_shift, cell: float, map_w: int, map_h: int,
                         order: int = 0, want_xyz: bool = False):
    _need_cuda(depth)
    H, W = depth.shape
    idx = torch.empty((H, W), dtype=torch.int32, device=depth.device)
    xyz = torch.empty((H, W, 3), dtype=torch.float32, device=depth.device) if want_xyz else None
    T16 = (C.c_float * 16)(*np.asarray(T, dtype=np.float32).reshape(-1).tolist())
    ps = (C.c_float * 3)(*np.asarray(proj_shift, dtype=np.float32).tolist())
    ms = (C.c_float * 3)(*np.asarray(map_shift, dtype=np.float32).tolist())
    fx, fy, cx, cy = [float(np.float32(v)) for v in intr]
    check(_lib.load().eod_unproject_grid_index(depth.data_ptr(), H, W, T16, fx, fy, cx, cy, ps, ms, float(np.float32(cell)), map_w,
                                               map_h, order, _ptr(xyz), idx.data_ptr(), _stream()), "eod_unproject_grid_index")
    return (idx, xyz) if want_xyz else idx


def memory_normalize_f16(mem: torch.Tensor, obs: torch.Tensor, out: Optional[torch.Tensor] = None) -> torch.Tensor:
    N, D = mem.shape
    if out is None:
        out = torch.empty((N, D), dtype=torch.float16, device=mem.device)
    check(_lib.load().eod_memory_normalize_f16(mem.data_ptr(), obs.data_ptr(), out.data_ptr(), N, D, _stream()),
          "eod_memory_normalize_f16")
    return out


def memory_normalize_dirty_f16(mem: torch.Tensor, obs: torch.Tensor, dirty: torch.Tensor, out: torch.Tensor) -> torch.Tensor:
    N, D = mem.shape
    check(_lib.load().eod_memory_normalize_dirty_f16(mem.data_ptr(), obs.data_ptr(), dirty.data_ptr(), out.data_ptr(), N, D, _stream()),
          "eod_memory_normalize_dirty_f16")
    return out


def pooled_rows(H: int, W: int) -> int:
    return int(_lib.load().eod_memory_pooled_halves(H, W)) // 512


def memory_gather_pool(mem_f16: torch.Tensor, proj: torch.Tensor, H: int, W: int, out: Optional[torch.Tensor] = None,
                       err: Optional[torch.Tensor] = None, torch_order: bool = False, batch: int = 1) -> torch.Tensor:
    N, D = mem_f16.shape[-2:]
    if out is None:
        out = torch.empty((batch * pooled_rows(H, W), D), dtype=torch.float16, device=mem_f16.device)
    check(_lib.load().eod_memory_gather_pool(mem_f16.data_ptr(), proj.data_ptr(), H, W, D, N, out.data_ptr(), _ptr(err), int(torch_order),
                                             batch, _stream()),
          "eod_memory_gather_pool")
    return out


class MemoryProjector:

# ... 725 lines not shown
```

include/eod_hip.h:

```cpp
#ifndef EOD_HIP_H
#define EOD_HIP_H
#include <stddef.h>
#include <stdint.h>

#ifdef __cplusplus
extern "C" {
#endif

typedef void* eod_stream_t;

#define EOD_OK 0
#define EOD_ERR_BAD_DIMS (-1)
#define EOD_ERR_ALIGN (-2)
#define EOD_ERR_LAUNCH (-3)
#define EOD_ERR_NULL (-4)
#define EOD_ERR_CAPACITY (-5)

#define EOD_MAX_BATCH 8
#define EOD_MAX_LEVELS 40

int eod_abi_version(void);

typedef struct EodConvDesc {
  const float* x;
  const float* w;
  const float* bias;
  const float* res;
  float* y;
  float* workspace;
  size_t workspace_bytes;
  const int32_t* m_count;
  int32_t m_unit;
  int32_t m_segments;
  int32_t N, H, W, Cin, OH, OW, Cout, KH, KW, stride, pad, Kpad;
  int32_t relu;
  int32_t res_mode;
  int32_t in_relu;
  int32_t out_mode;
  int32_t tap4;
  int32_t force_tile;
  int32_t force_splitk;
  float out_scale;
  int32_t levels;
  int32_t level_off[EOD_MAX_LEVELS + 1];
  int32_t level_h[EOD_MAX_LEVELS];
  int32_t level_w[EOD_MAX_LEVELS];
  const float* fuse_w;
  const int32_t* out_units;
  float fuse_b;
  const void* w_split;
  int32_t plan_rows;
  int32_t lds_reserve;
  double* gn_partial;
  int32_t gn_groups;
  float* y2;
  int32_t split_n;
  int32_t prefetch2;
  const float* gate;
  const void* w_half;
  int32_t math;
} EodConvDesc;
int eod_conv2d(const EodConvDesc* d, eod_stream_t stream);
int eod_conv2d_gn_fused(const EodConvDesc* d);
size_t eod_conv2d_workspace_bytes(const EodConvDesc* d);
typedef struct EodConvPlan {
  int32_t tile;
  int32_t bm, bn, bk;
  int32_t splitk, cps, nchunks;
  int32_t wavek;
  int32_t glds;
  int32_t tiles_m, tiles_n;
  int32_t gn_fused;
} EodConvPlan;
int eod_conv2d_plan(const EodConvDesc* d, EodConvPlan* out);
#define EOD_MATH_FP32 0
#define EOD_MATH_BF16X3 1
#define EOD_MATH_F16 2
int eod_set_conv_math(int mode);
int eod_get_conv_math(void);
size_t eod_conv_split_weights_bytes(int Cout, int Kpad);
int eod_conv_split_weights_bf16x3(const float* w, int Cout, int Kpad, void* out, eod_stream_t stream);
size_t eod_conv_half_weights_bytes(int Cout, int Kpad);
int eod_conv_half_weights(const float* w, int Cout, int Kpad, void* out, eod_stream_t stream);

int eod_preprocess_image(const uint8_t* img_chw, float* out_nhwc4, int H, int W, int Hp, int Wp,
                         const float* mean3, const float* std3, eod_stream_t stream);
int eod_maxpool3x3s2(const float* x, float* y, int N, int H, int W, int C, int OH, int OW, eod_stream_t stream);
size_t eod_groupnorm_workspace_bytes(const int32_t* level_off_host, int levels, int groups);
int eod_groupnorm_relu(const float* x, float* y, const float* gamma, const float* beta, const int32_t* level_off_host,
                       int levels, int C, int groups, float eps, float* stats, int partial_ready, eod_stream_t stream);
size_t eod_groupnorm_partial_offset(int levels, int groups);
size_t eod_groupnorm_backward_workspace_bytes(const int32_t* level_off_host, int levels, int C);
int eod_groupnorm_relu_backward(const float* x, const float* y, const float* dy, const float* gamma, const int32_t* level_off_host,
                                int levels, int C, int groups, float eps, const float* fwd_stats, void* workspace, float* dx,
                                float* dgamma, float* dbeta, eod_stream_t stream);
int eod_mask_predictor_sigmoid(const float* x, const float* w, float bias, float* prob, int rows, int C,
                               const int32_t* unit_count, int unit_rows, const int32_t* out_units ,
                               eod_stream_t stream);

typedef struct EodBoxRefine {
  const float* deltas;
  int32_t ld;
  float wx, wy, ww, wh;
  int32_t clip;
  float img_w, img_h;
  float* boxes_out;
} EodBoxRefine;
int eod_roi_align(const float* p3, const float* p4, const float* p5, int h3, int w3, int C,
                  const float* boxes , const int32_t* box_rows ,
                  const int32_t* count, int R_cap, int out_size, float* out , int batch, int boxes_per_image,
                  const EodBoxRefine* refine, eod_stream_t stream);

int eod_roi_align_backward(float* dp3, float* dp4, float* dp5, int h3, int w3, int C, const float* boxes ,
                           const int32_t* count, int R_cap, int out_size, const float* g, eod_stream_t stream);

typedef struct EodCenterNetLossDesc {
  const float* head_out;
  int32_t head_stride;
  int32_t P;
  int32_t levels;
  int32_t level_off[9];
  float level_scale[8];
  const float* agn_heatmap;
  const float* reg_targets;
  const int32_t* pos_inds;
  int32_t n_pos;
  float hm_focal_alpha, hm_focal_beta, loss_gamma, sigmoid_clamp, ignore_high_fp;
  float pos_weight, neg_weight, reg_weight;
  float num_pos_avg;
  float reg_norm;
  const int32_t* counts_local;
  const int32_t* counts_total;
  float world_size;
  float* d_head_out;
  float* losses;
  void* workspace;
  size_t workspace_bytes;
} EodCenterNetLossDesc;
size_t eod_centernet_loss_workspace_bytes(void);
int eod_centernet_loss(const EodCenterNetLossDesc* d, eod_stream_t stream);

typedef struct EodCenterNetTargetDesc {
  const float* gt_boxes;
  int32_t n_boxes;
  int32_t levels;
  int32_t level_off[9];
  int32_t level_w[8];
  int32_t level_stride[8];
  float soi_lo[8], soi_hi[8];
  double hm_min_overlap;
  double min_radius;
  float* agn_heatmap;
  float* reg_targets;
  int32_t* pos_inds;
  int32_t* counts;
} EodCenterNetTargetDesc;
int eod_centernet_targets(const EodCenterNetTargetDesc* d, eod_stream_t stream);

#define EOD_LOSS_FED (1 << 30)
#define EOD_FED_LOSS_PARAM_BYTES(C) ((16 + 12 * (size_t)(C) + 15) & ~(size_t)15)
size_t eod_fast_rcnn_loss_workspace_bytes(int B);
int eod_fast_rcnn_loss(const float* scores, int ld, const float* deltas , const float* proposal_boxes, const float* gt_boxes,
                       const int32_t* gt_classes, const float* class_weight, int B, int num_classes, float wx, float wy, float ww,
                       float wh, float smooth_l1_beta, float* d_scores, float* d_deltas, float* losses, void* workspace,
                       size_t workspace_bytes, eod_stream_t stream);

int eod_match_label(const float* boxes , int R, const float* gt_boxes , const int32_t* gt_classes , int G,
                    float iou_thresh, int num_classes, int32_t* matched_idx , float* matched_iou ,
                    int32_t* out_classes , float* out_gt_boxes , eod_stream_t stream);
int eod_match_label_proposals(const float* prop_boxes , const int32_t* prop_count , int cap,
                              const float* gt_boxes , const int32_t* gt_classes , int G, int append_gt, float iou_thresh,
                              int num_classes, float* all_boxes, int32_t* matched_idx, float* matched_iou, int32_t* out_classes,
                              float* out_gt_boxes, eod_stream_t stream);
int eod_sample_proposals(const int32_t* classes, const float* keys , int R, int num_classes,
                         int batch_size_per_image, float positive_fraction, int32_t* sampled_idx, int32_t* counts, eod_stream_t stream);
int eod_zs_logits(const float* feat, const float* zs_weight, int B, int D , int C1, float temp, float* logits, int ld,
                  float* featn_out, eod_stream_t stream);

int eod_zs_logits_backward(const float* feat, const float* zs_weight, const float* d_logits, int ld, int B, int D , int C1,
                           float temp, float* d_feat, eod_stream_t stream);

typedef struct EodProposalDesc {
  const float* head_out;
  int32_t head_stride;
  int32_t levels;
  int32_t level_off[6];
  int32_t level_w[5];
  int32_t level_stride[5];
  float level_scale[5];
  float score_thresh;
  int32_t pre_nms_topk;
  int32_t post_nms_topk;
  float nms_thresh;
  int32_t cap;
  float* out_boxes;
  float* out_scores;
  int32_t* out_count;
  void* workspace;
  size_t workspace_bytes;
  int32_t batch;
} EodProposalDesc;
size_t eod_proposals_workspace_bytes(int total_positions, int levels, int pre_nms_topk, int batch);
int eod_centernet_proposals(const EodProposalDesc* d, eod_stream_t stream);

#define EOD_ZS_WIDE 2
typedef struct EodStageTailDesc {
  const float* feat;
  const float* zs;
  float* prob_acc;
  int32_t accumulate;
  float* feat_norm_out;
  const int32_t* count;
  int32_t R_cap, D, C1;
  float temp;
  const float* zs_mem;
  const float* prop_scores;
  float* mem_scores_out;
  float final_inv_stages;
  int32_t batch;
  const float* hb;
  const float* w2;
  const float* b2;
  int32_t hb_dim, w2_ld;
  const float* boxes_in;
  float* boxes_out;
  float* deltas_out;
  float wx, wy, ww, wh;
  int32_t clip;
  float img_w, img_h;
} EodStageTailDesc;
int eod_cascade_stage_tail(const EodStageTailDesc* d, eod_stream_t stream);
int eod_zs_classify(const float* feat , const float* zs , float* prob_acc , int accumulate,
                    float* feat_norm_out , const int32_t* count, int R_cap, int D, int C1, float temp,
                    const float* zs_mem, const float* prop_scores, float* mem_scores_out, float final_inv_stages, int batch,
                    eod_stream_t stream);
int eod_apply_deltas(const float* deltas , int ld, const float* boxes, float* out, const int32_t* count, int R_cap,
                     float wx, float wy, float ww, float wh, int clip, float img_w, float img_h, int batch, eod_stream_t stream);
int eod_cascade_scores(float* prob_acc, const float* prop_scores, const int32_t* count, int R_cap, int C1, float inv_stages,
                       eod_stream_t stream);

typedef struct EodDetDesc {
  const float* boxes;
  const float* scores;
  const int32_t* count;
  int32_t R_cap, C1;
  float img_w, img_h, score_thresh, nms_thresh;
  int32_t topk;
  float* out_boxes;
  float* out_scores;
  int32_t* out_classes;
  int32_t* out_rows;
  int32_t* out_count;
  void* workspace; size_t workspace_bytes;
  int32_t* out_unique_rows;
  int32_t* out_unique_count;
  int32_t unique_cap;
  int32_t* out_rep_of;
  int32_t* out_rep_list;
  int32_t* out_rep_count;
  int32_t batch;
} EodDetDesc;
size_t eod_detections_workspace_bytes(int R_cap, int C1);
int eod_fast_rcnn_inference(const EodDetDesc* d, eod_stream_t stream);

int eod_concat_lists(const int32_t* lists, const int32_t* counts, int cap_in, int id_stride, int batch, int32_t* out ,
                     int32_t* out_count , eod_stream_t stream);

int eod_detector_postprocess(const float* boxes, const float* scores, const int32_t* classes, const int32_t* count, int cap,
                             float sx, float sy, float out_w, float out_h, float* out_boxes, float* out_scores,
                             int32_t* out_classes, int32_t* out_src, int32_t* out_count, const int32_t* remap, int batch,
                             eod_stream_t stream);
int eod_paste_masks(const float* prob, const float* boxes, const int32_t* rows, const int32_t* count, int K_cap,
                    int H, int W, float threshold, uint8_t* out, int batch, int prob_units ,
                    eod_stream_t stream);

int eod_unproject_grid_index(const float* depth, int H, int W, const float* T16_host, float fx, float fy, float cx, float cy,
                             const float* proj_shift3_host, const float* map_shift3_host, float cell, int map_w, int map_h,
                             int order, float* xyz_or_null, int32_t* idx, eod_stream_t stream);
int eod_memory_normalize_f16(const float* mem, const float* obs, uint16_t* out_f16, int n_cells, int D, eod_stream_t stream);
int eod_memory_normalize_dirty_f16(const float* mem, const float* obs, int32_t* dirty, uint16_t* out_f16, int n_cells, int D,
                                   eod_stream_t stream);
#define EOD_FLAG_BAD_CELL_INDEX 1
size_t eod_memory_pooled_halves(int H, int W);
int eod_memory_gather_pool(const uint16_t* mem_f16, const int32_t* proj, int H, int W, int D, int n_cells,
                           uint16_t* pooled_f16, int32_t* err_flags, int torch_order, int batch, eod_stream_t stream);
size_t eod_memory_project_weights_bytes(void);
int eod_memory_project_prepare(const float* w1, const float* b1, const float* w2, const float* b2, const float* w3,
                               const float* b3, void* prepared, eod_stream_t stream);
int eod_memory_project_fuse(const uint16_t* pooled_f16, const void* prepared, float* feats, int H, int W, float weight,
                            int mode, int batch, eod_stream_t stream);
int eod_memory_scores(const float* featn , const float* zs, const float* prop_scores, float* scores ,
                      const int32_t* count, int R_cap, int D, int C1, eod_stream_t stream);
int eod_unique_rows(const int32_t* rows, const int32_t* count, int K_cap, int R_cap, int32_t* out_rows, int32_t* out_count,
                    eod_stream_t stream);
int eod_memory_project_backward_weights(const float* g3, const float* g4, const float* g5, const uint16_t* pooled_f16, int H, int W,
                                        float weight, float* dw3, float* db3, float* dw4, float* db4, float* dw5, float* db5,
                                        eod_stream_t stream);
size_t eod_memory_project_backward_weights_workspace_bytes(void);
int eod_memory_project_backward_weights_ws(const float* g3, const float* g4, const float* g5, const uint16_t* pooled_f16, int H, int W,
                                           float weight, float* dw3, float* db3, float* dw4, float* db4, float* dw5, float* db5,
                                           void* workspace, size_t workspace_bytes, eod_stream_t stream);
int eod_memory_pool_backward(const float* dec3, const float* dec4, const float* dec5, int H, int W, uint16_t* ge3_f16, uint16_t* ge4_f16,
                             uint16_t* ge5_f16, float* ge2, eod_stream_t stream);

int eod_conv2d_backward_weights(const float* x, const float* g, int N, int H, int W, int Cin, int Cout, int KH, int KW, int pad,
                                int stride, float* dw, float* db, eod_stream_t stream);
size_t eod_conv2d_backward_weights_workspace_bytes(int N, int H, int W, int Cin, int Cout, int KH, int KW, int pad, int stride);
int eod_conv2d_backward_weights_ws(const float* x, const float* g, int N, int H, int W, int Cin, int Cout, int KH, int KW, int pad,
                                   int stride, float* dw, float* db, void* workspace, size_t workspace_bytes, eod_stream_t stream);
#define EOD_WGRAD_F16 512
size_t eod_conv2d_backward_weights_levels_workspace_bytes(int rows, int Cin, int Cout, int KH, int KW);
int eod_conv2d_backward_weights_levels(const float* x, const float* g, int levels, const int32_t* level_off, const int32_t* level_h,
                                       const int32_t* level_w, int Cin, int Cout, int KH, int KW, int pad, float* dw, float* db,
                                       void* workspace, size_t workspace_bytes, eod_stream_t stream);
int eod_conv2d_backward_input(const float* g, const float* w, int Kpad, int N, int H, int W, int Cin, int Cout, int KH, int KW, int pad,
                              int stride, float* dx, eod_stream_t stream);
int eod_upsample2_sum_backward(const float* g, float* out, int N, int h, int w, int C, int accumulate, eod_stream_t stream);
int eod_maxpool3x3s2_backward(const float* x, const float* y, const float* g, float* dx, int N, int H, int W, int C, int OH, int OW,
                              eod_stream_t stream);
int eod_relu_backward(const float* g, const float* y, float* out, size_t n, eod_stream_t stream);

int eod_adamw_step(float* param, const float* grad, float* exp_avg, float* exp_avg_sq, size_t n, double lr, double beta1, double beta2,
                   double eps, double weight_decay, int step, double clip_value, eod_stream_t stream);

int eod_conv_rotate_weights(const float* w, int Cout, int KH, int KW, int Cin, int ld_in, float* out, int ld_out, eod_stream_t stream);

typedef struct EodRotateTensor {
  const float* w;
  float* out;
  int32_t Cout, KH, KW, Cin, ld_in, ld_out;
} EodRotateTensor;
int eod_conv_rotate_weights_multi(const EodRotateTensor* tensors, int count, eod_stream_t stream);

typedef struct EodAdamWTensor {
  float* param;
  const float* grad;
  float* exp_avg;
  float* exp_avg_sq;
  size_t n;
  double lr;
  double weight_decay;
  int32_t step;
  float* folded_out;
  const float* row_scale;
  int32_t cols, ld_out;
  int32_t grad_of_folded;
  float inv_scale;
  int32_t* found_inf;
} EodAdamWTensor;
int eod_adamw_step_multi(const EodAdamWTensor* tensors, int count, double beta1, double beta2, double eps, double clip_value,
                         eod_stream_t stream);

typedef struct EodMemWriteDesc {
  const float* featn;
  const float* prop_boxes;
  const float* prop_masks;
  const int32_t* det_rows;
  const int32_t* det_count;
  int32_t K_cap, R_cap;
  const int32_t* proj;
  int32_t H, W, D, n_cells;
  float mask_thresh;
// ... 35 lines not shown
```

Baseline: 306.6.

## Write batched FPN outputs into pyramid slots and reuse preallocated trunk inputs

Adds a per-image output stride to the conv epilogue so batched FPN output convs can write straight into the per-set pyramid buffers, skipping the later copies. Frame preprocessing now writes into a cached batch tensor instead of calling torch.cat. Also adds an opt-in 64-row wavek conv kernel variant, whose auto-selection is off by default. The trade-off is extra stride arithmetic in the epilogue, a larger descriptor, and a fallback path used when a strided write is rejected.

```diff
diff --git a/embodied_object_detection_amd/_lib.py b/embodied_object_detection_amd/_lib.py
--- a/embodied_object_detection_amd/_lib.py
+++ b/embodied_object_detection_amd/_lib.py
@@ -39,7 +39,7 @@
         ("level_w", C.c_int32 * MAX_LEVELS), ("fuse_w", C.c_void_p), ("out_units", C.c_void_p), ("fuse_b", C.c_float), ("w_split", C.c_void_p),
         ("plan_rows", C.c_int32), ("lds_reserve", C.c_int32), ("gn_partial", C.c_void_p), ("gn_groups", C.c_int32),
         ("y2", C.c_void_p), ("split_n", C.c_int32), ("prefetch2", C.c_int32), ("gate", C.c_void_p),
-        ("w_half", C.c_void_p), ("math", C.c_int32),
+        ("w_half", C.c_void_p), ("y_image_stride", C.c_int64), ("math", C.c_int32),
     ]
 
 
diff --git a/embodied_object_detection_amd/csrc/conv_common.h b/embodied_object_detection_amd/csrc/conv_common.h
--- a/embodied_object_detection_amd/csrc/conv_common.h
+++ b/embodied_object_detection_amd/csrc/conv_common.h
@@ -39,6 +39,8 @@
   FastDiv div_ow, div_oh, div_cd, div_row;
   int border;
   FastDiv div_bh, div_bw, div_bi;
+  long long y_img_extra;
+  FastDiv div_img;
 };
 
 __device__ __forceinline__ int conv_row_limit(const ConvArgs& p, int M) {
@@ -74,7 +76,7 @@
   return (b.img * p.OH + b.oy) * p.OW + b.ox;
 }
 
-template <bool GATE = false>
+template <bool GATE = false, bool STRIDED = false>
 __device__ __forceinline__ float epilogue_store(const ConvArgs& p, float v, int m, int n) {
   int co = n;
   size_t oidx;
@@ -90,6 +92,7 @@
     oidx = ((size_t)(img * 2 * p.OH + 2 * oy + dy) * (2 * p.OW) + (2 * ox + dx)) * Cd + co;
   } else {
     oidx = (size_t)m * p.Cout + n;
+    if constexpr (STRIDED) oidx += (size_t)fdiv((unsigned)m, p.div_img) * (size_t)p.y_img_extra;
   }
   if (p.bias) v += p.bias[co];
   v *= p.out_scale;
@@ -131,7 +134,7 @@
   return mask;
 }
 
-template <int TM, int TN, bool GATE = false, bool BORDER = false>
+template <int TM, int TN, bool GATE = false, bool BORDER = false, bool STRIDED = false>
 __device__ __forceinline__ void store_wave_tiles(const ConvArgs& p, const f32x16 (&acc)[TM][TN], int m_base, int n_base, int M, int z,
                                                  int lane) {
   const int half = lane >> 5;
@@ -152,7 +155,7 @@
           } else if (p.splitk > 1) {
             p.partial[((size_t)z * p.M + m) * p.Cout + n] = v;
           } else {
-            epilogue_store<GATE>(p, v, m, n);
+            epilogue_store<GATE, STRIDED>(p, v, m, n);
           }
         }
       }
@@ -162,7 +165,7 @@
 
 void launch_conv_fp32(const ConvArgs& a, int tile, int bk, bool tap4, dim3 grid, hipStream_t s, int lds_reserve = 0, int prefetch2 = 0);
 void launch_conv_bf16x3(const ConvArgs& a, int tile, dim3 grid, hipStream_t s);
-void launch_conv_wavek(const ConvArgs& a, int nw, dim3 grid, hipStream_t s);
+void launch_conv_wavek(const ConvArgs& a, int nw, bool rows64, dim3 grid, hipStream_t s);
 void launch_conv_pointwise(const ConvArgs& a, int np, dim3 grid, hipStream_t s);
 void launch_split_weights(const float* w, void* out, int Cout, int Kpad, hipStream_t s);
 void launch_conv_f16(const ConvArgs& a, int tile, int bk, dim3 grid, hipStream_t s);
diff --git a/embodied_object_detection_amd/csrc/conv_fp32.hip b/embodied_object_detection_amd/csrc/conv_fp32.hip
--- a/embodied_object_detection_amd/csrc/conv_fp32.hip
+++ b/embodied_object_detection_amd/csrc/conv_fp32.hip
@@ -269,72 +269,76 @@
 }
 
 
-template <int NW, bool MULTI>
-__global__ __launch_bounds__(NW * 64) void conv_wavek_kernel(ConvArgs p) {
+template <int NW, bool MULTI, int RB>
+__device__ __forceinline__ void wavek_tile(const ConvArgs& p, float* lds, int wave_lds, int M, int m0, int n0) {
   constexpr int BK = 32;
   constexpr int LS = BK + 4;
   constexpr int AR = 4;
-  __shared__ __attribute__((aligned(16))) float lds[NW * 2 * 32 * LS];
   const int tid = threadIdx.x;
   const int lane = tid & 63;
   const int wave = tid >> 6;
-  float* As = lds + wave * (2 * 32 * LS);
-  float* Bs = As + 32 * LS;
-
-  int M;
-  const int t = conv_first_tile<32>(p, M);
-  if (t < 0) return;
-  const int tile_m = t / p.tiles_n;
-  const int tile_n = t - tile_m * p.tiles_n;
-  const int m0 = tile_m * 32, n0 = tile_n * 32;
-  if (!conv_tile_active(p, m0, 32)) return;
+  float* As = lds + wave * wave_lds;
+  float* Bs = As + RB * 32 * LS;
 
   int c_end;
   const int c_begin = conv_chunk_range(p, (p.nchunks + NW - 1) / NW, wave, c_end);
 
   const int lr = lane >> 3, lq = lane & 7;
-  unsigned a_voff[AR];
-  unsigned long long a_mask[AR];
-  unsigned a_pitch[MULTI ? AR : 1];
+  unsigned a_voff[RB * AR];
+  constexpr bool PACKED = RB == 2;
+  unsigned long long a_mask[PACKED ? 1 : AR];
+  unsigned a_mask2[PACKED ? AR : 1];
+  unsigned a_pitch[MULTI ? RB * AR : 1];
   unsigned w_voff[AR];
 #pragma unroll
-  for (int i = 0; i < AR; ++i) {
-    conv_row_address<MULTI>(p, m0 + lr + 8 * i, M, lq, a_voff[i], a_mask[i], a_pitch[MULTI ? i : 0]);
-    w_voff[i] = conv_w_row_offset(p, n0 + lr + 8 * i, lq);
-  }
+  for (int i = 0; i < RB * AR; ++i) {
+    unsigned long long mask;
+    conv_row_address<MULTI>(p, m0 + lr + 8 * i, M, lq, a_voff[i], mask, a_pitch[MULTI ? i : 0]);
+    if constexpr (PACKED) a_mask2[i % AR] = i < AR ? (unsigned)mask : (a_mask2[i % AR] | ((unsigned)mask << 16));
+    else a_mask[i] = mask;
+  }
+#pragma unroll
+  for (int j = 0; j < AR; ++j) w_voff[j] = conv_w_row_offset(p, n0 + lr + 8 * j, lq);
   const __amdgpu_buffer_rsrc_t rsrc_x = conv_buffer(p.x, p.x_bytes);
   const __amdgpu_buffer_rsrc_t rsrc_w = conv_buffer(p.w, p.w_bytes);
 
-  f32x4 ar0[AR], br0[AR], ar1[AR], br1[AR];
+  f32x4 ar0[RB * AR], br0[AR], ar1[RB * AR], br1[AR];
   ChunkWalker<BK, MULTI> walk(p, c_begin);
-  auto load_chunk = [&](int chunk, f32x4 (&ar)[AR], f32x4 (&br)[AR]) {
+  auto load_chunk = [&](int chunk, f32x4 (&ar)[RB * AR], f32x4 (&br)[AR]) {
     const int k0 = chunk * BK;
     const TapInfo ti = walk.next(p);
 #pragma unroll
-    for (int i = 0; i < AR; ++i) ar[i] = conv_load_a<MULTI>(rsrc_x, ti, a_voff[i], a_mask[i], a_pitch[MULTI ? i : 0]);
+    for (int i = 0; i < RB * AR; ++i) {
+      if constexpr (PACKED)
+        ar[i] = conv_load_a_if<MULTI>(rsrc_x, ti, a_voff[i], (a_mask2[i % AR] >> (ti.tap + 16 * (i / AR))) & 1u, a_pitch[MULTI ? i : 0]);
+      else
+        ar[i] = conv_load_a<MULTI>(rsrc_x, ti, a_voff[i], a_mask[i], a_pitch[MULTI ? i : 0]);
+    }
     if (p.in_relu) {
 #pragma unroll
-      for (int i = 0; i < AR; ++i) ar[i] = conv_relu4(ar[i]);
+      for (int i = 0; i < RB * AR; ++i) ar[i] = conv_relu4(ar[i]);
     }
 #pragma unroll
     for (int j = 0; j < AR; ++j)
       br[j] = __builtin_bit_cast(f32x4, __builtin_amdgcn_raw_buffer_load_b128(rsrc_w, w_voff[j], k0 * 4, 0));
   };
 
-  f32x16 acc, acc_b;
-#pragma unroll
-  for (int r = 0; r < 16; ++r) {
-    acc[r] = 0.f;
-    acc_b[r] = 0.f;
-  }
+  f32x16 acc[RB], acc_b[RB];
+#pragma unroll
+  for (int b = 0; b < RB; ++b)
+#pragma unroll
+    for (int r = 0; r < 16; ++r) {
+      acc[b][r] = 0.f;
+      acc_b[b][r] = 0.f;
+    }
   const int frag_row = lane & 31;
   const int frag_k = 4 * (lane >> 5);
   const float* a_base = As + frag_row * LS + frag_k;
   const float* b_base = Bs + frag_row * LS + frag_k;
 
-  auto stage_and_multiply = [&](f32x4 (&ar)[AR], f32x4 (&br)[AR], int next_chunk) {
-#pragma unroll
-    for (int i = 0; i < AR; ++i) *reinterpret_cast<f32x4*>(As + (lr + 8 * i) * LS + 4 * lq) = ar[i];
+  auto stage_and_multiply = [&](f32x4 (&ar)[RB * AR], f32x4 (&br)[AR], int next_chunk) {
+#pragma unroll
+    for (int i = 0; i < RB * AR; ++i) *reinterpret_cast<f32x4*>(As + (lr + 8 * i) * LS + 4 * lq) = ar[i];
 #pragma unroll
     for (int j = 0; j < AR; ++j) *reinterpret_cast<f32x4*>(Bs + (lr + 8 * j) * LS + 4 * lq) = br[j];
     __builtin_amdgcn_fence(__ATOMIC_RELEASE, "wavefront");
@@ -343,12 +347,15 @@
     if (next_chunk < c_end) load_chunk(next_chunk, ar, br);
 #pragma unroll
     for (int kk = 0; kk < BK / 8; ++kk) {
-      const f32x4 af = *reinterpret_cast<const f32x4*>(a_base + kk * 8);
       const f32x4 bf = *reinterpret_cast<const f32x4*>(b_base + kk * 8);
-      acc = __builtin_amdgcn_mfma_f32_32x32x2f32(af[0], bf[0], acc, 0, 0, 0);
-      acc_b = __builtin_amdgcn_mfma_f32_32x32x2f32(af[1], bf[1], acc_b, 0, 0, 0);
-      acc = __builtin_amdgcn_mfma_f32_32x32x2f32(af[2], bf[2], acc, 0, 0, 0);
-      acc_b = __builtin_amdgcn_mfma_f32_32x32x2f32(af[3], bf[3], acc_b, 0, 0, 0);
+#pragma unroll
+      for (int b = 0; b < RB; ++b) {
+        const f32x4 af = *reinterpret_cast<const f32x4*>(a_base + b * 32 * LS + kk * 8);
+        acc[b] = __builtin_amdgcn_mfma_f32_32x32x2f32(af[0], bf[0], acc[b], 0, 0, 0);
+        acc_b[b] = __builtin_amdgcn_mfma_f32_32x32x2f32(af[1], bf[1], acc_b[b], 0, 0, 0);
+        acc[b] = __builtin_amdgcn_mfma_f32_32x32x2f32(af[2], bf[2], acc[b], 0, 0, 0);
+        acc_b[b] = __builtin_amdgcn_mfma_f32_32x32x2f32(af[3], bf[3], acc_b[b], 0, 0, 0);
+      }
     }
     __builtin_amdgcn_fence(__ATOMIC_RELEASE, "wavefront");
     __builtin_amdgcn_wave_barrier();
@@ -361,23 +368,60 @@
     if (chunk + 1 < c_end) stage_and_multiply(ar1, br1, chunk + 3);
   }
 #pragma unroll
-  for (int r = 0; r < 16; ++r) acc[r] += acc_b[r];
+  for (int b = 0; b < RB; ++b)
+#pragma unroll
+    for (int r = 0; r < 16; ++r) acc[b][r] += acc_b[b][r];
 
   __syncthreads();
   float* red = lds;
   if (wave > 0) {
 #pragma unroll
-    for (int r = 0; r < 16; ++r) red[((wave - 1) * 16 + r) * 64 + lane] = acc[r];
+    for (int b = 0; b < RB; ++b)
+#pragma unroll
+      for (int r = 0; r < 16; ++r) red[(((wave - 1) * RB + b) * 16 + r) * 64 + lane] = acc[b][r];
   }
   __syncthreads();
   if (wave != 0) return;
 #pragma unroll
-  for (int w = 1; w < NW; ++w)
-#pragma unroll
-    for (int r = 0; r < 16; ++r) acc[r] += red[((w - 1) * 16 + r) * 64 + lane];
-  f32x16 out[1][1];
-  out[0][0] = acc;
-  store_wave_tiles<1, 1, true>(p, out, m0, n0, M, 0, lane);
+  for (int b = 0; b < RB; ++b) {
+    f32x16 out[1][1];
+    out[0][0] = acc[b];
+#pragma unroll
+    for (int w = 1; w < NW; ++w)
+#pragma unroll
+      for (int r = 0; r < 16; ++r) out[0][0][r] += red[(((w - 1) * RB + b) * 16 + r) * 64 + lane];
+    store_wave_tiles<1, 1, true, false, true>(p, out, m0 + 32 * b, n0, M, 0, lane);
+    if (RB > 1) __builtin_amdgcn_sched_barrier(0);
+  }
+}
+
+template <int NW, bool MULTI>
+__global__ __launch_bounds__(NW * 64) void conv_wavek_kernel(ConvArgs p) {
+  constexpr int WAVE_LDS = 2 * 32 * 36;
+  __shared__ __attribute__((aligned(16))) float lds[NW * WAVE_LDS];
+  int M;
+  const int t = conv_first_tile<32>(p, M);
+  if (t < 0) return;
+  const int tile_m = t / p.tiles_n;
+  const int tile_n = t - tile_m * p.tiles_n;
+  const int m0 = tile_m * 32, n0 = tile_n * 32;
+  if (!conv_tile_active(p, m0, 32)) return;
+  wavek_tile<NW, MULTI, 1>(p, lds, WAVE_LDS, M, m0, n0);
+}
+
+template <int NW>
+__global__ __launch_bounds__(NW * 64, 2) void conv_wavek_rows_kernel(ConvArgs p) {
+  constexpr int WAVE_LDS = 3 * 32 * 36;
+  __shared__ __attribute__((aligned(16))) float lds[NW * WAVE_LDS];
+  int M;
+  const int t = conv_first_tile<64>(p, M);
+  if (t < 0) return;
+  const int tile_m = t / p.tiles_n;
+  const int tile_n = t - tile_m * p.tiles_n;
+  const int m0 = tile_m * 64, n0 = tile_n * 32;
+  if (!conv_tile_active(p, m0, 64)) return;
+  if (m0 + 32 < M) wavek_tile<NW, false, 2>(p, lds, WAVE_LDS, M, m0, n0);
+  else wavek_tile<NW, false, 1>(p, lds, WAVE_LDS, M, m0, n0);
 }
 
 }
@@ -419,8 +463,11 @@
   }
 }
 
-void launch_conv_wavek(const ConvArgs& a, int nw, dim3 grid, hipStream_t s) {
-  if (a.nlv > 0) {
+void launch_conv_wavek(const ConvArgs& a, int nw, bool rows64, dim3 grid, hipStream_t s) {
+  if (rows64) {
+    if (nw == 8) hipLaunchKernelGGL((conv_wavek_rows_kernel<8>), grid, dim3(512), 0, s, a);
+    else hipLaunchKernelGGL((conv_wavek_rows_kernel<4>), grid, dim3(256), 0, s, a);
+  } else if (a.nlv > 0) {
     if (nw == 8) hipLaunchKernelGGL((conv_wavek_kernel<8, true>), grid, dim3(512), 0, s, a);
     else hipLaunchKernelGGL((conv_wavek_kernel<4, true>), grid, dim3(256), 0, s, a);
   } else {
diff --git a/embodied_object_detection_amd/csrc/conv_igemm.hip b/embodied_object_detection_amd/csrc/conv_igemm.hip
--- a/embodied_object_detection_amd/csrc/conv_igemm.hip
+++ b/embodied_object_detection_amd/csrc/conv_igemm.hip
@@ -31,14 +31,14 @@
         for (int j = 0; j < 4; ++j)
           if (zb + j < p.splitk) v += t[j];
       }
-      epilogue_store<true>(p, v.x, (int)m, (int)n);
-      epilogue_store<true>(p, v.y, (int)m, (int)n + 1);
-      epilogue_store<true>(p, v.z, (int)m, (int)n + 2);
-      epilogue_store<true>(p, v.w, (int)m, (int)n + 3);
+      epilogue_store<true, true>(p, v.x, (int)m, (int)n);
+      epilogue_store<true, true>(p, v.y, (int)m, (int)n + 1);
+      epilogue_store<true, true>(p, v.z, (int)m, (int)n + 2);
+      epilogue_store<true, true>(p, v.w, (int)m, (int)n + 3);
     } else {
       float v = 0.f;
       for (int z = 0; z < p.splitk; ++z) v += src[z * slab];
-      epilogue_store<true>(p, v, (int)m, (int)n);
+      epilogue_store<true, true>(p, v, (int)m, (int)n);
     }
   }
 }
@@ -121,6 +121,7 @@
   int glds;
   int bm, bn, tiles_m, tiles_n, splitk, cps, nchunks;
   int wavek;
+  int wavek_rows64;
   int pw_np;
   int border;
 };
@@ -144,6 +145,17 @@
          d->m_count && d->m_segments <= 1 && d->m_unit == d->OH * d->OW && d->OH >= 3 && d->OW >= 3 && d->Cin % 32 == 0 &&
          d->out_mode == 0 && d->res_mode == 0 && !d->in_relu && !d->gate && d->split_n == 0 && !d->gn_partial && d->prefetch2 == 0;
 }
+
+constexpr int kForceWaveKRows4 = 46, kForceWaveKRows8 = 47;
+bool wavek_rows_forced(const EodConvDesc* d) { return d->force_tile == kForceWaveKRows4 || d->force_tile == kForceWaveKRows8; }
+
+bool wavek_rows_eligible(const EodConvDesc* d) {
+  return d->levels <= 0 && !d->tap4 && d->out_mode != 2 && d->Kpad / 32 >= 8 && d->KH * d->KW <= 16 && d->force_splitk == 0;
+}
+
+constexpr bool kWaveKRowsAuto = false;
+constexpr int kWaveKRowsMinM = 512;
+constexpr int kWaveKRowsMinCout = 256;
 
 Plan make_plan(const EodConvDesc* d, int M) {
   static const int cfg[5][2] = {{128, 128}, {128, 64}, {64, 64}, {256, 128}, {64, 256}};
@@ -194,14 +206,19 @@
   } else if (d->force_splitk > 0) {
     splitk = d->force_splitk;
   } else if (pl.glds == 0 && !d->tap4 && nchunks >= 8 &&
-             ((d->force_tile == 6 || d->force_tile == 7) ||
+             ((d->force_tile == 6 || d->force_tile == 7 || wavek_rows_forced(d)) ||
               (tiles < 256 && nchunks <= 192 && pl.bk == 32 && d->force_tile == 0 &&
                ((Mp <= 512 && nchunks / (nchunks >= 64 ? 8 : 4) >= 8) || nchunks >= 128)))) {
-    pl.wavek = d->force_tile == 6 ? 4 : (d->force_tile == 7 ? 8 : (nchunks >= 64 ? 8 : 4));
+    const int ftw = d->force_tile % 10;
+    pl.wavek = ftw == 6 ? 4 : (ftw == 7 ? 8 : (nchunks >= 64 ? 8 : 4));
+    pl.wavek_rows64 = (wavek_rows_forced(d) || (kWaveKRowsAuto && d->force_tile == 0 && wavek_rows_eligible(d) && M >= kWaveKRowsMinM &&
+                                                d->Cout >= kWaveKRowsMinCout && !d->m_count))
+                          ? 1 : 0;
     pl.bk = 32;
     pl.nchunks = d->Kpad / 32;
-    pl.bm = pl.bn = 32;
-    pl.tiles_m = (M + 31) / 32;
+    pl.bm = pl.wavek_rows64 ? 64 : 32;
+    pl.bn = 32;
+    pl.tiles_m = (M + pl.bm - 1) / pl.bm;
     pl.tiles_n = (d->Cout + 31) / 32;
   } else if (tiles < 256 && nchunks >= 8) {
     const int target = (nchunks >= 128 && Mp <= 512) ? 1792 : 512;
@@ -248,6 +265,7 @@
     pl.splitk = 1;
     pl.cps = pl.nchunks;
     pl.wavek = 0;
+    pl.wavek_rows64 = 0;
   }
   const bool border_forced = d->force_tile == kForceBorder && d->force_splitk <= 1;
   const bool border_auto = kBorderAuto && d->force_tile == 0 && border_eligible(d) && pl.glds == 0 && pl.tile == 3 && pl.bk == 32 &&
@@ -305,7 +323,8 @@
     if (((long)(d->N / d->m_segments) * d->OH * d->OW) % d->m_unit != 0) return EOD_ERR_BAD_DIMS;
   }
   if (d->gate && (d->out_mode != 0 || d->split_n != 0 || d->gn_partial)) return EOD_ERR_BAD_DIMS;
-  if (d->gate && d->force_tile != 0 && d->force_tile % 10 != 3 && d->force_tile != 6 && d->force_tile != 7) return EOD_ERR_BAD_DIMS;
+  if (d->gate && d->force_tile != 0 && d->force_tile % 10 != 3 && d->force_tile != 6 && d->force_tile != 7 && !wavek_rows_forced(d))
+    return EOD_ERR_BAD_DIMS;
   if (d->gate && d->force_tile / 10 == 5) return EOD_ERR_BAD_DIMS;
   if (d->gate && (d->force_tile / 10 == 8 || d->force_tile / 10 == 9) &&
       (d->math != EOD_MATH_F16 + 1 || d->force_tile % 10 != 3 || d->levels > 0 || d->tap4 || d->in_relu))
@@ -315,6 +334,7 @@
   if (d->lds_reserve < 0 || d->lds_reserve > 48 * 1024) return EOD_ERR_BAD_DIMS;
   if (d->force_tile == kForcePointwise && (!pointwise_eligible(d) || d->force_splitk > 1)) return EOD_ERR_BAD_DIMS;
   if (d->force_tile == kForceBorder && (!border_eligible(d) || d->force_splitk > 1)) return EOD_ERR_BAD_DIMS;
+  if (wavek_rows_forced(d) && !wavek_rows_eligible(d)) return EOD_ERR_BAD_DIMS;
   if (d->split_n != 0) {
     if (!d->y2) return EOD_ERR_NULL;
     if (d->split_n < 0 || d->split_n >= d->Cout || d->out_mode != 0 || d->res_mode != 0 || d->levels > 0 || d->gn_partial)
@@ -326,6 +346,10 @@
         cpg > 64 || (cpg & (cpg - 1)) != 0 || cpg < 4 || d->Cout % 4 != 0 || d->Cout > 1024 || 256 % (d->Cout / 4) != 0 ||
         64 % (cpg / 4) != 0)
       return EOD_ERR_BAD_DIMS;
+  }
+  if (d->y_image_stride != 0) {
+    if (d->levels > 0 || d->out_mode != 0 || d->split_n != 0 || d->m_count || d->gn_partial || d->gate) return EOD_ERR_BAD_DIMS;
+    if (d->y_image_stride < (long long)d->OH * d->OW * d->Cout || d->y_image_stride % 4 != 0) return EOD_ERR_BAD_DIMS;
   }
   if (!eod_aligned16(d->x) || !eod_aligned16(d->w) || !eod_aligned16(d->w_split) || !eod_aligned16(d->w_half)) return EOD_ERR_ALIGN;
   return EOD_OK;
@@ -438,6 +462,12 @@
   a.split_n = d->split_n;
   const Plan pl = make_plan(d, a.M);
   if (d->gn_partial && pl.splitk <= 1) return EOD_ERR_BAD_DIMS;
+  if (d->y_image_stride != 0 && !(pl.splitk > 1 || pl.wavek)) return EOD_ERR_BAD_DIMS;
+  {
+    const long long img_rows = (long long)d->OH * d->OW;
+    a.y_img_extra = d->y_image_stride != 0 ? d->y_image_stride - img_rows * d->Cout : 0;
+    a.div_img = eod_make_fastdiv((unsigned)(img_rows > 0 ? img_rows : 1));
+  }
   a.nchunks = pl.nchunks;
   a.splitk = pl.splitk; a.cps = pl.cps; a.tiles_m = pl.tiles_m; a.tiles_n = pl.tiles_n;
   a.border = pl.border;
@@ -448,7 +478,7 @@
   dim3 grid(pl.tiles_m * pl.tiles_n, pl.splitk);
   if (pl.border) grid.x = (pl.tiles_m + 7) / 8 * 8 * pl.tiles_n;
   if (pl.pw_np) launch_conv_pointwise(a, pl.pw_np, grid, s);
-  else if (pl.wavek) launch_conv_wavek(a, pl.wavek, grid, s);
+  else if (pl.wavek) launch_conv_wavek(a, pl.wavek, pl.wavek_rows64 != 0, grid, s);
   else if (pl.glds == 3) launch_conv_f16(a, pl.tile, pl.bk, grid, s);
   else if (pl.glds == 2) launch_conv_bf16x3(a, pl.tile, grid, s);
   else launch_conv_fp32(a, pl.tile, pl.bk, d->tap4 != 0, grid, s, d->lds_reserve, d->prefetch2);
diff --git a/embodied_object_detection_amd/csrc/conv_operands.h b/embodied_object_detection_amd/csrc/conv_operands.h
--- a/embodied_object_detection_amd/csrc/conv_operands.h
+++ b/embodied_object_detection_amd/csrc/conv_operands.h
@@ -140,13 +140,16 @@
 };
 
 template <bool MULTI>
-__device__ __forceinline__ f32x4 conv_load_a(__amdgpu_buffer_rsrc_t rsrc_x, const TapInfo& ti, unsigned voff, unsigned long long mask,
-                                             unsigned pitch) {
-  const bool ok = (mask >> ti.tap) & 1ull;
+__device__ __forceinline__ f32x4 conv_load_a_if(__amdgpu_buffer_rsrc_t rsrc_x, const TapInfo& ti, unsigned voff, bool ok, unsigned pitch) {
   unsigned vo = voff + ti.tap_off;
   if (MULTI) vo += (unsigned)ti.ky * pitch;
   vo = ok ? vo : 0xFFFFFFFFu;
   return __builtin_bit_cast(f32x4, __builtin_amdgcn_raw_buffer_load_b128(rsrc_x, vo, 0, 0));
+}
+template <bool MULTI>
+__device__ __forceinline__ f32x4 conv_load_a(__amdgpu_buffer_rsrc_t rsrc_x, const TapInfo& ti, unsigned voff, unsigned long long mask,
+                                             unsigned pitch) {
+  return conv_load_a_if<MULTI>(rsrc_x, ti, voff, (mask >> ti.tap) & 1ull, pitch);
 }
 
 __device__ __forceinline__ f32x4 conv_relu4(f32x4 v) {
diff --git a/embodied_object_detection_amd/modeling/backbone.py b/embodied_object_detection_amd/modeling/backbone.py
--- a/embodied_object_detection_amd/modeling/backbone.py
+++ b/embodied_object_detection_amd/modeling/backbone.py
@@ -5,6 +5,7 @@
 import torch
 
 from .. import ops
+from .._lib import EodError
 from ..registry import BACKBONE_REGISTRY
 
 RESNET50_LAYERS = (3, 4, 6, 3)
@@ -95,6 +96,8 @@
         self.merge = ops.MemoryProjector([sd[f"backbone.map_merge_projection{i}.weight"] for i in (1, 2, 3)],
                                          [sd[f"backbone.map_merge_projection{i}.bias"] for i in (1, 2, 3)], device)
         self._plans = {}
+        self._arenas = {}
+        self.pyramid_sets = 2
         self.pool_in_torch_order = True
 
     def level_shapes(self, H: int, W: int) -> List[Tuple[int, int]]:
@@ -110,7 +113,10 @@
             off = [0]
             for (h, w) in shapes:
                 off.append(off[-1] + h * w)
-            feats = torch.empty((off[-1], 256), dtype=torch.float32, device=self.device)
+            if (H, W) not in self._arenas:
+                self._arenas[(H, W)] = torch.empty((max(self.pyramid_sets, which + 1), off[-1], 256), dtype=torch.float32, device=self.device)
+            arena = self._arenas[(H, W)]
+            feats = arena[which] if which < arena.shape[0] else torch.empty((off[-1], 256), dtype=torch.float32, device=self.device)
             views = [feats[off[i]:off[i + 1]].view(1, shapes[i][0], shapes[i][1], 256) for i in range(5)]
             pooled = torch.empty((ops.pooled_rows(H, W), 512), dtype=torch.float16, device=self.device)
             self._plans[key] = (shapes, off, feats, views, pooled)
@@ -127,14 +133,35 @@
         lat3 = self.lateral[3](c3, 1, h3, w3, res=lat4, res_mode=2)
         self.output[3](lat3, 1, h3, w3, out=views[0])
 
-    def top_down_batched(self, c: dict, H: int, W: int, N: int):
+    def set_stride(self, H: int, W: int, first: int, N: int) -> int:
+        self._plan(H, W, first)
+        arena = self._arenas[(H, W)]
+        if first < 0 or first + N > arena.shape[0] or ops.get_conv_math() != "fp32":
+            return 0
+        return arena.stride(0)
+
+    def _output_batched(self, l: int, lat: torch.Tensor, N: int, h: int, w: int, first_view: Optional[torch.Tensor], stride: int):
+        conv = self.output[l]
+        if stride:
+            try:
+                with conv.strided_output(stride):
+                    conv(lat, N, h, w, plan_rows=h * w, out=first_view)
+                return None
+            except EodError as e:
+                if "EOD_ERR_BAD_DIMS" not in str(e):
+                    raise
+        return conv(lat, N, h, w, plan_rows=h * w)
+
+    def top_down_batched(self, c: dict, H: int, W: int, N: int, first_set: Optional[int] = None):
         (c5, h5, w5), (c4, h4, w4), (c3, h3, w3) = c["layer5"], c["layer4"], c["layer3"]
+        stride = self.set_stride(H, W, first_set, N) if first_set is not None else 0
+        views = self._plan(H, W, first_set)[3] if stride else [None] * 3
         lat5 = self.lateral[5](c5, N, h5, w5, plan_rows=h5 * w5)
-        p5 = self.output[5](lat5, N, h5, w5, plan_rows=h5 * w5)
+        p5 = self._output_batched(5, lat5, N, h5, w5, views[2], stride)
         lat4 = self.lateral[4](c4, N, h4, w4, res=lat5, res_mode=2, plan_rows=h4 * w4)
-        p4 = self.output[4](lat4, N, h4, w4, plan_rows=h4 * w4)
+        p4 = self._output_batched(4, lat4, N, h4, w4, views[1], stride)
         lat3 = self.lateral[3](c3, N, h3, w3, res=lat4, res_mode=2, plan_rows=h3 * w3)
-        p3 = self.output[3](lat3, N, h3, w3, plan_rows=h3 * w3)
+        p3 = self._output_batched(3, lat3, N, h3, w3, views[0], stride)
         return [p3, p4, p5]
 
     def fuse_memory_and_top(self, H: int, W: int, memory_f16: Optional[torch.Tensor], proj: Optional[torch.Tensor], which: int = 0,
diff --git a/embodied_object_detection_amd/modeling/batched.py b/embodied_object_detection_amd/modeling/batched.py
--- a/embodied_object_detection_amd/modeling/batched.py
+++ b/embodied_object_detection_amd/modeling/batched.py
@@ -48,6 +48,7 @@
         self.streams = list(self._stream_pool)
         self.trunk_stream = torch.cuda.Stream(device=self.device, priority=-1)
         self._ev_in = torch.cuda.Event()
+        self._trunk_inputs = {}
         self._ev_trunk = torch.cuda.Event()
         self._ev_done = [[torch.cuda.Event(), torch.cuda.Event()] for _ in range(batch)]
         for m in self.scenes:
@@ -67,11 +68,13 @@
         H, W = int(frames[0]["image"].shape[-2]), int(frames[0]["image"].shape[-1])
         if any((int(f["image"].shape[-2]), int(f["image"].shape[-1])) != (H, W) for f in frames):
             raise ValueError("the frames of one lock-step must have one size")
-        xs = []
-        for m, f in zip(scenes, frames):
-            x4, Hp, Wp = ops.preprocess_image(m._device_image(f), m.pixel_mean, m.pixel_std)
-            xs.append(x4)
-        x = torch.cat(xs, dim=0)
+        Hp, Wp = (H + 31) // 32 * 32, (W + 31) // 32 * 32
+        key = (B, Hp, Wp, torch.cuda.current_stream(self.device).cuda_stream)
+        if key not in self._trunk_inputs:
+            self._trunk_inputs[key] = torch.empty((B, Hp, Wp, 4), dtype=torch.float32, device=self.device)
+        x = self._trunk_inputs[key]
+        for b, (m, f) in enumerate(zip(scenes, frames)):
+            ops.preprocess_image(m._device_image(f), m.pixel_mean, m.pixel_std, out=x[b:b + 1])
         c = m0.backbone.bottom_up.forward(x, Hp, Wp, N=B)
         p345 = m0.backbone.top_down_batched(c, Hp, Wp, B)
         for b, (m, f) in enumerate(zip(scenes, frames)):
diff --git a/embodied_object_detection_amd/modeling/meta_arch.py b/embodied_object_detection_amd/modeling/meta_arch.py
--- a/embodied_object_detection_amd/modeling/meta_arch.py
+++ b/embodied_object_detection_amd/modeling/meta_arch.py
@@ -107,6 +107,7 @@
         self._ev_call = None
         self._ev_det = [None] * RESULT_SETS
         self._pyr_reader = {}
+        self._trunk_inputs = {}
         self._frame_no = 0
 
         num_classes = int(cfg.MODEL.ROI_HEADS.NUM_CLASSES)
@@ -128,6 +129,7 @@
         self.C1 = self.zs_weight.shape[1]
 
         self.backbone = BACKBONE_REGISTRY.get(cfg.MODEL.BACKBONE.NAME)(cfg, state_dict, self.device)
+        self.backbone.pyramid_sets = PYRAMID_SETS
         self.proposal_generator = PROPOSAL_GENERATOR_REGISTRY.get(cfg.MODEL.PROPOSAL_GENERATOR.NAME)(cfg, state_dict, self.device)
         self.roi_heads = ROI_HEADS_REGISTRY.get(cfg.MODEL.ROI_HEADS.NAME)(cfg, state_dict, self.device, self.proposal_generator.cap)
         R = self.proposal_generator.cap
@@ -313,23 +315,32 @@
                 ts.wait_event(self._pyr_reader[st])
         with torch.cuda.stream(ts):
             self._mark("trunk_lookahead_begin", ts)
-            xs = []
-            for f in frames:
-                x4, Hp, Wp = ops.preprocess_image(self._device_image(f), self.pixel_mean, self.pixel_std)
-                xs.append(x4)
-            if len(frames) == 1:
-                self.backbone.top_down(self.backbone.bottom_up.forward(xs[0], Hp, Wp), Hp, Wp, sets[0])
+            n = len(frames)
+            imgs = [self._device_image(f) for f in frames]
+            x = self._trunk_input(n, imgs[0])
+            for b, img in enumerate(imgs):
+                _x4, Hp, Wp = ops.preprocess_image(img, self.pixel_mean, self.pixel_std, out=x[b:b + 1])
+            if n == 1:
+                self.backbone.top_down(self.backbone.bottom_up.forward(x, Hp, Wp), Hp, Wp, sets[0])
             else:
-                n = len(frames)
-                c = self.backbone.bottom_up.forward(torch.cat(xs, dim=0), Hp, Wp, N=n)
-                p345 = self.backbone.top_down_batched(c, Hp, Wp, n)
+                c = self.backbone.bottom_up.forward(x, Hp, Wp, N=n)
+                consecutive = all(st == sets[0] + b for b, st in enumerate(sets))
+                p345 = self.backbone.top_down_batched(c, Hp, Wp, n, first_set=sets[0] if consecutive else None)
                 for b, st in enumerate(sets):
                     views = self.backbone._plan(Hp, Wp, st)[3]
                     for l in range(3):
-                        views[l].copy_(p345[l][b:b + 1])
+                        if p345[l] is not None:
+                            views[l].copy_(p345[l][b:b + 1])
             done.record(ts)
             self._mark("trunk_lookahead", ts)
         self._ahead = self._ahead + [dict(image=f["image"], Hp=Hp, Wp=Wp, event=done) for f in frames]
+
+    def _trunk_input(self, n: int, img: torch.Tensor) -> torch.Tensor:
+        Hp, Wp = (int(img.shape[-2]) + 31) // 32 * 32, (int(img.shape[-1]) + 31) // 32 * 32
+        key = (n, Hp, Wp)
+        if key not in self._trunk_inputs:
+            self._trunk_inputs[key] = torch.empty((n, Hp, Wp, 4), dtype=torch.float32, device=self.device)
+        return self._trunk_inputs[key]
 
     def inference_frame(self, frame: dict, refresh_memory_snapshot: bool = True, materialize: bool = True,
                         next_frame=None, trailing_detection_pass: bool = False):
diff --git a/embodied_object_detection_amd/ops.py b/embodied_object_detection_amd/ops.py
--- a/embodied_object_detection_amd/ops.py
+++ b/embodied_object_detection_amd/ops.py
@@ -1,5 +1,6 @@
 from __future__ import annotations
 
+import contextlib
 import ctypes as C
 from typing import Dict, Optional, Sequence, Tuple
 
@@ -118,6 +119,7 @@
         self.event_tag = None
         self.lds_reserve = 0
         self.prefetch2 = 0
+        self.out_image_stride = 0
 
     def out_hw(self, H: int, W: int) -> Tuple[int, int]:
         return ((H + 2 * self.pad - self.KH) // self.stride + 1, (W + 2 * self.pad - self.KW) // self.stride + 1)
@@ -161,6 +163,7 @@
         d.plan_rows = plan_rows
         d.lds_reserve = self.lds_reserve
         d.prefetch2 = self.prefetch2
+        d.y_image_stride = self.out_image_stride
         d.gn_partial, d.gn_groups = None, 0
         self.gn_fused = False
         if split is not None:
@@ -213,6 +216,14 @@
         check(self._lib.eod_conv2d(C.byref(d), _stream()), f"eod_conv2d[{self.name}]")
         return out
 
+    @contextlib.contextmanager
+    def strided_output(self, stride: int):
+        self.out_image_stride = int(stride)
+        try:
+            yield self
+        finally:
+            self.out_image_stride = 0
+
     def plan(self) -> Dict[str, int]:
         p = _lib.EodConvPlan()
         check(self._lib.eod_conv2d_plan(C.byref(self.desc), C.byref(p)), f"eod_conv2d_plan[{self.name}]")
diff --git a/include/eod_hip.h b/include/eod_hip.h
--- a/include/eod_hip.h
+++ b/include/eod_hip.h
@@ -58,6 +58,7 @@
   int32_t prefetch2;
   const float* gate;
   const void* w_half;
+  int64_t y_image_stride;
   int32_t math;
 } EodConvDesc;
 int eod_conv2d(const EodConvDesc* d, eod_stream_t stream);
```

Result: no change. 306.3 (-0.1%).
